# jzhang-dev/FEDRANN

Hardware: AMD Instinct MI355X
Metric: read-pairs/sec (overlap candidates) (higher is better)
Workload: dtype f32 (canonical fp32 results; fp16 MFMA candidate prefilter + exact fp32 re-rank)

## Files before the change

### fedrann_amd/csrc/fedrann_hip.hip

```cpp
#include <hip/hip_runtime.h>
#include <rocprim/device/device_radix_sort.hpp>
#include <rocprim/device/device_scan.hpp>
#include <rocprim/device/device_run_length_encode.hpp>
#include <rocprim/device/device_merge.hpp>
#include <rocprim/device/device_reduce_by_key.hpp>

#include <algorithm>
#include <array>
#include <atomic>
#include <cmath>
#include <condition_variable>
#include <cstdarg>
#include <cstdint>
#include <cstdio>
#include <cstdlib>
#include <cstring>
#include <functional>
#include <limits>
#include <mutex>
#include <new>
#include <string>
#include <thread>
#include <type_traits>
#include <utility>
// ... 392 lines not shown
    auto ask = [&](const auto &call) {
        size_t bytes = 0;
        if (e == hipSuccess) e = call(nullptr, bytes);
        need = std::max(need, bytes);
    };
    (ask(calls), ...);
    if (e != hipSuccess) return fail(FDR_E_HIP, "rocprim temporary storage size query failed: %s", hipGetErrorString(e));
    return tmp.reserve(need);
}
template <class F>
static int rocprim_run(DevArray<char> &tmp, const char *what, const F &call) {
    if (int rc = rocprim_reserve(tmp, call)) return rc;
    size_t bytes = tmp.bytes();
    const hipError_t e = call(tmp.ptr(), bytes);
    if (e != hipSuccess)
        return fail(e == hipErrorOutOfMemory ? FDR_E_NOMEM : FDR_E_HIP, "%s failed: %s", what, hipGetErrorString(e));
    return FDR_OK;
}

struct PinnedBuf {
    void *p = nullptr;
    size_t cap = 0;
    int reserve(size_t bytes) {
        if (bytes <= cap) return FDR_OK;
        if (p) (void)hipHostFree(p);
        p = nullptr;
        cap = 0;
        hipError_t e = hipHostMalloc(&p, bytes ? bytes : 1, hipHostMallocDefault);
        if (e != hipSuccess) {
            p = nullptr;
            return fail(FDR_E_NOMEM, "hipHostMalloc(%zu bytes) failed: %s", bytes, hipGetErrorString(e));
        }
        cap = bytes;
        return FDR_OK;
    }
    PinnedBuf() = default;
    PinnedBuf(const PinnedBuf &) = delete;
    PinnedBuf &operator=(const PinnedBuf &) = delete;
    ~PinnedBuf() {
        if (p) (void)hipHostFree(p);
    }
};

struct KnnCallRecord {
    struct {
        int flagged = 0;
        int launches = 0, queues = 0;
    } pass;
    int unique_targets = 0, unique_queries = 0;
    struct {
        const uint8_t *dev = nullptr;
        int64_t n = 0;
        uint8_t all = FDR_PATH_NONE;
        hipStream_t stream = nullptr;
    } paths;
    fdr_knn_trace trace = {};
    struct {
        int nseg = 0;
        int nt = 0;
        SegBounds segs;
        hipStream_t stream = nullptr;
    } skip;
};

struct KnnArgs {
    const float *Qhat;
    const uint8_t *qzero;
    int64_t nq;
    const float *That;
    const uint8_t *tzero;
    int64_t nt, t_base;
    int d, k;
    int32_t *idx;
    float *dist;
    void *ws;
    size_t ws_bytes;
    hipStream_t st;
};


struct KmerSearchScratch {
    DevArray<unsigned char> seq;
    DevArray<long long> off;
    DevArray<u64> lib_codes;
    DevArray<u64> keys;
    DevArray<unsigned> vals;
    DevArray<u64> bloom;
    DevArray<unsigned long long> counter;
    DevArray<u64> pairs, sorted;
    DevArray<int> flag, scan;
    DevArray<int> indices, rows;
    DevArray<long long> indptr;
    DevArray<char> tmp;
    long long nnz = 0;
    void release() {
        release_all(seq, off, lib_codes, keys, vals, bloom, counter, pairs, sorted, flag, scan, indices, rows, indptr, tmp);
        nnz = 0;
    }
};

struct KmerCountScratch {
    DevArray<unsigned char> seq;
    DevArray<long long> off;
    DevArray<u64> codes;
    DevArray<u64> sorted;
    DevArray<unsigned> run_len;
    DevArray<unsigned> n_runs;
    DevArray<u64> run_counts;
    DevArray<u64> acc_codes[2], acc_counts[2];
    DevArray<u64> merged_codes, merged_counts;
    DevArray<unsigned long long> n_table;
    DevArray<int> keep, keep_scan;
    DevArray<u64> kept_counts;
    DevArray<long long> run_off, samp_pre;
    DevArray<u64> samples, bounds;
    DevArray<long long> slices;
    DevArray<long long> part_off;
    DevArray<char> tmp;
    int k = 0;
    int acc = 0;
    long long na = 0;
    long long n = 0;
    int64_t block_chars = 0;
    int blocks = 0;
    void release() {
        release_all(seq, off, codes, sorted, run_len, n_runs, run_counts, acc_codes[0], acc_codes[1], acc_counts[0],
                    acc_counts[1], merged_codes, merged_counts, n_table, keep, keep_scan, kept_counts, run_off, samp_pre,
                    samples, bounds, slices, part_off, tmp);
        k = acc = 0;
        na = n = 0;
    }
};

struct SparseIndex {
    DevArray<long long> indptr;
    DevArray<int> indices;
    DevArray<float> values;
    DevArray<float> xhat;
    DevArray<int> asize;
    DevArray<float> mass;
    DevArray<unsigned char> zero;
    DevArray<u64> keys, sorted_keys;
    DevArray<unsigned> pos, sorted_pos;
    DevArray<int> efeat;
    DevArray<float> pval;
    DevArray<long long> runptr;
    DevArray<int> runfeat;
    DevArray<int> heavy;
    DevArray<u64> cnt;
    DevArray<char> tmp;
    struct Built {
        bool valid = false;
        int metric = 0;
        long long n = 0, kept = 0, nzero = 0;
        long long n_features = 0;
    } built;
    int *run_flags() const { return reinterpret_cast<int *>(keys.ptr()); }
    int *run_numbers(long long kept) const { return run_flags() + kept; }
    int *posting_rows() const { return reinterpret_cast<int *>(pos.ptr()); }
    static constexpr size_t cnt_words = 8 + FDR_MAX_K;
    int *zidx() const { return reinterpret_cast<int *>(cnt.ptr() + 8); }
    float *zdist() const { return reinterpret_cast<float *>(zidx() + FDR_MAX_K); }
    template <class F>
    auto each(F f) {
        return f(indptr, indices, values, xhat, asize, mass, zero, keys, sorted_keys, pos, sorted_pos, efeat, pval, runptr,
                 runfeat, heavy, cnt, tmp);
    }
    size_t bytes() {
        return each([](auto &...a) { return (a.bytes() + ...); });
    }
    void release() {
        each([](auto &...a) { release_all(a...); });
        built = {};
    }
};

struct SparseQuerySet {
    DevArray<long long> indptr;
    DevArray<int> indices;
    DevArray<float> values;
    DevArray<float> xhat;
    DevArray<int> efeat;
    DevArray<int> asize;
    DevArray<float> mass;
    DevArray<unsigned char> zero;
    DevArray<int> heavy;
    template <class F>
    auto each(F f) {
        return f(indptr, indices, values, xhat, efeat, asize, mass, zero, heavy);
    }
    size_t bytes() {
        return each([](auto &...a) { return (a.bytes() + ...); });
    }
    void release() {
        each([](auto &...a) { release_all(a...); });
    }
};

#define RR_FLAG_MISMATCH 0
#define RR_FLAG_ZLIST 1
#define RR_FLAG_ZEROQ 2
#define RR_FLAG_NZERO 3
#define RR_FLAGS 4
struct RadiusResult {
    DevArray<long long> count, off;
    DevArray<u64> keys, sorted;
    DevArray<int> zlist;
    DevArray<u64> flags;
    long long counted = 0;
    long long held = -1;
    int *idx() const { return reinterpret_cast<int *>(keys.ptr()); }
    float *dist() const { return reinterpret_cast<float *>(idx() + held); }
    void drop() { held = -1; }
    template <class F>
    auto each(F f) { return f(count, off, keys, sorted, zlist, flags); }
    size_t bytes() { return each([](auto &...a) { return (a.bytes() + ...); }); }
    void release() {
        each([](auto &...a) { release_all(a...); });
        counted = 0;
        held = -1;
    }
};

struct SparseRadius {
    RadiusResult rr;
    DevArray<long long> seg_lo, seg_hi;
    DevArray<unsigned char> handed;
    size_t bytes() { return rr.bytes() + seg_lo.bytes() + seg_hi.bytes() + handed.bytes(); }
    void release() {
        rr.release();
        release_all(seg_lo, seg_hi, handed);
    }
};

struct DenseIndex {
    DevArray<float> ehat;
    DevArray<_Float16> half;
    DevArray<unsigned char> zero;
    DevArray<float> qhat;
    DevArray<_Float16> qhalf;
    DevArray<unsigned char> qzero;
    DevArray<float> theta;
    RadiusResult rr;
    DevArray<long long> ind;
    DevArray<int> fill;
    DevArray<char> tmp;
    bool valid = false;
    long long n = 0, nzero = 0;
    int d = 0, dp = 0;
    long long last_candidates = 0, last_hits = 0;
    int last_query_blocks = 0, last_segments = 0;
    template <class F>
    auto each(F f) {
        return f(ehat, half, zero, qhat, qhalf, qzero, theta, ind, fill, tmp);
    }
    size_t bytes() { return rr.bytes() + each([](auto &...a) { return (a.bytes() + ...); }); }
    void release() {
        each([](auto &...a) { release_all(a...); });
        rr.release();
        valid = false;
        n = nzero = 0;
        d = dp = 0;
        last_candidates = last_hits = 0;
        last_query_blocks = last_segments = 0;
    }
};

struct TopkMergeScratch {
    DevArray<int> idx_parts;
    DevArray<float> dist_parts;
    DevArray<int> idx_out;
    DevArray<float> dist_out;
    DevArray<u64> refusal;
    void release() { release_all(idx_parts, dist_parts, idx_out, dist_out, refusal); }
};

struct fdr_ctx {
    int device = 0;
    int num_cus = 256;
    hipStream_t stream = nullptr;
    hipStream_t aux_stream[3] = {nullptr, nullptr, nullptr};
    hipEvent_t aux_ev[4] = {nullptr, nullptr, nullptr, nullptr};
    hipDeviceProp_t prop;
    long long n_features = 0;
    int d = 0;
    long long p_nnz = 0, p_rows = 0;
    DevBuf ftab, crow, ent;
    std::vector<uint32_t> h_bits;
    DevBuf a_indptr, a_indices, E, Ehat, zero, idx, dist, ws;
    DevBuf c_indptr, c_indices;
    PinnedBuf stage_ids, stage_ptr;
    hipEvent_t up_ev[3] = {nullptr, nullptr, nullptr};
    hup::WorkerPool up_pool;
    KmerSearchScratch ks;
    KmerCountScratch kc;
    SparseIndex sp;
    SparseQuerySet spq;
    SparseRadius spr;
    DenseIndex di;
    TopkMergeScratch tm;
    int knn_mode = FDR_MODE_AUTO;
    int dedup_mode = FDR_DEDUP_AUTO;
    int live_mode = FDR_LIVE_AUTO;
    std::vector<unsigned> live_host;
    int skip_mode = FDR_SKIP_AUTO;
    std::vector<int> skip_host;
    int compact_mode = FDR_COMPACT_AUTO;
    KnnCallRecord last;
    struct {
        int what = 0;
        bool cand_valid = false, range_valid = false;
        int64_t nq = 0, n_range = 0;
        int kp = 0, qbits = 0;
        DevBuf cand, rq, rtheta, rcnt, rrows;
        DevBuf lists;
        hipStream_t stream = nullptr;
    } cap;
    struct {
        bool valid = false;
        const float *That = nullptr;
        const uint8_t *tzero = nullptr;
        int64_t nt = 0, nq_max = 0;
        int d = 0, k = 0, nu = 0;
        void *ws = nullptr;
        size_t ws_bytes = 0;
    } cls;
    bool timing = false;
    std::vector<hipEvent_t> ev_pool[FDR_NUM_KERNELS];
    size_t ev_used[FDR_NUM_KERNELS] = {};
};

static void knn_call_begin(fdr_ctx *ctx) {
    ctx->last.trace = fdr_knn_trace{};
    ctx->last.paths = {};
    ctx->last.skip.nseg = 0;
    ctx->cap.cand_valid = ctx->cap.range_valid = false;
    ctx->cap.nq = ctx->cap.n_range = 0;
}

static void knn_call_header(fdr_ctx *ctx, int kind, int dp, int k, int64_t nq, int64_t nt) {
    ctx->last.trace.kind = kind;
    ctx->last.trace.dp = dp;
    ctx->last.trace.k = k;
    ctx->last.trace.queries = nq;
    ctx->last.trace.targets = nt;
}
static void knn_call_whole(fdr_ctx *ctx, uint8_t path, int kind, int dp, int k, int64_t nq, int64_t nt) {
    knn_call_header(ctx, kind, dp, k, nq, nt);
    ctx->last.paths = {nullptr, nq, path, nullptr};
    ctx->last.pass = {};
}

static int timing_begin(fdr_ctx *ctx, int kind, hipStream_t st) {
    if (!ctx->timing) return FDR_OK;
    std::vector<hipEvent_t> &pool = ctx->ev_pool[kind];
    if (ctx->ev_used[kind] + 2 > pool.size()) {
        hipEvent_t a, b;
        HIP_TRY(hipEventCreate(&a));
        HIP_TRY(hipEventCreate(&b));
        pool.push_back(a);
        pool.push_back(b);
    }
    HIP_TRY(hipEventRecord(pool[ctx->ev_used[kind]], st));
    return FDR_OK;
}

static int timing_end(fdr_ctx *ctx, int kind, hipStream_t st) {
    if (!ctx->timing) return FDR_OK;
    HIP_TRY(hipEventRecord(ctx->ev_pool[kind][ctx->ev_used[kind] + 1], st));
    ctx->ev_used[kind] += 2;
    return FDR_OK;
}

static int use_device(fdr_ctx *ctx) {
    if (!ctx) return fail(FDR_E_ARG, "null context");
    HIP_TRY(hipSetDevice(ctx->device));
    return FDR_OK;
}

FDR_EXPORT const char *fdr_last_error(void) { return g_err; }

FDR_EXPORT int fdr_padded_dim(int d) { return padded_dim(d); }

FDR_EXPORT int fdr_create(int device_id, fdr_ctx **out) {
    if (!out) return fail(FDR_E_ARG, "fdr_create: out is null");
    *out = nullptr;
    int n = 0;
    HIP_TRY(hipGetDeviceCount(&n));
    if (n <= 0) return fail(FDR_E_HIP, "no HIP device visible: the MI355X path cannot run");
    if (device_id < 0 || device_id >= n)
        return fail(FDR_E_ARG, "device %d out of range (have %d)", device_id, n);
    fdr_ctx *c = new (std::nothrow) fdr_ctx();
    if (!c) return fail(FDR_E_NOMEM, "out of host memory");
    c->device = device_id;
    hipError_t e = hipSetDevice(device_id);
    if (e == hipSuccess) e = hipGetDeviceProperties(&c->prop, device_id);
    if (e == hipSuccess) e = hipStreamCreateWithFlags(&c->stream, hipStreamNonBlocking);
    if (e != hipSuccess) {
        delete c;
        return fail(FDR_E_HIP, "fdr_create: device %d: %s", device_id, hipGetErrorString(e));
    }
    c->num_cus = c->prop.multiProcessorCount > 0 ? c->prop.multiProcessorCount : 256;
    if (const char *m = getenv("FDR_KNN_MODE")) {
        if (strcmp(m, "exact") == 0) c->knn_mode = FDR_MODE_EXACT;
        else if (strcmp(m, "prefilter") == 0) c->knn_mode = FDR_MODE_PREFILTER;
    }
    *out = c;
    return FDR_OK;
}

FDR_EXPORT int fdr_destroy(fdr_ctx *ctx) {
    if (!ctx) return FDR_OK;
    (void)hipSetDevice(ctx->device);
    (void)hipStreamSynchronize(ctx->stream);
    ctx->up_pool.stop();
    for (hipEvent_t e : ctx->up_ev)
        if (e) (void)hipEventDestroy(e);
    for (int i = 0; i < FDR_NUM_KERNELS; ++i)
        for (hipEvent_t e : ctx->ev_pool[i]) (void)hipEventDestroy(e);
    (void)hipStreamDestroy(ctx->stream);
    for (hipStream_t a : ctx->aux_stream)
        if (a) {
            (void)hipStreamSynchronize(a);
            (void)hipStreamDestroy(a);
        }
    for (hipEvent_t e : ctx->aux_ev)
        if (e) (void)hipEventDestroy(e);
    delete ctx;
    return FDR_OK;
}

FDR_EXPORT int fdr_device_info(fdr_ctx *ctx, char *buf, int buflen) {
    if (!ctx || !buf || buflen <= 0) return fail(FDR_E_ARG, "fdr_device_info: bad argument");
    snprintf(buf, (size_t)buflen, "%s|%s|%d|%zu", ctx->prop.name, ctx->prop.gcnArchName,
             ctx->prop.multiProcessorCount, (size_t)ctx->prop.totalGlobalMem);
    return FDR_OK;
}

FDR_EXPORT int fdr_last_uncertified(fdr_ctx *ctx) { return ctx ? ctx->last.pass.flagged : 0; }

FDR_EXPORT int fdr_last_query_paths(fdr_ctx *ctx, uint8_t *paths, int64_t n_queries) {
    int rc = use_device(ctx);
    if (rc) return rc;
    if (!paths || n_queries <= 0) return fail(FDR_E_ARG, "last_query_paths: bad argument");
    const auto &rec = ctx->last.paths;
    if (rec.n != n_queries)
        return fail(FDR_E_STATE, "last_query_paths: the last k-NN call recorded codes for %lld query rows, not %lld",
                    (long long)rec.n, (long long)n_queries);
    if (!rec.dev) {
        memset(paths, rec.all, (size_t)n_queries);
        return FDR_OK;
    }
    HIP_TRY(hipMemcpyAsync(paths, rec.dev, (size_t)n_queries, hipMemcpyDeviceToHost, rec.stream));
    HIP_TRY(hipStreamSynchronize(rec.stream));
    return FDR_OK;
}

FDR_EXPORT int fdr_last_unique(fdr_ctx *ctx, int *unique_targets, int *unique_queries) {
    if (!ctx || !unique_targets || !unique_queries) return fail(FDR_E_ARG, "bad argument");
    *unique_targets = ctx->last.unique_targets;
    *unique_queries = ctx->last.unique_queries;
    return FDR_OK;
}

FDR_EXPORT int fdr_last_prefilter_launches(fdr_ctx *ctx, int *launches, int *queues) {
    if (!ctx || !launches || !queues) return fail(FDR_E_ARG, "bad argument");
    *launches = ctx->last.pass.launches;
    *queues = ctx->last.pass.queues;
    return FDR_OK;
}

FDR_EXPORT int fdr_last_knn_trace(fdr_ctx *ctx, fdr_knn_trace *out) {
    if (!ctx || !out) return fail(FDR_E_ARG, "bad argument");
    *out = ctx->last.trace;
    return FDR_OK;
}

FDR_EXPORT int fdr_set_knn_capture(fdr_ctx *ctx, int what) {
    if (!ctx || what < 0 || what > (FDR_CAPTURE_CANDIDATES | FDR_CAPTURE_RANGE | FDR_CAPTURE_LIVE_LISTS)) return fail(FDR_E_ARG, "bad capture flags");
    ctx->cap.what = what;
    return FDR_OK;
}

FDR_EXPORT int fdr_last_candidates(fdr_ctx *ctx, uint64_t *keys, int64_t n_queries, int32_t kp, int32_t *qbits_out) {
    int rc = use_device(ctx);
    if (rc) return rc;
    if (!keys || n_queries <= 0 || kp <= 0) return fail(FDR_E_ARG, "last_candidates: bad argument");
    if (!ctx->cap.cand_valid) return fail(FDR_E_STATE, "last_candidates: the last k-NN call captured no candidates");
    if (ctx->cap.nq != n_queries || ctx->cap.kp != kp)
        return fail(FDR_E_STATE, "last_candidates: the last k-NN call captured %lld x %d keys, not %lld x %d",
                    (long long)ctx->cap.nq, ctx->cap.kp, (long long)n_queries, kp);
    HIP_TRY(hipMemcpyAsync(keys, ctx->cap.cand.p, (size_t)n_queries * kp * 8, hipMemcpyDeviceToHost, ctx->cap.stream));
    HIP_TRY(hipStreamSynchronize(ctx->cap.stream));
    if (qbits_out) *qbits_out = ctx->cap.qbits;
    return FDR_OK;
}

FDR_EXPORT int fdr_last_range_sets(fdr_ctx *ctx, int64_t n_range, int32_t *queries, float *theta, int32_t *counts,
                                   int32_t *rows) {
    int rc = use_device(ctx);
    if (rc) return rc;
    if (!queries || !theta || !counts || !rows || n_range <= 0) return fail(FDR_E_ARG, "last_range_sets: bad argument");
    if (!ctx->cap.range_valid) return fail(FDR_E_STATE, "last_range_sets: the last k-NN call captured no range pass");
    if (ctx->cap.n_range != n_range)
        return fail(FDR_E_STATE, "last_range_sets: the last k-NN call captured %lld range queries, not %lld",
                    (long long)ctx->cap.n_range, (long long)n_range);
    const hipStream_t st = ctx->cap.stream;
    HIP_TRY(hipMemcpyAsync(queries, ctx->cap.rq.p, (size_t)n_range * 4, hipMemcpyDeviceToHost, st));
    HIP_TRY(hipMemcpyAsync(theta, ctx->cap.rtheta.p, (size_t)n_range * 4, hipMemcpyDeviceToHost, st));
    HIP_TRY(hipMemcpyAsync(counts, ctx->cap.rcnt.p, (size_t)n_range * 4, hipMemcpyDeviceToHost, st));
    HIP_TRY(hipMemcpyAsync(rows, ctx->cap.rrows.p, (size_t)n_range * RANGE_CAP * 4, hipMemcpyDeviceToHost, st));
    HIP_TRY(hipStreamSynchronize(st));
    for (int64_t i = 0; i < n_range; ++i)
        for (int m = std::max(0, std::min(counts[i], RANGE_CAP)); m < RANGE_CAP; ++m) rows[i * RANGE_CAP + m] = -1;
    return FDR_OK;
}

FDR_EXPORT int fdr_set_knn_mode(fdr_ctx *ctx, int mode) {
    if (!ctx || mode < FDR_MODE_AUTO || mode > FDR_MODE_PREFILTER) return fail(FDR_E_ARG, "bad k-NN mode");
    ctx->knn_mode = mode;
    return FDR_OK;
}

FDR_EXPORT int fdr_set_dedup_mode(fdr_ctx *ctx, int mode) {
    if (!ctx || mode < FDR_DEDUP_AUTO || mode > FDR_DEDUP_FORCE) return fail(FDR_E_ARG, "bad duplicate-row mode");
    ctx->dedup_mode = mode;
    return FDR_OK;
}

FDR_EXPORT int fdr_set_live_chunks(fdr_ctx *ctx, int mode) {
    if (!ctx || mode < FDR_LIVE_AUTO || mode > FDR_LIVE_FORCE) return fail(FDR_E_ARG, "bad live-chunk mode");
    ctx->live_mode = mode;
    return FDR_OK;
}

FDR_EXPORT int fdr_set_live_skip(fdr_ctx *ctx, int mode) {
    if (!ctx || mode < FDR_SKIP_AUTO || mode > FDR_SKIP_OFF) return fail(FDR_E_ARG, "bad stage-skip mode");
    ctx->skip_mode = mode;
    return FDR_OK;
}

FDR_EXPORT int fdr_set_rerank_compact(fdr_ctx *ctx, int mode) {
    if (!ctx || mode < FDR_COMPACT_AUTO || mode > FDR_COMPACT_FORCE) return fail(FDR_E_ARG, "bad compact re-rank mode");
    ctx->compact_mode = mode;
    return FDR_OK;
}

FDR_EXPORT int fdr_last_live_stage_lists(fdr_ctx *ctx, int32_t segment, int32_t *first_row_out, int32_t *nstages_out,
                                         int32_t *lens, uint16_t *lists) {
    int rc = use_device(ctx);
    if (rc) return rc;
    const auto &rec = ctx->last.skip;
    if (rec.nseg <= 0)
        return fail(FDR_E_STATE, "last_live_stage_lists: the last k-NN call captured no live-chunk pass's stage lists");
    if (segment < 0 || segment >= rec.nseg || !nstages_out)
        return fail(FDR_E_ARG, "last_live_stage_lists: bad argument (the pass had %d segments)", rec.nseg);
    const int t_begin = rec.segs.b[segment], t_end = std::min(rec.nt, rec.segs.b[segment + 1]);
    const int nstages = t_end > t_begin ? (t_end - t_begin + 127) >> 7 : 0;
    *nstages_out = nstages;
    if (first_row_out) *first_row_out = t_begin;
    if (lens) memcpy(lens, ctx->skip_host.data() + (size_t)segment * 256, 256 * sizeof(int));
    if (!lists || nstages == 0) return FDR_OK;
    const int stride = live_list_stride(nstages);
    HIP_TRY(hipMemcpy2DAsync(lists, (size_t)nstages * 2, static_cast<const uint16_t *>(ctx->cap.lists.p) + (size_t)live_stage_row(t_begin, segment) * 256,
                             (size_t)stride * 2, (size_t)nstages * 2, 256, hipMemcpyDeviceToHost, rec.stream));
    HIP_TRY(hipStreamSynchronize(rec.stream));
    for (int v = 0; v < 256; ++v)
        for (int i = std::max(0, std::min(ctx->skip_host[(size_t)segment * 256 + v], nstages)); i < nstages; ++i)
            lists[(size_t)v * nstages + i] = 0xffffu;
    return FDR_OK;
}

FDR_EXPORT int fdr_timing(fdr_ctx *ctx, int enable) {
    if (!ctx) return fail(FDR_E_ARG, "null context");
    ctx->timing = enable != 0;
    for (int i = 0; i < FDR_NUM_KERNELS; ++i) ctx->ev_used[i] = 0;
    return FDR_OK;
}

FDR_EXPORT int fdr_timing_read(fdr_ctx *ctx, int which, int *count_out, float *total_ms_out) {
    int rc = use_device(ctx);
    if (rc) return rc;
    if (which < 0 || which >= FDR_NUM_KERNELS || !count_out || !total_ms_out)
        return fail(FDR_E_ARG, "fdr_timing_read: bad argument");
    float total = 0.f;
    const size_t used = ctx->ev_used[which];
    for (size_t i = 0; i + 1 < used; i += 2) {
        float ms = 0.f;
        HIP_TRY(hipEventSynchronize(ctx->ev_pool[which][i + 1]));
        HIP_TRY(hipEventElapsedTime(&ms, ctx->ev_pool[which][i], ctx->ev_pool[which][i + 1]));
        total += ms;
    }
    *count_out = (int)(used / 2);
    *total_ms_out = total;
    ctx->ev_used[which] = 0;
    return FDR_OK;
}

FDR_EXPORT int fdr_projection_load(fdr_ctx *ctx, int64_t n_features, int32_t d,
                                   const int64_t *p_indptr, const int32_t *p_cols,
                                   const float *p_vals) {
    int rc = use_device(ctx);
    if (rc) return rc;
    ProjectionTables T;
    if ((rc = build_projection_tables(n_features, d, p_indptr, p_cols, p_vals, T))) return rc;
    const std::vector<PU2> &ftab = T.ftab, &ent = T.ent;
    const std::vector<PU4> &crow = T.rowinfo;
    const int64_t nnz = p_indptr[n_features];
    const unsigned rows = T.rows;
    static_assert(sizeof(PU2) == sizeof(uint2) && sizeof(PU4) == sizeof(uint4), "table records = the kernel's uint2 / uint4");
    if ((rc = ctx->ftab.reserve(ftab.size() * sizeof(uint2)))) return rc;
    if ((rc = ctx->crow.reserve(crow.size() * sizeof(uint4)))) return rc;
    if ((rc = ctx->ent.reserve(ent.size() * sizeof(uint2)))) return rc;
    HIP_TRY(hipMemcpyAsync(ctx->ftab.p, ftab.data(), ftab.size() * sizeof(uint2), hipMemcpyHostToDevice, ctx->stream));
    HIP_TRY(hipMemcpyAsync(ctx->crow.p, crow.data(), crow.size() * sizeof(uint4), hipMemcpyHostToDevice, ctx->stream));
    HIP_TRY(hipMemcpyAsync(ctx->ent.p, ent.data(), ent.size() * sizeof(uint2), hipMemcpyHostToDevice, ctx->stream));
    HIP_TRY(hipStreamSynchronize(ctx->stream));
    ctx->n_features = n_features;
    ctx->d = d;
    ctx->p_nnz = nnz;
    ctx->p_rows = rows;
    ctx->h_bits.resize(ftab.size());
    for (size_t w = 0; w < ftab.size(); ++w) ctx->h_bits[w] = ftab[w].x;
    return FDR_OK;
}

FDR_EXPORT int fdr_csr_compact(fdr_ctx *ctx, int64_t n_rows, const int64_t *a_indptr, const int32_t *a_indices,
                               int64_t *out_indptr, int32_t *out_indices, int64_t out_capacity, int32_t n_threads) {
    if (!ctx) return fail(FDR_E_ARG, "null context");
    if (ctx->n_features <= 0) return fail(FDR_E_STATE, "csr_compact: no projection loaded");
    return csrc::compact(ctx->h_bits, ctx->n_features, n_rows, a_indptr, a_indices, out_indptr, out_indices,
                         out_capacity, n_threads);
}

FDR_EXPORT int fdr_host_register(fdr_ctx *ctx, void *ptr, size_t bytes) {
    int rc = use_device(ctx);
    if (rc) return rc;
    if (!ptr || bytes == 0) return fail(FDR_E_ARG, "host_register: empty buffer");
    HIP_TRY(hipHostRegister(ptr, bytes, hipHostRegisterDefault));
    return FDR_OK;
}

FDR_EXPORT int fdr_host_unregister(fdr_ctx *ctx, void *ptr) {
    int rc = use_device(ctx);
    if (rc) return rc;
    if (!ptr) return fail(FDR_E_ARG, "host_unregister: null pointer");
    HIP_TRY(hipHostUnregister(ptr));
    return FDR_OK;
}

static int launch_embed(fdr_ctx *ctx, int64_t n_rows, const int64_t *d_indptr,
                        const int32_t *d_indices, float *d_E, hipStream_t st) {
    if (ctx->n_features <= 0) return fail(FDR_E_STATE, "embed: no projection loaded");
    if (n_rows < 0) return fail(FDR_E_ARG, "embed: n_rows < 0");
    if (n_rows == 0) return FDR_OK;
    const int dp = fdr_padded_dim(ctx->d);
    const long long blocks_needed = (n_rows + 7) / 8;
    const int grid = (int)std::min<long long>(blocks_needed, (long long)ctx->num_cus * 8 * 4);
    int trc = timing_begin(ctx, FDR_KERNEL_EMBED, st);
    if (trc) return trc;
#define FDR_LAUNCH_EMBED(DP_)                                                                   \
    hipLaunchKernelGGL(FDR_EMBED_KERNEL<DP_>, dim3(grid), dim3(256), 0, st, (long long)n_rows,  \
                       (const long long *)d_indptr, d_indices, ctx->n_features,                 \
                       (const uint2 *)ctx->ftab.p, (const uint4 *)ctx->crow.p,                  \
                       (const uint2 *)ctx->ent.p, ctx->d, d_E)
#define FDR_EMBED_KERNEL embed_csr_kernel
    if (dp == 128)
        FDR_LAUNCH_EMBED(128);
    else if (dp == 256)
        FDR_LAUNCH_EMBED(256);
    else if (dp == 512)
        FDR_LAUNCH_EMBED(512);
#undef FDR_EMBED_KERNEL
#define FDR_EMBED_KERNEL embed_csr_wide_kernel
    else if (dp == 1024)
        FDR_LAUNCH_EMBED(1024);
    else
        FDR_LAUNCH_EMBED(2048);
#undef FDR_EMBED_KERNEL
#undef FDR_LAUNCH_EMBED
    HIP_TRY(hipGetLastError());
    return timing_end(ctx, FDR_KERNEL_EMBED, st);
}

static int launch_normalize(fdr_ctx *ctx, const float *d_E, int64_t n_rows, int d, float *d_Ehat,
                            uint8_t *d_zero, hipStream_t st) {
    const int dp = fdr_padded_dim(d);
    if (dp < 0) return fail(FDR_E_ARG, "normalize: dimension %d unsupported (1..%d)", d, FDR_MAX_DIM);
    if (n_rows < 0) return fail(FDR_E_ARG, "normalize: n_rows < 0");
    if (n_rows == 0) return FDR_OK;
    const int rb = dp == 128 ? 64 : dp == 256 ? 32 : dp == 512 ? 16 : dp == 1024 ? 8 : 4;
    const long long grid = (n_rows + rb - 1) / rb;
    if (grid > 0x7fffffffll) return fail(FDR_E_ARG, "normalize: too many rows");
    int trc = timing_begin(ctx, FDR_KERNEL_NORMALIZE, st);
    if (trc) return trc;
    const bool vec = d % 4 == 0 && (reinterpret_cast<uintptr_t>(d_E) & 15) == 0 && (reinterpret_cast<uintptr_t>(d_Ehat) & 15) == 0;
#define FDR_LAUNCH_NORM(DP_, RB_)                                                                                  \
    do {                                                                                                            \
        if (vec)                                                                                                    \
            hipLaunchKernelGGL((normalize_rows_kernel<DP_, RB_, true>), dim3((unsigned)grid), dim3(256), 0, st, d_E, \
                               (long long)n_rows, d, d_Ehat, d_zero);                                              \
        else                                                                                                        \
            hipLaunchKernelGGL((normalize_rows_kernel<DP_, RB_, false>), dim3((unsigned)grid), dim3(256), 0, st,    \
                               d_E, (long long)n_rows, d, d_Ehat, d_zero);                                         \
    } while (0)
    if (dp == 128) FDR_LAUNCH_NORM(128, 64);
    else if (dp == 256) FDR_LAUNCH_NORM(256, 32);
    else if (dp == 512) FDR_LAUNCH_NORM(512, 16);
    else if (dp == 1024) FDR_LAUNCH_NORM(1024, 8);
    else FDR_LAUNCH_NORM(2048, 4);
#undef FDR_LAUNCH_NORM
    HIP_TRY(hipGetLastError());
    return timing_end(ctx, FDR_KERNEL_NORMALIZE, st);
}

static size_t order_sort_tmp_bytes(size_t rows) {
    size_t t = 0;
    (void)rocprim::radix_sort_pairs(nullptr, t, (u64 *)nullptr, (u64 *)nullptr, (int *)nullptr, (int *)nullptr, rows, 0, 40,
                                    (hipStream_t) nullptr);
    return t;
}
static size_t class_tables_tmp_bytes(size_t rows) {
    size_t t_sort = 0, t_scan = 0;
    (void)rocprim::radix_sort_pairs(nullptr, t_sort, (u64 *)nullptr, (u64 *)nullptr, (int *)nullptr, (int *)nullptr, rows, 0,
                                    64, (hipStream_t) nullptr);
    (void)rocprim::inclusive_scan(nullptr, t_scan, (int *)nullptr, (int *)nullptr, rows, rocprim::plus<int>(),
                                  (hipStream_t) nullptr);
    return std::max(t_sort, t_scan);
}
static WsEnv ws_env(const fdr_ctx *ctx) {
    return {ctx->num_cus, ctx->knn_mode, ctx->dedup_mode, order_sort_tmp_bytes, class_tables_tmp_bytes, ctx->live_mode,
            ctx->compact_mode};
}

FDR_EXPORT size_t fdr_knn_workspace_bytes(fdr_ctx *ctx, int64_t nq, int64_t nt, int32_t d,
                                          int32_t k) {
    if (!ctx || nq <= 0 || nt <= 0 || k <= 0 || k > FDR_MAX_K || fdr_padded_dim(d) < 0) return 0;
    return knn_workspace_bytes(ws_env(ctx), nq, nt, d, k);
}

#ifndef FDR_SHAPE_MASK
#define FDR_SHAPE_MASK (~0ull)
#endif
#ifndef FDR_LH_MASK
#define FDR_LH_MASK 48
#endif
typedef void (*TileKernel)(const float *, const unsigned char *, int, const float *, const unsigned *, int, int, SegBounds,
                           int, int, u64 *, unsigned *, int, int, int FDR_DBG_PARAM);
typedef void (*PassKernel)(const _Float16 *, int, const _Float16 *, int, int, SegBounds, int, int, u64 *, unsigned *, int,
                           int, int, OrderArgs FDR_DBG_PARAM);
typedef void (*RangeKernel)(const _Float16 *, const float *, int, const _Float16 *, int, int, SegBounds, RangeOut);
static_assert(kShapes[FDR_R128].tps == RANGE_STAGES && kShapes[FDR_R256].tps == RANGE_STAGES &&
              kShapes[FDR_R512].tps == RANGE_STAGES, "the range kernel's ring");

template <int S>
static constexpr bool shape_compiled() {
    constexpr KnnShape e = kShapes[S];
#ifdef FDR_DEV
    constexpr bool built = true;
#else
    constexpr bool built = e.release;
#endif
    constexpr bool pass = e.family == FDR_FAM_PREFILTER || e.family == FDR_FAM_PINGPONG;
    return built && (!pass || (((unsigned long long)(FDR_SHAPE_MASK) >> S) & 1));
}
template <int S>
static constexpr TileKernel tile_kernel() {
    constexpr KnnShape e = kShapes[S];
    if constexpr (e.family == FDR_FAM_TILE && shape_compiled<S>()) return knn_tile_kernel<e.dp, e.nq, e.nw, e.wps>;
    else if constexpr (e.family == FDR_FAM_TILE_SPLIT && shape_compiled<S>()) return knn_tile_split_kernel<e.dp>;
    else return nullptr;
}
template <int S, int LH>
static constexpr PassKernel pass_kernel() {
    constexpr KnnShape e = kShapes[S];
    if constexpr (!shape_compiled<S>() || !(e.lists & LH & FDR_LH_MASK)) return nullptr;
    else if constexpr (e.family == FDR_FAM_PREFILTER)
        return knn_prefilter_kernel<e.dp, e.nq, e.nw, e.wps, e.units(), LH, e.paired && LH == 16>;
    else if constexpr (e.family == FDR_FAM_PINGPONG) return knn_prefilter_pp_kernel<e.dp, e.units(), LH>;
    else return nullptr;
}
template <int S>
static constexpr RangeKernel range_kernel() {
    constexpr KnnShape e = kShapes[S];
    if constexpr (!shape_compiled<S>()) return nullptr;
    else if constexpr (e.family == FDR_FAM_RANGE) return knn_range_kernel<e.dp, e.nw, e.dp == 128 ? e.wps : 2>;
    else if constexpr (e.family == FDR_FAM_RANGE_PP) return knn_range_pp_kernel<e.dp, e.units()>;
    else return nullptr;
}
template <size_t... S>
struct KnnKernelTable {
    static constexpr TileKernel tile[] = {tile_kernel<S>()...};
    static constexpr PassKernel pass[][2] = {{pass_kernel<S, 16>(), pass_kernel<S, 32>()}...};
    static constexpr RangeKernel range[] = {range_kernel<S>()...};
};
template <size_t... S>
static KnnKernelTable<S...> knn_kernel_table(std::index_sequence<S...>);
typedef decltype(knn_kernel_table(std::make_index_sequence<FDR_NUM_SHAPES>())) KnnKernels;

static int no_kernel(int shape) {
    return fail(FDR_E_STATE, "this development build was compiled without the kernel shape this call needs (kShapes[%d])",
                shape);
}

#include "knn_debug.inc"

struct Rounds { int launches = 0, queues = 0; };
template <class Launch>
static int launch_rounds(fdr_ctx *ctx, const KnnPlan &p, const std::vector<long long> &items, int max_queues, int kind,
                         bool span_each, hipStream_t st, Rounds &r, Launch launch) {
    const int dealt = p.cohort > 0 ? std::max(1, std::min(p.queues, max_queues)) : 1;
    const std::vector<RoundLaunch> sched = round_schedule(items, p.cohort > 0 ? p.cohort : 0, dealt);
    const int nqueues = sched.size() > 1 ? dealt : 1;
    hipStream_t qs[4] = {st, st, st, st};
    if (nqueues > 1) {
        if (!ctx->aux_ev[0]) {
            for (hipStream_t &a : ctx->aux_stream) HIP_TRY(hipStreamCreateWithFlags(&a, hipStreamNonBlocking));
            for (hipEvent_t &e : ctx->aux_ev) HIP_TRY(hipEventCreateWithFlags(&e, hipEventDisableTiming));
        }
        for (int q = 1; q < nqueues; ++q) qs[q] = ctx->aux_stream[q - 1];
    }
    const bool one_span = nqueues > 1 || !span_each;
    int trc;
    if (one_span && (trc = timing_begin(ctx, kind, st))) return trc;
    if (nqueues > 1) {
        HIP_TRY(hipEventRecord(ctx->aux_ev[0], st));
        for (int q = 1; q < nqueues; ++q) HIP_TRY(hipStreamWaitEvent(qs[q], ctx->aux_ev[0], 0));
    }
    for (const RoundLaunch &l : sched) {
        const hipStream_t ls = qs[l.queue];
        if (!one_span && (trc = timing_begin(ctx, kind, ls))) return trc;
        launch(ls, (unsigned)l.grid, l.base, l.group);
        if (!one_span && (trc = timing_end(ctx, kind, ls))) return trc;
    }
    HIP_TRY(hipGetLastError());
    r.launches = (int)sched.size();
    r.queues = nqueues;
    for (int q = 1; q < nqueues; ++q) {
        HIP_TRY(hipEventRecord(ctx->aux_ev[q], qs[q]));
        HIP_TRY(hipStreamWaitEvent(st, ctx->aux_ev[q], 0));
    }
    return one_span ? timing_end(ctx, kind, st) : FDR_OK;
}

static int check_knn_args(fdr_ctx *, const KnnArgs &a) {
    const int dp = fdr_padded_dim(a.d);
    if (dp < 0) return fail(FDR_E_ARG, "knn: dimension %d unsupported (1..%d)", a.d, FDR_MAX_DIM);
    if (a.k < 1 || a.k > FDR_MAX_K) return fail(FDR_E_ARG, "knn: k=%d, d=%d outside the MFMA kernels' shapes", a.k, a.d);
    if (a.nq < 0 || a.nt < a.k) return fail(FDR_E_ARG, "knn: need n_targets (%lld) >= k (%d)", (long long)a.nt, a.k);
    if (a.nt + a.t_base > 0x7fffffffll || a.nq > 0x7fffffffll) return fail(FDR_E_ARG, "knn: row numbers exceed int32");
    if (a.nq == 0) return FDR_OK;
    const bool need_ws = knn_route(dp, a.k, a.nt) != FDR_ROUTE_GENERIC;
    if (!a.Qhat || !a.qzero || !a.That || !a.tzero || !a.idx || !a.dist || (need_ws && !a.ws))
        return fail(FDR_E_ARG, "knn: null device pointer");
    return FDR_OK;
}
static_assert(FDR_MAX_K == FDR_EXACT_MAX_K, "every k the generic kernel takes, the exact MFMA pass takes from 8192 targets");

static int launch_knn_exact(fdr_ctx *ctx, const KnnArgs &a) {
    if (a.nq == 0) return FDR_OK;
    const hipStream_t st = a.st;
    const int k = a.k;
    const KnnPlan p = knn_plan(ctx->num_cus, a.nq, a.nt, a.d, k);
    if (a.ws_bytes < p.total_bytes) return fail(FDR_E_ARG, "knn: workspace %zu < required %zu bytes", a.ws_bytes, p.total_bytes);
    const TileKernel kern = KnnKernels::tile[p.shape];
    if (!kern) return no_kernel(p.shape);
    const PlanRegions R = plan_regions(a.ws, p);
    hipLaunchKernelGGL(pack_zero_bits_kernel, dim3((unsigned)((a.nt + 255) / 256)), dim3(256), 0, st,
                       a.tzero, (int)a.nt, R.bits, R.shared, p.nq_pad);
    HIP_TRY(hipGetLastError());
    const KnnShape &sh = kShapes[p.shape];
    const size_t lds = knn_lds_bytes(sh, k);
    if (lds > 160 * 1024) return fail(FDR_E_ARG, "knn: k=%d, d=%d needs %zu B of LDS (> 160 KiB)", k, a.d, lds);
    ctx->last.trace.exact_calls++;
    ctx->last.trace.exact_queries += (int32_t)a.nq;
    ctx->last.trace.exact_waves = sh.nw;
    ctx->last.trace.exact_qsets = sh.nq;
    ctx->last.trace.exact_segments = p.nseg;
    [[maybe_unused]] const int dbg = dev_knobs().debug;
    const int qcap = knn_qcap(sh, k);
    HIP_TRY(hipFuncSetAttribute(reinterpret_cast<const void *>(kern), hipFuncAttributeMaxDynamicSharedMemorySize, (int)lds));
    Rounds r;
    int trc = launch_rounds(ctx, p, {(long long)p.nqb * p.nseg}, 2, FDR_KERNEL_KNN_TILE, false, st, r,
                            [&](hipStream_t s, unsigned grid, int base, int) {
        hipLaunchKernelGGL(kern, dim3(grid), dim3(64 * sh.nw), lds, s, a.Qhat, a.qzero, (int)a.nq, a.That, R.bits, (int)a.nt,
                           (int)a.t_base, p.segs, k, p.nq_pad, R.partial, R.shared, qcap, base, p.nqb FDR_DBG_ARG(dbg));
    });
    if (trc) return trc;
    if ((trc = dump_debug_counters(st, "tile", p, "update calls, rounds, flushes, flush iterations, rescans, -"))) return trc;
    if ((trc = timing_begin(ctx, FDR_KERNEL_KNN_MERGE, st))) return trc;
    hipLaunchKernelGGL(k <= FDR_FAST_MAX_K ? knn_merge_kernel : knn_merge_wide_kernel, dim3((unsigned)((a.nq + 3) / 4)),
                       dim3(256), 0, st, (const u64 *)R.partial, p.nseg, (int)a.nq, p.nq_pad, k, a.idx, a.dist);
    HIP_TRY(hipGetLastError());
    return timing_end(ctx, FDR_KERNEL_KNN_MERGE, st);
}

struct PrefilterCounts { int exact, zero, range; };
struct PrefilterCall {
    fdr_ctx *ctx;
    KnnArgs a;
    bool self;
    int dp;
    PrefilterWs L;
    int shape;
    KnnPlan p;
    PassKernel kern;
    PlanRegions R;
    int ib;
    const _Float16 *p1_q, *p1_t;
    OrderArgs ord;
    const KnnShape &sh() const { return kShapes[shape]; }
    size_t lds() const { return knn_lds_bytes(sh(), L.kp); }
    _Float16 *hq() const { return self ? L.ht : L.hq; }
    int setup(), pass_dense(Rounds &r), pass_live(Rounds &r);
    int certify(PrefilterCounts &n), range(PrefilterCounts &n), exact_rest(const PrefilterCounts &n);
};

int PrefilterCall::setup() {
    const hipStream_t st = a.st;
    const int64_t nq = a.nq, nt = a.nt;
    int trc = timing_begin(ctx, FDR_KERNEL_KNN_RERANK, st);
    if (trc) return trc;
    HIP_TRY(hipMemsetAsync(L.counter, 0, 64, st));
    if (L.rc) {
        hipLaunchKernelGGL(to_half_compact_kernel, dim3((unsigned)((nt * (dp / 8) + 255) / 256)), dim3(256), 0, st, a.That,
                           (long long)nt * (dp / 8), L.ht, L.rc, L.counter + 8);
    } else
        hipLaunchKernelGGL(to_half_kernel, dim3((unsigned)((nt * (dp / 8) + 255) / 256)), dim3(256), 0, st, a.That,
                           (long long)nt * (dp / 8), L.ht);
    if (!self)
        hipLaunchKernelGGL(to_half_kernel, dim3((unsigned)((nq * (dp / 8) + 255) / 256)), dim3(256), 0, st, a.Qhat,
                           (long long)nq * (dp / 8), L.hq);
    hipLaunchKernelGGL(pack_zero_bits_kernel, dim3((unsigned)((nt + 255) / 256)), dim3(256), 0, st,
                       a.tzero, (int)nt, R.bits, R.shared, p.nq_pad);
    HIP_TRY(hipGetLastError());
    ord = {nullptr, nullptr};
    p1_q = hq();
    p1_t = L.ht;
    if (L.ordered) {
        _Float16 *const ho_t = L.ho_t, *const ho_q = self ? L.ho_t : L.ho_q;
        auto order = [&](const float *X, int64_t n, int *perm, _Float16 *out) -> int {
            hipLaunchKernelGGL(row_chunk_keys_kernel, dim3((unsigned)(((size_t)n * 16 + 255) / 256)), dim3(256), 0, st, X,
                               (int)n, dp, L.okeys, L.ovals);
            size_t tb = L.otmp_bytes;
            HIP_TRY(rocprim::radix_sort_pairs(L.otmp, tb, L.okeys, L.okeys_s, L.ovals, perm, (size_t)n, 0, 40, st));
            const long long groups = (long long)n * (dp / 8);
            hipLaunchKernelGGL(to_half_ordered_kernel, dim3((unsigned)((groups + 255) / 256)), dim3(256), 0, st, X,
                               (const int *)perm, groups, dp / 8, out);
            HIP_TRY(hipGetLastError());
            return FDR_OK;
        };
        int orc;
        if ((orc = order(a.That, nt, L.perm_t, ho_t))) return orc;
        if (L.live) {
            int max_stages = 1;
            for (int i = 0; i < p.nseg; ++i)
                max_stages = std::max(max_stages, (std::min<int>((int)nt, p.segs.b[i + 1]) - p.segs.b[i] + 127) >> 7);
            hipLaunchKernelGGL(live_stage_masks_kernel, dim3((unsigned)max_stages, (unsigned)p.nseg), dim3(64), 0, st,
                               (const u64 *)L.okeys_s, (int)nt, p.segs, L.live_smask);
            const int all = !(FDR_SKIP_AUTO_ON && ctx->skip_mode == FDR_SKIP_AUTO);
            hipLaunchKernelGGL(live_stage_lists_kernel, dim3(256, (unsigned)p.nseg), dim3(64), 0, st,
                               (const uint8_t *)L.live_smask, (int)nt, p.segs, all, L.live_lists, L.live_lens);
            HIP_TRY(hipGetLastError());
            ctx->last.trace.skip_live = !all;
        }
        if (!self && (orc = order(a.Qhat, nq, L.perm_q, ho_q))) return orc;
        ord.perm_t = L.perm_t;
        p1_t = ho_t;
        ord.perm_q = self ? L.perm_t : L.perm_q;
        p1_q = ho_q;
        if (L.live) {
            const long long bgroups = (long long)((nt + 31) / 32 + 4) * 32 * 16;
            hipLaunchKernelGGL(to_half_blocked_kernel, dim3((unsigned)((bgroups + 255) / 256)), dim3(256), 0, st, a.That,
                               (const int *)L.perm_t, (int)nt, bgroups, L.hb_t);
            hipLaunchKernelGGL(live_block_masks_kernel, dim3((unsigned)((nq + 255) / 256)), dim3(64), 0, st,
                               (const u64 *)L.okeys_s, (int)nq, L.live_masks);
            HIP_TRY(hipGetLastError());
        }
    }
    int max_seg = 1;
    for (int i = 0; i < p.nseg; ++i) max_seg = std::max(max_seg, p.segs.b[i + 1] - p.segs.b[i]);
    ib = prefilter_index_bits(max_seg);
    if (ib > FDR_PREFILTER_MAX_IB) return fail(FDR_E_ARG, "knn prefilter: segment of %d rows", max_seg);
    if ((trc = timing_end(ctx, FDR_KERNEL_KNN_RERANK, st))) return trc;
    if (lds() > 32768)
        HIP_TRY(hipFuncSetAttribute(reinterpret_cast<const void *>(kern), hipFuncAttributeMaxDynamicSharedMemorySize, (int)lds()));
    return FDR_OK;
}

int PrefilterCall::pass_dense(Rounds &r) {
    return launch_rounds(ctx, p, {(long long)p.nqb * p.nseg}, 4, FDR_KERNEL_KNN_PREFILTER, true, a.st, r,
                         [&](hipStream_t s, unsigned grid, int base, int) {
        hipLaunchKernelGGL(kern, dim3(grid), dim3(64 * sh().nw), lds(), s, p1_q, (int)a.nq, p1_t, (int)a.nt, (int)a.t_base,
                           p.segs, L.kp, p.nq_pad, R.partial, R.shared, ib, base, p.nqb, ord FDR_DBG_ARG(dev_knobs().debug));
    });
}

int PrefilterCall::pass_live(Rounds &r) {
    const hipStream_t st = a.st;
    const int nqb = p.nqb, kp = L.kp;
    fdr_knn_trace &tr = ctx->last.trace;
    std::vector<unsigned> &masks = ctx->live_host;
    masks.resize((size_t)nqb);
    HIP_TRY(hipMemcpyAsync(masks.data(), L.live_masks, (size_t)nqb * 4, hipMemcpyDeviceToHost, st));
    std::vector<int> &lens = ctx->skip_host;
    lens.resize((size_t)p.nseg * 256);
    HIP_TRY(hipMemcpyAsync(lens.data(), L.live_lens, (size_t)p.nseg * 256 * 4, hipMemcpyDeviceToHost, st));
    HIP_TRY(hipStreamSynchronize(st));
    if (ctx->cap.what & FDR_CAPTURE_LIVE_LISTS) {
        const size_t bytes = live_stage_rows(a.nt) * 256 * sizeof(uint16_t);
        int crc = ctx->cap.lists.reserve(bytes);
        if (crc) return crc;
        HIP_TRY(hipMemcpyAsync(ctx->cap.lists.p, L.live_lists, bytes, hipMemcpyDeviceToDevice, st));
        ctx->last.skip.nseg = p.nseg;
        ctx->last.skip.nt = (int)a.nt;
        ctx->last.skip.segs = p.segs;
        ctx->last.skip.stream = st;
    }
    const LivePlan lp = live_plan(masks.data(), nqb, p.nseg, ctx->live_mode == FDR_LIVE_FORCE ? 0 : p.cohort);
    HIP_TRY(hipMemcpyAsync(L.live_ids, lp.ids.data(), (size_t)nqb * 4, hipMemcpyHostToDevice, st));
    HIP_TRY(hipMemcpyAsync(L.live_order, lp.order.data(), (size_t)nqb * 4, hipMemcpyHostToDevice, st));
    HIP_TRY(hipStreamSynchronize(st));
    tr.pass_live = 1;
    int dense_nq = 0;
    std::vector<long long> items;
    for (const LiveGroup &g : lp.groups) {
        items.push_back((long long)g.count * p.nseg);
        if (g.nl != FDR_LIVE_DENSE) {
            tr.pass_live_items[g.nl - FDR_LIVE_MIN_NL] = g.count * p.nseg;
            for (int sg = 0; sg < p.nseg; ++sg) {
                const int len = std::min<int>((int)a.nt, p.segs.b[sg + 1]) - p.segs.b[sg];
                const int64_t nst = len > 0 ? (len + 127) >> 7 : 0;
                int64_t walked = 0;
                for (int i = 0; i < g.count; ++i)
                    walked += std::min<int64_t>(nst, lens[(size_t)sg * 256 + (masks[(size_t)lp.order[(size_t)(g.first + i)]] & 0xffu)]);
                tr.skip_stages_walked += walked;
                tr.skip_stages_skipped += nst * g.count - walked;
            }
            continue;
        }
        tr.pass_live_dense_items = g.count * p.nseg;
        const int last = lp.order[(size_t)(g.first + g.count - 1)];
        dense_nq = (g.count - 1) * 256 + (int)std::min<int64_t>(256, a.nq - (int64_t)last * 256);
        hipLaunchKernelGGL(live_gather_dense_kernel, dim3((unsigned)g.count), dim3(256), 0, st, p1_q, ord.perm_q,
                           (const unsigned *)R.shared, (int)a.nq, (const int *)(L.live_order + g.first), L.live_hq,
                           L.live_perm, L.live_tau);
    }
    for (int nl = FDR_LIVE_MIN_NL; nl <= FDR_LIVE_MAX_NL; ++nl)
        if (live_lds_bytes(nl) > 32768)
            HIP_TRY(hipFuncSetAttribute(reinterpret_cast<const void *>(kLiveKernels[nl - FDR_LIVE_MIN_NL]),
                                        hipFuncAttributeMaxDynamicSharedMemorySize, (int)live_lds_bytes(nl)));
    return launch_rounds(ctx, p, items, 4, FDR_KERNEL_KNN_PREFILTER, false, st, r,
                         [&](hipStream_t s, unsigned grid, int base, int group) {
        const LiveGroup &g = lp.groups[(size_t)group];
        if (g.nl == FDR_LIVE_DENSE)
            hipLaunchKernelGGL(kern, dim3(grid), dim3(64 * sh().nw), lds(), s, (const _Float16 *)L.live_hq, dense_nq, p1_t,
                               (int)a.nt, (int)a.t_base, p.segs, kp, p.nq_pad, R.partial, L.live_tau, ib, base, g.count,
                               OrderArgs{ord.perm_t, (const int *)L.live_perm} FDR_DBG_ARG(dev_knobs().debug));
        else
            hipLaunchKernelGGL(kLiveKernels[g.nl - FDR_LIVE_MIN_NL], dim3(grid), dim3(512), live_lds_bytes(g.nl), s,
                               p1_q, (int)a.nq, (const _Float16 *)L.hb_t, (int)a.nt, (int)a.t_base, p.segs, kp, p.nq_pad,
                               R.partial, R.shared, ib, base, g.count, (const int *)(L.live_order + g.first),
                               (const unsigned *)L.live_ids, ord, (const unsigned *)L.live_masks,
                               reinterpret_cast<const unsigned *>(L.live_lists), (const int *)L.live_lens);
    });
}

int PrefilterCall::certify(PrefilterCounts &n) {
    const hipStream_t st = a.st;
    const int kp = L.kp, k = a.k;
    const int64_t nq = a.nq;
    int trc;
    if ((trc = timing_begin(ctx, FDR_KERNEL_KNN_RERANK, st))) return trc;
    const int64_t mq = p.nseg * kp <= 64 ? 4 * MERGE_QPW : 4;
    hipLaunchKernelGGL(knn_merge_keys_kernel, dim3((unsigned)((nq + mq - 1) / mq)), dim3(256), 0, st,
                       (const u64 *)R.partial, p.nseg, (int)nq, p.nq_pad, kp, L.cand);
    HIP_TRY(hipGetLastError());
    if (ctx->cap.what & FDR_CAPTURE_CANDIDATES) {
        if ((trc = ctx->cap.cand.reserve((size_t)nq * kp * 8))) return trc;
        HIP_TRY(hipMemcpyAsync(ctx->cap.cand.p, L.cand, (size_t)nq * kp * 8, hipMemcpyDeviceToDevice, st));
        ctx->cap.nq = nq;
        ctx->cap.kp = kp;
        ctx->cap.qbits = std::min(20, 32 - ib);
        ctx->cap.stream = st;
        ctx->cap.cand_valid = true;
    }
    const float margin = 2.0f * prefilter_eps(ib) + 4.0e-7f;
    const auto rerank = L.rc ? knn_rerank_kernel<RERANK_ROWS_COMPACT> : knn_rerank_kernel<RERANK_ROWS_DENSE>;
    const int rerank_lds = L.rc ? RERANK_LDS_BYTES(RERANK_ROWS_COMPACT) : RERANK_LDS_BYTES(RERANK_ROWS_DENSE);
    const int long_limit = ctx->compact_mode == FDR_COMPACT_FORCE ? 0x7fffffff : (int)(a.nt / RC_LONG_SHARE);
    HIP_TRY(hipFuncSetAttribute(reinterpret_cast<const void *>(rerank), hipFuncAttributeMaxDynamicSharedMemorySize, rerank_lds));
    hipLaunchKernelGGL(rerank, dim3((unsigned)((nq + 3) / 4)), dim3(256), rerank_lds, st,
                       (const u64 *)L.cand, kp, k, a.Qhat, a.qzero, a.That, (int)nq, dp, (int)a.t_base, margin,
                       a.idx, a.dist, L.counter, L.flagged, L.rlist, L.theta, L.path, (const unsigned char *)L.rc, long_limit);
    hipLaunchKernelGGL(zero_answer_kernel, dim3(1), dim3(1024), 0, st, (const unsigned *)R.bits, (int)a.nt,
                       (int)a.t_base, k, L.zidx, L.zdist);
    hipLaunchKernelGGL(scatter_zero_answer_kernel, dim3((unsigned)(((int64_t)nq * k + 255) / 256)),
                       dim3(256), 0, st, (const int *)L.zidx, (const float *)L.zdist,
                       (const int *)L.flagged, (int)nq, (const int *)L.counter, k, a.idx, a.dist);
    HIP_TRY(hipGetLastError());
    if ((trc = timing_end(ctx, FDR_KERNEL_KNN_RERANK, st))) return trc;
    int counts[9] = {};
    HIP_TRY(hipMemcpyAsync(counts, L.counter, sizeof counts, hipMemcpyDeviceToHost, st));
    HIP_TRY(hipStreamSynchronize(st));
    n = {counts[0], counts[1], counts[2]};
    ctx->last.trace.rerank_compact = L.rc && counts[8] <= long_limit;
    ctx->last.trace.rerank_compact_entries = L.rc ? RC_ENTRIES : 0;
    ctx->last.trace.rerank_compact_long = counts[8];
    ctx->last.pass.flagged = n.exact + n.range;
    ctx->last.trace.uncertified = n.exact;
    ctx->last.trace.zero_queries = n.zero;
    ctx->last.trace.range_queries = n.range;
    return FDR_OK;
}

int PrefilterCall::range(PrefilterCounts &n) {
    const hipStream_t st = a.st;
    const int rcount = n.range;
    fdr_knn_trace &tr = ctx->last.trace;
    int trc;
    if ((trc = timing_begin(ctx, FDR_KERNEL_KNN_RERANK, st))) return trc;
    const bool rcap = ctx->cap.what & FDR_CAPTURE_RANGE;
    if (rcap) {
        if ((trc = ctx->cap.rq.reserve((size_t)rcount * 4)) || (trc = ctx->cap.rtheta.reserve((size_t)rcount * 4)) ||
            (trc = ctx->cap.rcnt.reserve((size_t)rcount * 4)) || (trc = ctx->cap.rrows.reserve((size_t)rcount * RANGE_CAP * 4)))
            return trc;
        ctx->cap.stream = st;
    }
    for (int first = 0; first < rcount; first += L.rchunk) {
        const int cq = std::min(L.rchunk, rcount - first);
        hipLaunchKernelGGL(gather_half_queries_kernel, dim3((unsigned)cq), dim3(256), 0, st, (const _Float16 *)hq(),
                           (const float *)L.theta, (const int *)L.rlist, first, cq, dp, L.hqc, L.thetac, L.cnt);
        HIP_TRY(hipGetLastError());
        const int rs = range_shape(dp, cq, rcount);
        const KnnShape &rsh = kShapes[rs];
        const RangeKernel rk = KnnKernels::range[rs];
        if (!rk) return no_kernel(rs);
        const KnnPlan rp = knn_plan(ctx->num_cus, cq, a.nt, a.d, 1, rs);
        const size_t rlds = knn_lds_bytes(rsh, 1) + (size_t)RANGE_LANE_BUF * 64 * rsh.nw * 4;
        if (rsh.family == FDR_FAM_RANGE_PP)
            HIP_TRY(hipFuncSetAttribute(reinterpret_cast<const void *>(rk), hipFuncAttributeMaxDynamicSharedMemorySize, (int)rlds));
        hipLaunchKernelGGL(rk, dim3((unsigned)rp.nqb, (unsigned)rp.nseg), dim3(64 * rsh.nw), rlds, st, (const _Float16 *)L.hqc,
                           (const float *)L.thetac, cq, (const _Float16 *)L.ht, (int)a.nt, (int)a.t_base, rp.segs, RangeOut{L.cnt, L.rcand});
        HIP_TRY(hipGetLastError());
        tr.range_chunks++;
        tr.range_pp_chunks += rsh.family == FDR_FAM_RANGE_PP;
        tr.range_w8_chunks += rs == FDR_R128_W8;
        if (rcap) {
            auto keep = [&](const DevBuf &to, const void *from, size_t row_bytes) {
                return hipMemcpyAsync(static_cast<char *>(to.p) + first * row_bytes, from, cq * row_bytes, hipMemcpyDeviceToDevice, st);
            };
            HIP_TRY(keep(ctx->cap.rq, L.rlist + first, 4));
            HIP_TRY(keep(ctx->cap.rtheta, L.thetac, 4));
            HIP_TRY(keep(ctx->cap.rcnt, L.cnt, 4));
            HIP_TRY(keep(ctx->cap.rrows, L.rcand, (size_t)RANGE_CAP * 4));
        }
        hipLaunchKernelGGL(knn_rerank_long_kernel, dim3((unsigned)((cq + 3) / 4)), dim3(256), 0, st,
                           (const int *)(L.rlist + first), cq, (const int *)L.cnt, (const int *)L.rcand, a.k,
                           a.Qhat, a.That, dp, (int)a.t_base, a.idx, a.dist, L.counter, L.flagged, L.path);
        HIP_TRY(hipGetLastError());
    }
    if (rcap) {
        ctx->cap.n_range = rcount;
        ctx->cap.range_valid = true;
    }
    if ((trc = timing_end(ctx, FDR_KERNEL_KNN_RERANK, st))) return trc;
    int count = 0;
    HIP_TRY(hipMemcpyAsync(&count, L.counter, 4, hipMemcpyDeviceToHost, st));
    HIP_TRY(hipStreamSynchronize(st));
    tr.range_overflow = count - n.exact;
    n.exact = count;
    return FDR_OK;
}

int PrefilterCall::exact_rest(const PrefilterCounts &n) {
    const hipStream_t st = a.st;
    KnnArgs e = a;
    e.ws_bytes = L.knn_bytes;
    if ((int64_t)n.exact * 2 > a.nq - n.zero) {
        ctx->last.trace.exact_fallback = FDR_FALLBACK_WHOLE;
        ctx->last.paths = {nullptr, a.nq, FDR_PATH_EXACT, nullptr};
        return launch_knn_exact(ctx, e);
    }
    ctx->last.trace.exact_fallback = FDR_FALLBACK_CHUNKED;
    e.Qhat = L.qc;
    e.qzero = L.qzc;
    e.idx = L.idxc;
    e.dist = L.distc;
    for (int first = 0; first < n.exact; first += L.chunk) {
        const int cq = std::min(L.chunk, n.exact - first);
        hipLaunchKernelGGL(gather_queries_kernel, dim3((unsigned)cq), dim3(256), 0, st, a.Qhat, a.qzero,
                           (const int *)L.flagged, first, cq, dp, L.qc, L.qzc);
        HIP_TRY(hipGetLastError());
        e.nq = cq;
        int rc = launch_knn_exact(ctx, e);
        if (rc) return rc;
        hipLaunchKernelGGL(scatter_results_kernel, dim3((unsigned)(((int64_t)cq * a.k + 255) / 256)), dim3(256), 0, st,
                           (const int *)L.idxc, (const float *)L.distc, (const int *)L.flagged, first, cq, a.k, a.idx, a.dist);
        HIP_TRY(hipGetLastError());
    }
    return FDR_OK;
}

static int launch_knn_prefilter(fdr_ctx *ctx, const KnnArgs &a) {
    PrefilterCall c = {ctx, a};
    c.self = a.Qhat == a.That && a.qzero == a.tzero && a.nq == a.nt;
    c.dp = fdr_padded_dim(a.d);
    c.L = prefilter_ws(ws_env(ctx), a.ws, a.nq, a.nt, a.d, a.k);
    if (a.ws_bytes < c.L.total) return fail(FDR_E_ARG, "knn: workspace %zu < required %zu bytes", a.ws_bytes, c.L.total);
    const int kp = c.L.kp;
    knn_call_header(ctx, FDR_TRACE_PREFILTER, c.dp, a.k, a.nq, a.nt);
    ctx->last.paths = {c.L.path, a.nq, FDR_PATH_NONE, a.st};

    c.shape = prefilter_shape_live(ctx->live_mode, c.dp, kp, a.nq, ctx->num_cus, a.nt);
    c.p = knn_plan(ctx->num_cus, a.nq, a.nt, a.d, kp, c.shape);
    fdr_knn_trace &tr = ctx->last.trace;
    tr.kp = kp;
    tr.pass_waves = c.sh().nw;
    tr.pass_wps = c.sh().wps;
    tr.pass_units = c.sh().tps;
    tr.pass_list_keys = kp <= 32 ? 16 : 32;
    tr.pass_pingpong = c.sh().family == FDR_FAM_PINGPONG;
    tr.pass_segments = c.p.nseg;
    c.kern = KnnKernels::pass[c.shape][kp > 32];
    if (!c.kern) return no_kernel(c.shape);
    c.R = plan_regions(c.L.knn, c.p);
    int rc;
    if ((rc = c.setup())) return rc;
    Rounds r;
    rc = c.L.live ? c.pass_live(r) : c.pass_dense(r);
    ctx->last.pass.launches = r.launches;
    ctx->last.pass.queues = r.queues;
    tr.pass_launches = r.launches;
    tr.pass_queues = r.queues;
    if (rc) return rc;
#ifdef FDR_STAMPS
    if ((rc = dump_stamps(a.st, c.sh().nw))) return rc;
#endif
    if ((rc = dump_debug_counters(a.st, "prefilter", c.p, "wave-tiles, cold, groups, rounds, second rounds, candidates"))) return rc;
    PrefilterCounts n;
    if ((rc = c.certify(n))) return rc;
    if (n.range > 0 && (rc = c.range(n))) return rc;
    if (n.exact <= 0) return FDR_OK;
    return c.exact_rest(n);
}

static int launch_knn_mode(fdr_ctx *ctx, const KnnArgs &a) {
    const int dp = fdr_padded_dim(a.d);
    if (knn_route(dp, a.k, a.nt) == FDR_ROUTE_FAST && a.nq > 0 && knn_prefilter_wanted(ctx->knn_mode, a.nt, a.k)) {
        const int rc = launch_knn_prefilter(ctx, a);
        if (rc) ctx->cap.cand_valid = ctx->cap.range_valid = false;
        return rc;
    }
    knn_call_whole(ctx, FDR_PATH_EXACT, FDR_TRACE_EXACT, dp, a.k, a.nq, a.nt);
    return launch_knn_exact(ctx, a);
}

static int queue_class_tables(const DedupWs &W, const float *d_That, int n, int dp, hipStream_t st) {
    const unsigned g1 = (unsigned)((n + 255) / 256);
    size_t tb = W.tmp_bytes;
    HIP_TRY(rocprim::radix_sort_pairs(W.tmp, tb, W.hash, W.hash_s, W.idx, W.idx_s, (size_t)n, 0, 64, st));
    hipLaunchKernelGGL(mark_class_starts_kernel, dim3(g1), dim3(256), 0, st, d_That, n, dp, (const u64 *)W.hash_s,
                       (const int *)W.idx_s, W.flag);
    tb = W.tmp_bytes;
    HIP_TRY(rocprim::inclusive_scan(W.tmp, tb, W.flag, W.cid, (size_t)n, rocprim::plus<int>(), st));
    hipLaunchKernelGGL(class_tables_kernel, dim3(g1), dim3(256), 0, st, n, (const int *)W.flag, (const int *)W.cid,
                       (const int *)W.idx_s, W.cls, W.cstart, W.isrep);
    tb = W.tmp_bytes;
    HIP_TRY(rocprim::inclusive_scan(W.tmp, tb, W.isrep, W.upos, (size_t)n, rocprim::plus<int>(), st));
    hipLaunchKernelGGL(unique_tables_kernel, dim3(g1), dim3(256), 0, st, n, (const int *)W.isrep, (const int *)W.upos,
                       (const int *)W.cls, (const int *)W.cstart, W.uofc, W.cofu, W.rep_m);
    HIP_TRY(hipGetLastError());
    return FDR_OK;
}

static int launch_expand(const DedupWs &W, int64_t q0, int64_t nq, int k, int64_t t_base, const int *uqpos,
                         const int32_t *idx_u, const float *dist_u, int64_t u_stride, int32_t *d_idx, float *d_dist,
                         const uint8_t *upath, uint8_t path_all, uint8_t *rowpath, hipStream_t st) {
    const int xw = (size_t)4 * k * k * 8 <= 32768 ? 4 : (size_t)2 * k * k * 8 <= 32768 ? 2 : 1;
    const int xq = xw * (64 / k) * EXPAND_UNROLL;
    hipLaunchKernelGGL(expand_classes_kernel, dim3((unsigned)((nq + xq - 1) / xq)), dim3(64 * xw), (size_t)xw * k * k * 8,
                       st, (int)q0, (int)nq, k, 64 / k, (int)t_base, (const int *)W.cls, (const int *)W.uofc, uqpos,
                       (const int *)idx_u, dist_u, (const int *)W.idx_s, (const int4 *)W.rep_m, d_idx, d_dist,
                       (int)u_stride, upath, path_all, rowpath);
    HIP_TRY(hipGetLastError());
    return FDR_OK;
}

static int launch_knn(fdr_ctx *ctx, const KnnArgs &a) {
    int rc = check_knn_args(ctx, a);
    if (rc) return rc;
    const float *const d_Qhat = a.Qhat, *const d_That = a.That;
    const int64_t nq = a.nq, nt = a.nt;
    const int d = a.d, k = a.k;
    const hipStream_t st = a.st;
    const int dp = fdr_padded_dim(d);
    const int route = knn_route(dp, k, nt);
    if (route == FDR_ROUTE_GENERIC) {
        if (nq == 0) return FDR_OK;
        ctx->last.unique_targets = (int)nt;
        ctx->last.unique_queries = (int)nq;
        knn_call_whole(ctx, FDR_PATH_GENERIC, FDR_TRACE_GENERIC, dp, k, nq, nt);
        ctx->last.trace.generic = 1;
        int trc = timing_begin(ctx, FDR_KERNEL_KNN_TILE, st);
        if (trc) return trc;
        hipLaunchKernelGGL(knn_generic_kernel, dim3((unsigned)((nq + GEN_QPB - 1) / GEN_QPB)), dim3(256),
                           (size_t)GEN_QPB * dp * 4, st, d_Qhat, a.qzero, (int)nq, d_That, a.tzero, (int)nt, (int)a.t_base, dp, k,
                           a.idx, a.dist);
        HIP_TRY(hipGetLastError());
        return timing_end(ctx, FDR_KERNEL_KNN_TILE, st);
    }
    auto plain = [&](size_t bytes) {
        ctx->last.unique_targets = (int)nt;
        ctx->last.unique_queries = (int)nq;
        KnnArgs b = a;
        b.ws_bytes = bytes;
        return launch_knn_mode(ctx, b);
    };
    const bool q_in_t = nq > 0 && d_Qhat >= d_That && d_Qhat + (size_t)nq * dp <= d_That + (size_t)nt * dp &&
                        ((d_Qhat - d_That) % dp) == 0;
    if (!(route == FDR_ROUTE_FAST && q_in_t && knn_dedup_wanted(ctx->dedup_mode, nq, nt))) return plain(a.ws_bytes);
    const WsEnv env = ws_env(ctx);
    const DedupWs W = dedup_ws(env, a.ws, nq, nt, d, k);
    if (a.ws_bytes < W.total) return fail(FDR_E_ARG, "knn: workspace %zu < required %zu bytes", a.ws_bytes, W.total);
    const int n = (int)nt;
    const int q0 = (int)((d_Qhat - d_That) / dp);
    const unsigned g16 = (unsigned)(((size_t)n * 16 + 255) / 256), g1 = (unsigned)((n + 255) / 256);

    int trc = timing_begin(ctx, FDR_KERNEL_KNN_DEDUP, st);
    if (trc) return trc;
    hipLaunchKernelGGL(hash_rows_kernel, dim3(g16), dim3(256), 0, st, d_That, n, dp, W.hash, W.idx);
    HIP_TRY(hipGetLastError());
    if (ctx->dedup_mode != FDR_DEDUP_FORCE && W.probe_slots) {
        HIP_TRY(hipMemsetAsync(W.probe_table, 0, (size_t)W.probe_slots * 8 + 4, st));
        hipLaunchKernelGGL(dedup_probe_kernel, dim3(g1), dim3(256), 0, st, (const u64 *)W.hash, n, W.probe_table,
                           W.probe_slots - 1, W.probe_count);
        HIP_TRY(hipGetLastError());
        int dups = 0;
        HIP_TRY(hipMemcpyAsync(&dups, W.probe_count, 4, hipMemcpyDeviceToHost, st));
        HIP_TRY(hipStreamSynchronize(st));
        if ((double)dups < 0.05 * (double)n) {
            if ((trc = timing_end(ctx, FDR_KERNEL_KNN_DEDUP, st))) return trc;
            return plain(W.inner_bytes);
        }
    }
    if ((rc = queue_class_tables(W, d_That, n, dp, st))) return rc;
    HIP_TRY(hipMemsetAsync(W.uqflag, 0, (size_t)n * 4, st));
    hipLaunchKernelGGL(mark_query_classes_kernel, dim3((unsigned)((nq + 255) / 256)), dim3(256), 0, st, q0,
                       (int)nq, (const int *)W.cls, (const int *)W.uofc, W.uqflag);
    size_t tb = W.tmp_bytes;
    HIP_TRY(rocprim::inclusive_scan(W.tmp, tb, W.uqflag, W.uqpos, (size_t)n, rocprim::plus<int>(), st));
    HIP_TRY(hipGetLastError());
    int nu = 0, nuq = 0;
    HIP_TRY(hipMemcpyAsync(&nu, W.cid + (n - 1), 4, hipMemcpyDeviceToHost, st));
    HIP_TRY(hipMemcpyAsync(&nuq, W.uqpos + (n - 1), 4, hipMemcpyDeviceToHost, st));
    HIP_TRY(hipStreamSynchronize(st));
    if (!dedup_worth(nu, nuq, nt, nq, k, ctx->dedup_mode) || knn_mode_workspace_bytes(env, nuq, nu, d, k) > W.inner_bytes) {
        if ((trc = timing_end(ctx, FDR_KERNEL_KNN_DEDUP, st))) return trc;
        return plain(W.inner_bytes);
    }
    ctx->last.unique_targets = nu;
    ctx->last.unique_queries = nuq;
    hipLaunchKernelGGL(gather_unique_rows_kernel, dim3(g16), dim3(256), 0, st, d_That, a.tzero, n, dp,
                       (const int *)W.isrep, (const int *)W.upos, W.U, W.uzero);
    if (nuq != nu)
        hipLaunchKernelGGL(gather_unique_queries_kernel, dim3((unsigned)(((size_t)nu * 16 + 255) / 256)), dim3(256),
                           0, st, (const float *)W.U, (const unsigned char *)W.uzero, nu, dp, (const int *)W.uqflag,
                           (const int *)W.uqpos, W.Uq, W.uqz);
    HIP_TRY(hipGetLastError());
    if ((trc = timing_end(ctx, FDR_KERNEL_KNN_DEDUP, st))) return trc;
    const bool all_q = nuq == nu;
    KnnArgs u = a;
    u.Qhat = all_q ? W.U : W.Uq;
    u.qzero = all_q ? W.uzero : W.uqz;
    u.nq = nuq;
    u.That = W.U;
    u.tzero = W.uzero;
    u.nt = nu;
    u.t_base = 0;
    u.idx = W.idx_u;
    u.dist = W.dist_u;
    u.ws_bytes = W.inner_bytes;
    if ((rc = launch_knn_mode(ctx, u))) return rc;
    if ((trc = timing_begin(ctx, FDR_KERNEL_KNN_DEDUP, st))) return trc;
    const auto &inner = ctx->last.paths;
    if ((rc = launch_expand(W, q0, nq, k, a.t_base, W.uqpos, W.idx_u, W.dist_u, k, a.idx, a.dist,
                            inner.n == nuq ? inner.dev : nullptr, inner.all, W.rowpath, st)))
        return rc;
    ctx->last.paths = {W.rowpath, nq, FDR_PATH_NONE, st};
    return timing_end(ctx, FDR_KERNEL_KNN_DEDUP, st);
}

FDR_EXPORT int fdr_knn_classes_dev(fdr_ctx *ctx, const float *d_That, const uint8_t *d_tzero, int64_t nt, int32_t d,
                                   int32_t k, int64_t nq_max, void *d_ws, size_t ws_bytes, void *stream,
                                   int32_t *n_unique_out) {
    int rc = use_device(ctx);
    if (rc) return rc;
    knn_call_begin(ctx);
    hipStream_t st = (hipStream_t)stream;
    ctx->cls.valid = false;
    if (!n_unique_out) return fail(FDR_E_ARG, "knn_classes: n_unique_out is null");
    *n_unique_out = 0;
    const int dp = fdr_padded_dim(d);
    if (dp < 0 || k < 1 || k > FDR_MAX_K || nt < k || nq_max <= 0 || nq_max > nt || !d_That || !d_tzero || !d_ws ||
        nt > 0x7fffffffll)
        return fail(FDR_E_ARG, "knn_classes: bad argument");
    if (knn_route(dp, k, nt) != FDR_ROUTE_FAST) return FDR_OK;
    if (!knn_dedup_wanted(ctx->dedup_mode, nq_max, nt)) return FDR_OK;
    const DedupWs W = dedup_ws(ws_env(ctx), d_ws, nq_max, nt, d, k);
    if (ws_bytes < W.total) return fail(FDR_E_ARG, "knn_classes: workspace %zu < required %zu bytes", ws_bytes, W.total);
    const int n = (int)nt;
    const unsigned g16 = (unsigned)(((size_t)n * 16 + 255) / 256);
    int trc = timing_begin(ctx, FDR_KERNEL_KNN_DEDUP, st);
    if (trc) return trc;
    hipLaunchKernelGGL(hash_rows_kernel, dim3(g16), dim3(256), 0, st, d_That, n, dp, W.hash, W.idx);
    HIP_TRY(hipGetLastError());
    if ((rc = queue_class_tables(W, d_That, n, dp, st))) return rc;
    int nu = 0;
    HIP_TRY(hipMemcpyAsync(&nu, W.cid + (n - 1), 4, hipMemcpyDeviceToHost, st));
    HIP_TRY(hipStreamSynchronize(st));
    if (!dedup_worth(nu, nu, nt, nt, k, ctx->dedup_mode)) return timing_end(ctx, FDR_KERNEL_KNN_DEDUP, st);
    hipLaunchKernelGGL(gather_unique_rows_kernel, dim3(g16), dim3(256), 0, st, d_That, d_tzero, n, dp,
                       (const int *)W.isrep, (const int *)W.upos, W.U, W.uzero);
    HIP_TRY(hipGetLastError());
    if ((trc = timing_end(ctx, FDR_KERNEL_KNN_DEDUP, st))) return trc;
    ctx->cls.valid = true;
    ctx->cls.That = d_That;
    ctx->cls.tzero = d_tzero;
    ctx->cls.nt = nt;
    ctx->cls.nq_max = nq_max;
    ctx->cls.d = d;
    ctx->cls.k = k;
    ctx->cls.nu = nu;
    ctx->cls.ws = d_ws;
    ctx->cls.ws_bytes = ws_bytes;
    ctx->last.unique_targets = nu;
    *n_unique_out = nu;
    return FDR_OK;
}

static DedupWs classes_ws(const fdr_ctx *ctx) {
    return dedup_ws(ws_env(ctx), ctx->cls.ws, ctx->cls.nq_max, ctx->cls.nt, ctx->cls.d, ctx->cls.k);
}

FDR_EXPORT int fdr_knn_unique_dev(fdr_ctx *ctx, int64_t u_lo, int64_t u_hi, int32_t *d_idx_u, float *d_dist_u,
                                  void *stream) {
    int rc = use_device(ctx);
    if (rc) return rc;
    knn_call_begin(ctx);
    if (!ctx->cls.valid) return fail(FDR_E_STATE, "knn_unique: no classes (call fdr_knn_classes_dev first)");
    if (u_lo < 0 || u_hi < u_lo || u_hi > ctx->cls.nu || u_hi - u_lo > ctx->cls.nq_max)
        return fail(FDR_E_ARG, "knn_unique: bad range [%lld, %lld) of %d unique rows (at most %lld per call)",
                    (long long)u_lo, (long long)u_hi, ctx->cls.nu, (long long)ctx->cls.nq_max);
    if (u_hi == u_lo) return FDR_OK;
    if (!d_idx_u || !d_dist_u) return fail(FDR_E_ARG, "knn_unique: null output");
    const int dp = fdr_padded_dim(ctx->cls.d);
    const DedupWs W = classes_ws(ctx);
    ctx->last.unique_queries = (int)(u_hi - u_lo);
    rc = launch_knn_mode(ctx, KnnArgs{W.U + (size_t)u_lo * dp, W.uzero + u_lo, u_hi - u_lo, W.U, W.uzero, ctx->cls.nu, 0,
                                      ctx->cls.d, ctx->cls.k, d_idx_u, d_dist_u, ctx->cls.ws, W.inner_bytes,
                                      (hipStream_t)stream});
    ctx->last.paths = {};
    return rc;
}

FDR_EXPORT int fdr_knn_expand_dev(fdr_ctx *ctx, int64_t q0, int64_t nq, int64_t t_base, const int32_t *d_idx_u_all,
                                  const float *d_dist_u_all, int64_t u_row_stride, int32_t *d_idx, float *d_dist,
                                  void *stream) {
    int rc = use_device(ctx);
    if (rc) return rc;
    knn_call_begin(ctx);
    if (!ctx->cls.valid) return fail(FDR_E_STATE, "knn_expand: no classes (call fdr_knn_classes_dev first)");
    if (q0 < 0 || nq < 0 || q0 + nq > ctx->cls.nt) return fail(FDR_E_ARG, "knn_expand: bad row range");
    if (nq == 0) return FDR_OK;
    if (!d_idx_u_all || !d_dist_u_all || !d_idx || !d_dist) return fail(FDR_E_ARG, "knn_expand: null pointer");
    hipStream_t st = (hipStream_t)stream;
    const int k = ctx->cls.k;
    if (u_row_stride == 0) u_row_stride = k;
    if (u_row_stride < k || u_row_stride > 0x7fffffffll) return fail(FDR_E_ARG, "knn_expand: bad row stride");
    int trc = timing_begin(ctx, FDR_KERNEL_KNN_DEDUP, st);
    if (trc) return trc;
    if ((rc = launch_expand(classes_ws(ctx), q0, nq, k, t_base, nullptr, d_idx_u_all, d_dist_u_all, u_row_stride, d_idx,
                            d_dist, nullptr, 0, nullptr, st)))
        return rc;
    return timing_end(ctx, FDR_KERNEL_KNN_DEDUP, st);
}

FDR_EXPORT int fdr_embed_dev(fdr_ctx *ctx, int64_t n_rows, const int64_t *d_indptr,
                             const int32_t *d_indices, float *d_E, void *stream) {
    int rc = use_device(ctx);
    if (rc) return rc;
    if (n_rows > 0 && (!d_indptr || !d_E)) return fail(FDR_E_ARG, "embed: null device pointer");
    return launch_embed(ctx, n_rows, d_indptr, d_indices, d_E, (hipStream_t)stream);
}

FDR_EXPORT int fdr_normalize_dev(fdr_ctx *ctx, const float *d_E, int64_t n_rows, int32_t d,
                                 float *d_Ehat, uint8_t *d_zero, void *stream) {
    int rc = use_device(ctx);
    if (rc) return rc;
    if (n_rows > 0 && (!d_E || !d_Ehat || !d_zero)) return fail(FDR_E_ARG, "normalize: null device pointer");
    return launch_normalize(ctx, d_E, n_rows, d, d_Ehat, d_zero, (hipStream_t)stream);
}

FDR_EXPORT int fdr_knn_dev(fdr_ctx *ctx, const float *d_Qhat, const uint8_t *d_qzero, int64_t nq,
                           const float *d_That, const uint8_t *d_tzero, int64_t nt, int64_t t_base,
                           int32_t d, int32_t k, int32_t *d_idx, float *d_dist, void *d_workspace,
                           size_t workspace_bytes, void *stream) {
    int rc = use_device(ctx);
    if (rc) return rc;
    knn_call_begin(ctx);
    if (d_workspace == ctx->cls.ws) ctx->cls.valid = false;
    return launch_knn(ctx, KnnArgs{d_Qhat, d_qzero, nq, d_That, d_tzero, nt, t_base, d, k, d_idx, d_dist, d_workspace,
                                   workspace_bytes, (hipStream_t)stream});
}

static int check_csr(int64_t n_rows, const int64_t *a_indptr, const int32_t *a_indices) {
    if (n_rows < 0 || !a_indptr) return fail(FDR_E_ARG, "embed: bad CSR (n_rows=%lld)", (long long)n_rows);
    if (a_indptr[0] != 0 || a_indptr[n_rows] < 0) return fail(FDR_E_ARG, "embed: bad indptr");
    if (a_indptr[n_rows] > 0 && !a_indices) return fail(FDR_E_ARG, "embed: indices is null");
    return FDR_OK;
}

static int upload_csr(fdr_ctx *ctx, int64_t n_rows, const int64_t *a_indptr,
                      const int32_t *a_indices) {
    int rc;
    const int64_t nnz = a_indptr[n_rows];
    if ((rc = ctx->a_indptr.reserve((size_t)(n_rows + 1) * 8))) return rc;
    if ((rc = ctx->a_indices.reserve((size_t)std::max<int64_t>(nnz, 1) * 4))) return rc;
    HIP_TRY(hipMemcpyAsync(ctx->a_indptr.p, a_indptr, (size_t)(n_rows + 1) * 8, hipMemcpyHostToDevice, ctx->stream));
    if (nnz > 0)
        HIP_TRY(hipMemcpyAsync(ctx->a_indices.p, a_indices, (size_t)nnz * 4, hipMemcpyHostToDevice, ctx->stream));
    return FDR_OK;
}

struct UploadLink {
    fdr_ctx *ctx;
    int64_t n_rows;
    const int64_t *a_indptr;
    const int32_t *a_indices;
    float *d_E;
    int64_t stage_cap;
    int send_raw(int64_t r0, int64_t r1, int slot) {
        hipStream_t st = ctx->stream;
        const int64_t o = a_indptr[r0], len = a_indptr[r1] - o;
        if (len > 0)
            HIP_TRY(hipMemcpyAsync((int32_t *)ctx->a_indices.p + o, a_indices + o, (size_t)len * 4, hipMemcpyHostToDevice, st));
        int erc = launch_embed(ctx, r1 - r0, (const int64_t *)ctx->a_indptr.p + r0, (const int32_t *)ctx->a_indices.p,
                               d_E + (size_t)r0 * ctx->d, st);
        if (erc) return erc;
        if (slot >= 0) HIP_TRY(hipEventRecord(ctx->up_ev[slot], st));
        return FDR_OK;
    }
    int wait_slot(int slot) {
        HIP_TRY(hipEventSynchronize(ctx->up_ev[slot]));
        return FDR_OK;
    }
    int send_staged(int64_t rb, int64_t used) {
        hipStream_t st = ctx->stream;
        const int32_t *stage_ids = (const int32_t *)ctx->stage_ids.p;
        const int64_t *stage_ptr = (const int64_t *)ctx->stage_ptr.p;
        if (used > 0)
            HIP_TRY(hipMemcpyAsync((int32_t *)ctx->c_indices.p + (stage_cap - used), stage_ids + (stage_cap - used),
                                   (size_t)used * 4, hipMemcpyHostToDevice, st));
        HIP_TRY(hipMemcpyAsync((int64_t *)ctx->c_indptr.p + rb, stage_ptr + rb, (size_t)(n_rows - rb + 1) * 8,
                               hipMemcpyHostToDevice, st));
        HIP_TRY(hipEventRecord(ctx->up_ev[2], st));
        return launch_embed(ctx, n_rows - rb, (const int64_t *)ctx->c_indptr.p + rb, (const int32_t *)ctx->c_indices.p,
                            d_E + (size_t)rb * ctx->d, st);
    }
};

static int upload_embed_pipelined(fdr_ctx *ctx, int64_t n_rows, const int64_t *a_indptr, const int32_t *a_indices,
                                  float *d_E) {
    int rc;
    const int64_t nnz = a_indptr[n_rows];
    const hup::Tuning tune;
    if (nnz < tune.min_ids || ctx->h_bits.empty()) {
        if ((rc = upload_csr(ctx, n_rows, a_indptr, a_indices))) return rc;
        return launch_embed(ctx, n_rows, (const int64_t *)ctx->a_indptr.p, (const int32_t *)ctx->a_indices.p, d_E, ctx->stream);
    }
    for (hipEvent_t &e : ctx->up_ev)
        if (!e) HIP_TRY(hipEventCreateWithFlags(&e, hipEventDisableTiming));
    HIP_TRY(hipEventSynchronize(ctx->up_ev[2]));
    const int64_t stage_cap = hup::Tuning::stage_cap(nnz);
    if ((rc = ctx->a_indptr.reserve((size_t)(n_rows + 1) * 8))) return rc;
    if ((rc = ctx->a_indices.reserve((size_t)nnz * 4))) return rc;
    if ((rc = ctx->c_indptr.reserve((size_t)(n_rows + 1) * 8))) return rc;
    if ((rc = ctx->c_indices.reserve((size_t)stage_cap * 4))) return rc;
    if ((rc = ctx->stage_ids.reserve((size_t)stage_cap * 4))) return rc;
    if ((rc = ctx->stage_ptr.reserve((size_t)(n_rows + 1) * 8))) return rc;
    HIP_TRY(hipMemcpyAsync(ctx->a_indptr.p, a_indptr, (size_t)(n_rows + 1) * 8, hipMemcpyHostToDevice, ctx->stream));
    UploadLink link{ctx, n_rows, a_indptr, a_indices, d_E, stage_cap};
    return hup::upload(tune, n_rows, a_indptr, a_indices, ctx->h_bits.data(), (uint64_t)ctx->n_features,
                       (int32_t *)ctx->stage_ids.p, (int64_t *)ctx->stage_ptr.p, stage_cap, ctx->up_pool,
                       hup::Tuning::helpers(host_cpu_budget()), link)
        .rc;
}

FDR_EXPORT int fdr_embed(fdr_ctx *ctx, int64_t n_rows, const int64_t *a_indptr,
                         const int32_t *a_indices, float *E_out) {
    int rc = use_device(ctx);
    if (rc) return rc;
    if ((rc = check_csr(n_rows, a_indptr, a_indices))) return rc;
    if (ctx->n_features <= 0) return fail(FDR_E_STATE, "embed: no projection loaded");
    if (n_rows == 0) return FDR_OK;
    if (!E_out) return fail(FDR_E_ARG, "embed: E_out is null");
    const size_t ebytes = (size_t)n_rows * ctx->d * 4;
    if ((rc = ctx->E.reserve(ebytes))) return rc;
    if ((rc = upload_embed_pipelined(ctx, n_rows, a_indptr, a_indices, (float *)ctx->E.p))) return rc;
    HIP_TRY(hipMemcpyAsync(E_out, ctx->E.p, ebytes, hipMemcpyDeviceToHost, ctx->stream));
    HIP_TRY(hipStreamSynchronize(ctx->stream));
    return FDR_OK;
}

static int knn_from_device_E(fdr_ctx *ctx, const float *d_E, int64_t n, int d, int k,
                             int32_t *idx_out, float *dist_out) {
    int rc;
    const int dp = fdr_padded_dim(d);
    if (dp < 0) return fail(FDR_E_ARG, "knn: dimension %d unsupported (1..%d)", d, FDR_MAX_DIM);
    if (k < 1 || k > FDR_MAX_K) return fail(FDR_E_ARG, "knn: k=%d unsupported (1..%d)", k, FDR_MAX_K);
    if (n < k) return fail(FDR_E_ARG, "knn: need n (%lld) >= k (%d)", (long long)n, k);
    if (!idx_out || !dist_out) return fail(FDR_E_ARG, "knn: null output pointer");
    if ((rc = ctx->Ehat.reserve((size_t)n * dp * 4))) return rc;
    if ((rc = ctx->zero.reserve((size_t)n))) return rc;
    if ((rc = ctx->idx.reserve((size_t)n * k * 4))) return rc;
    if ((rc = ctx->dist.reserve((size_t)n * k * 4))) return rc;
    const size_t wsb = fdr_knn_workspace_bytes(ctx, n, n, d, k);
    if ((rc = ctx->ws.reserve(wsb))) return rc;
    if ((rc = launch_normalize(ctx, d_E, n, d, (float *)ctx->Ehat.p, (uint8_t *)ctx->zero.p, ctx->stream)))
        return rc;
    const float *const Ehat = (const float *)ctx->Ehat.p;
    const uint8_t *const zero = (const uint8_t *)ctx->zero.p;
    const KnnArgs a = {Ehat, zero, n, Ehat, zero, n, 0, d, k, (int32_t *)ctx->idx.p, (float *)ctx->dist.p, ctx->ws.p, wsb, ctx->stream};
    if ((rc = launch_knn(ctx, a))) return rc;
    HIP_TRY(hipMemcpyAsync(idx_out, ctx->idx.p, (size_t)n * k * 4, hipMemcpyDeviceToHost, ctx->stream));
    HIP_TRY(hipMemcpyAsync(dist_out, ctx->dist.p, (size_t)n * k * 4, hipMemcpyDeviceToHost, ctx->stream));
    HIP_TRY(hipStreamSynchronize(ctx->stream));
    return FDR_OK;
}

FDR_EXPORT int fdr_knn(fdr_ctx *ctx, const float *E, int64_t n, int32_t d, int32_t k,
                       int32_t *idx_out, float *dist_out) {
    int rc = use_device(ctx);
    if (rc) return rc;
    knn_call_begin(ctx);
    if (!E || n <= 0) return fail(FDR_E_ARG, "knn: empty input");
    if (fdr_padded_dim(d) < 0) return fail(FDR_E_ARG, "knn: dimension %d unsupported (1..%d)", d, FDR_MAX_DIM);
    if ((rc = ctx->E.reserve((size_t)n * d * 4))) return rc;
    HIP_TRY(hipMemcpyAsync(ctx->E.p, E, (size_t)n * d * 4, hipMemcpyHostToDevice, ctx->stream));
    return knn_from_device_E(ctx, (const float *)ctx->E.p, n, d, k, idx_out, dist_out);
}

FDR_EXPORT int fdr_embed_knn(fdr_ctx *ctx, int64_t n_rows, const int64_t *a_indptr,
                             const int32_t *a_indices, int32_t k, int32_t *idx_out, float *dist_out,
                             float *E_out) {
    int rc = use_device(ctx);
    if (rc) return rc;
    knn_call_begin(ctx);
    if ((rc = check_csr(n_rows, a_indptr, a_indices))) return rc;
    if (ctx->n_features <= 0) return fail(FDR_E_STATE, "embed: no projection loaded");
    if (n_rows <= 0) return fail(FDR_E_ARG, "embed_knn: empty input");
    const size_t ebytes = (size_t)n_rows * ctx->d * 4;
    if ((rc = ctx->E.reserve(ebytes))) return rc;
    if ((rc = upload_embed_pipelined(ctx, n_rows, a_indptr, a_indices, (float *)ctx->E.p))) return rc;
    if (E_out) HIP_TRY(hipMemcpyAsync(E_out, ctx->E.p, ebytes, hipMemcpyDeviceToHost, ctx->stream));
    return knn_from_device_E(ctx, (const float *)ctx->E.p, n_rows, ctx->d, k, idx_out, dist_out);
}

#include "knn_sparse.inc"
#include "knn_radius_common.inc"
#include "knn_sparse_radius.inc"
#include "knn_dense_radius.inc"
#include "topk_merge.inc"
#include "kmer_search.inc"
#include "kmer_output_loader.inc"
#include "reads_parser.inc"
#include "overlaps_writer.inc"
```

### fedrann_amd/csrc/knn_order.inc

```

__global__ __launch_bounds__(256) void row_chunk_keys_kernel(const float *__restrict__ X, int n, int DP,
                                                             u64 *__restrict__ keys, int *__restrict__ vals) {
    const int t = blockIdx.x * 256 + threadIdx.x;
    const int row = t >> 4, sub = t & 15;
    unsigned m = 0;
    if (row < n) {
        const int per = DP / 16;
        const uint4 *p = reinterpret_cast<const uint4 *>(X + (size_t)row * DP + (size_t)sub * per);
        for (int i = 0; i < per / 4; ++i) {
            const uint4 v = p[i];
            const bool nz = ((v.x | v.y | v.z | v.w) & 0x7fffffffu) != 0u;
            if (nz) m |= 1u << ((sub * per + 4 * i) >> 4);
        }
    }
#pragma unroll
    for (int off = 8; off >= 1; off >>= 1) m |= __shfl_xor(m, off);
    if (row < n && sub == 0) {
        keys[row] = ((u64)__popc(m) << 32) | m;
        vals[row] = row;
    }
}

__global__ __launch_bounds__(256) void to_half_ordered_kernel(const float *__restrict__ Ehat,
                                                              const int *__restrict__ perm, long long n_groups,
                                                              int gpr, _Float16 *__restrict__ out) {
    const long long t = (long long)blockIdx.x * 256 + threadIdx.x;
    if (t >= n_groups) return;
    const long long i = t / gpr;
    const int g = (int)(t - i * gpr);
    const f32x4 *src = reinterpret_cast<const f32x4 *>(Ehat) + ((size_t)perm[i] * gpr + g) * 2;
    const f32x4 e = src[0], o = src[1];
    f16x8 h;
    h[0] = (_Float16)e.x; h[1] = (_Float16)o.x; h[2] = (_Float16)e.y; h[3] = (_Float16)o.y;
    h[4] = (_Float16)e.z; h[5] = (_Float16)o.z; h[6] = (_Float16)e.w; h[7] = (_Float16)o.w;
    reinterpret_cast<f16x8 *>(out)[t] = h;
}
```

### fedrann_amd/csrc/knn_prefilter.inc

```
typedef _Float16 f16x8 __attribute__((ext_vector_type(8)));

__device__ __forceinline__ void to_half_group(const float *__restrict__ Ehat, long long t, _Float16 *__restrict__ out,
                                              float (&v)[8]) {
    const f32x4 *src = reinterpret_cast<const f32x4 *>(Ehat) + t * 2;
    const f32x4 e = src[0], o = src[1];
    v[0] = e.x; v[1] = o.x; v[2] = e.y; v[3] = o.y; v[4] = e.z; v[5] = o.z; v[6] = e.w; v[7] = o.w;
    f16x8 h;
#pragma unroll
    for (int i = 0; i < 8; ++i) h[i] = (_Float16)v[i];
    reinterpret_cast<f16x8 *>(out)[t] = h;
}
__global__ __launch_bounds__(256) void to_half_kernel(const float *__restrict__ Ehat, long long n_groups,
                                                      _Float16 *__restrict__ out) {
    const long long t = (long long)blockIdx.x * 256 + threadIdx.x;
    if (t >= n_groups) return;
    float v[8];
    to_half_group(Ehat, t, out, v);
}

__global__ __launch_bounds__(256) void to_half_compact_kernel(const float *__restrict__ Ehat, long long n_groups,
                                                              _Float16 *__restrict__ out, unsigned char *__restrict__ rc,
                                                              int *__restrict__ n_long) {
    __shared__ int wg_long;
    if (threadIdx.x == 0) wg_long = 0;
    __syncthreads();
    const long long t = (long long)blockIdx.x * 256 + threadIdx.x;
    const bool live = t < n_groups;
    float v[8] = {0.f, 0.f, 0.f, 0.f, 0.f, 0.f, 0.f, 0.f};
    if (live) to_half_group(Ehat, t, out, v);
    const int g = (int)(t & 15);
    unsigned nzm = 0;
#pragma unroll
    for (int i = 0; i < 8; ++i) nzm |= (unsigned)((__float_as_uint(v[i]) & 0x7fffffffu) != 0u) << i;
    const int mine = __popc(nzm);
    int incl = mine;
#pragma unroll
    for (int off = 1; off < 16; off <<= 1) {
        const int below = __shfl_up(incl, off, 16);
        if (g >= off) incl += below;
    }
    const int total = __shfl(incl, 15, 16);
    if (live) {
        unsigned char *rec = rc + (size_t)(t >> 4) * RC_BYTES;
        if (g == 0) rec[0] = (unsigned char)total;
        if (total <= RC_ENTRIES) {
            int e = incl - mine;
#pragma unroll
            for (int i = 0; i < 8; ++i) {
                if ((nzm >> i) & 1u) {
                    unsigned char *hf = rec + 64 * (e / RC_HALF_ENTRIES);
                    const int s = e % RC_HALF_ENTRIES;
                    hf[1 + s] = (unsigned char)(8 * g + (i & 1) * 4 + (i >> 1));
                    reinterpret_cast<float *>(hf + 16)[s] = v[i];
                    ++e;
                }
            }
        }
    }
    const u64 lm = __ballot(live && g == 0 && total > RC_ENTRIES);
    if ((threadIdx.x & 63) == 0 && lm) atomicAdd(&wg_long, __popcll(lm));
    __syncthreads();
    if (threadIdx.x == 0 && wg_long) atomicAdd(n_long, wg_long);
}

template <int OFF>
__device__ __forceinline__ void lds_read128(f16x8 &dst, unsigned addr, std::integral_constant<int, OFF>) {
    static_assert(OFF >= 0 && OFF < 65536, "ds_read offset is 16 bits");
    asm volatile("ds_read_b128 %0, %1 offset:%2" : "=v"(dst) : "v"(addr), "n"(OFF));
}

template <int N>
__device__ __forceinline__ void wait_lgkmcnt(f16x8 &frag) {
    static_assert(N >= 0 && N <= 6, "count out of range");
    if constexpr (N == 0) asm volatile("s_waitcnt lgkmcnt(0)" : "+v"(frag));
    else if constexpr (N == 1) asm volatile("s_waitcnt lgkmcnt(1)" : "+v"(frag));
    else if constexpr (N == 2) asm volatile("s_waitcnt lgkmcnt(2)" : "+v"(frag));
    else if constexpr (N == 3) asm volatile("s_waitcnt lgkmcnt(3)" : "+v"(frag));
    else if constexpr (N == 4) asm volatile("s_waitcnt lgkmcnt(4)" : "+v"(frag));
    else if constexpr (N == 5) asm volatile("s_waitcnt lgkmcnt(5)" : "+v"(frag));
    else asm volatile("s_waitcnt lgkmcnt(6)" : "+v"(frag));
}

template <int... S, class F>
__device__ __forceinline__ void static_for(std::integer_sequence<int, S...>, F &&f) {
    (f(std::integral_constant<int, S>{}), ...);
}

template <int N>
__device__ __forceinline__ void wait_vmcnt() {
    static_assert(N >= 0 && N <= 16, "count out of range");
    if constexpr (N == 0) asm volatile("s_waitcnt vmcnt(0)" ::: "memory");
    else if constexpr (N == 1) asm volatile("s_waitcnt vmcnt(1)" ::: "memory");
    else if constexpr (N == 2) asm volatile("s_waitcnt vmcnt(2)" ::: "memory");
    else if constexpr (N == 3) asm volatile("s_waitcnt vmcnt(3)" ::: "memory");
    else if constexpr (N == 4) asm volatile("s_waitcnt vmcnt(4)" ::: "memory");
    else if constexpr (N == 6) asm volatile("s_waitcnt vmcnt(6)" ::: "memory");
    else if constexpr (N == 8) asm volatile("s_waitcnt vmcnt(8)" ::: "memory");
    else if constexpr (N == 12) asm volatile("s_waitcnt vmcnt(12)" ::: "memory");
    else if constexpr (N == 16) asm volatile("s_waitcnt vmcnt(16)" ::: "memory");
    else static_assert(N == 0, "add the literal form for this count");
}

#define PK_EMPTY 0xffffffffu
#ifdef FDR_STAMPS
__device__ unsigned long long g_stamps[16][8];
#define STAMP(v) const unsigned v = (unsigned)__builtin_readcyclecounter()
#define STAMP_ADD(ph, a, b) do { if (stamp_on) stamp_acc[ph] += (b) - (a); } while (0)
#else
#define STAMP(v) do { } while (0)
#define STAMP_ADD(ph, a, b) do { } while (0)
#endif
constexpr int FDR_SHARE_EVERY = 63;


__device__ __forceinline__ void fragment_addresses(unsigned (&fa)[8], const unsigned char *ring_base, int j, int h) {
    const unsigned ring = (unsigned)(size_t)(__attribute__((address_space(3))) const unsigned char *)ring_base;
#pragma unroll
    for (int s8 = 0; s8 < 8; ++s8) {
        fa[s8] = ring + (unsigned)(j * 256 + (((2 * s8 + h) ^ (j & 15)) * 16));
        asm volatile("" : "+v"(fa[s8]));
    }
}

__device__ __forceinline__ unsigned partner32(unsigned x, int h) {
    const auto r = __builtin_amdgcn_permlane32_swap(x, x, false, false);
    return h ? r[0] : r[1];
}

template <int LH>
struct RegList {
    unsigned v[LH];
    unsigned pmax;
};

template <int LH>
__device__ __forceinline__ unsigned reglist_round(RegList<LH> &L, unsigned cand, int h) {
    const unsigned c = min(cand, partner32(cand, h));
    const unsigned mymax = L.v[LH - 1];
    const bool hold = mymax > L.pmax || (mymax == L.pmax && h == 0);
    const unsigned ce = (hold && c < mymax) ? c : PK_EMPTY;
#pragma unroll
    for (int e = LH - 1; e >= 1; --e) L.v[e] = max(min(L.v[e - 1], ce), min(max(L.v[e - 1], ce), L.v[e]));
    L.v[0] = min(L.v[0], ce);
    L.pmax = partner32(L.v[LH - 1], h);
    return c;
}

struct OrderArgs {
    const int *perm_t;
    const int *perm_q;
};

template <int DP, int NQ, int NW, int WPS, int U, int LH, bool PAIRED = false>
__global__ __launch_bounds__(64 * NW, WPS) void knn_prefilter_kernel(
    const _Float16 *__restrict__ Qh, int nq, const _Float16 *__restrict__ Th, int nt, int t_base,
    SegBounds segs, int K, int nq_pad, u64 *__restrict__ partial, unsigned *__restrict__ tau_shared,
    int ib, int item_base, int nqb, OrderArgs ord FDR_DBG_PARAM) {
#ifndef FDR_DEV
    constexpr int dbg = 0;
#endif
    extern __shared__ __attribute__((aligned(16))) unsigned char smem[];
    constexpr int QW = 32 * NQ * NW;
    constexpr int NCH = DP / 128;
    const int item = item_base + (int)blockIdx.x;
    const int seg = item / nqb, qb = item - seg * nqb;
    constexpr int UNIT_BYTES = 32 * 256;
    constexpr int STAGE_BYTES = U * UNIT_BYTES;
    constexpr int ROW_BYTES = DP * 2;
    static_assert(NCH % U == 0 || U % NCH == 0, "a stage holds whole tiles or a tile spans whole stages");
    static_assert(NCH <= 2 * U, "a tile spans at most two stages (the loop is unrolled by stage parity)");

    const int tid = threadIdx.x;
    const int lane = tid & 63;
    const int wave = __builtin_amdgcn_readfirstlane(tid >> 6);
    const int j = lane & 31, h = lane >> 5;
    const int ql0 = wave * 32 * NQ + j;
    const int qg0 = qb * QW + ql0;

    f16x8 b[NQ][NCH * 8];
#pragma unroll
    for (int n = 0; n < NQ; ++n) {
        const int qg = qg0 + 32 * n;
        const f16x8 *qp = reinterpret_cast<const f16x8 *>(Qh + (size_t)(qg < nq ? qg : nq - 1) * DP);
#pragma unroll
        for (int i = 0; i < NCH * 8; ++i) b[n][i] = qp[2 * i + h];
    }
    const int qbits = min(20, 32 - ib);
    const unsigned QM1 = (1u << qbits) - 2u;
    const float qscale = (float)QM1, qinv = 1.0f / qscale;
    const int nlive = (K - h + 1) >> 1, dead = LH - nlive;
    RegList<LH> L[NQ];
    unsigned flim[NQ];
    int cthr[NQ];
#pragma unroll
    for (int n = 0; n < NQ; ++n) {
#pragma unroll
        for (int e = 0; e < LH; ++e) L[n].v[e] = e < dead ? 0u : PK_EMPTY;
        L[n].pmax = PK_EMPTY;
    }
    auto share = [&](RegList<LH> &Ln, unsigned &fl, int n) {
        unsigned *slot = tau_shared + qg0 + 32 * n;
        const unsigned tk = max(Ln.v[LH - 1], Ln.pmax);
        const unsigned mine = tk == PK_EMPTY ? 0x7F800000u : (tk >> ib);
        unsigned seen = mine;
        if (h == 0) {
            const unsigned old = mine <= QM1
                                     ? __hip_atomic_fetch_min(slot, mine, __ATOMIC_RELAXED, __HIP_MEMORY_SCOPE_AGENT)
                                     : __hip_atomic_load(slot, __ATOMIC_RELAXED, __HIP_MEMORY_SCOPE_AGENT);
            seen = min(old, mine);
        }
        const unsigned ps = partner32(seen, h);
        fl = min(h ? ps : seen, QM1 + 1);
    };
    auto rethreshold = [&](const RegList<LH> &Ln, unsigned fl) -> int {
        const unsigned tk = max(Ln.v[LH - 1], Ln.pmax);
        const unsigned oq = tk >> ib;
        const unsigned lim = tk == PK_EMPTY ? fl : min(oq - 1u, fl);
        int th = lim >= QM1 ? (int)0x80000000u : __float_as_int(((float)(QM1 - lim) - 0.75f) * qinv) + 1;
        if (tk != PK_EMPTY && oq == 0u) th = 0x7fffffff;
        return th;
    };
#pragma unroll
    for (int n = 0; n < NQ; ++n) {
        share(L[n], flim[n], n);
        cthr[n] = rethreshold(L[n], flim[n]);
        if (dbg & 16) cthr[n] = 0x7fffffff;
    }

    const int t_begin = segs.b[seg];
    const int t_end = min(nt, segs.b[seg + 1]);
    const int ntiles = (t_end - t_begin + 31) >> 5;
    const int nunits = ntiles * NCH;
    const int nstages = (nunits + U - 1) / U;

    constexpr int PPW = 8 * U / NW;
    static_assert((8 * U) % NW == 0, "unsupported wave count");
    const char *seg_base = reinterpret_cast<const char *>(Th + (size_t)t_begin * DP);
    const unsigned last_row_off = (unsigned)(t_end - 1 - t_begin) * ROW_BYTES;
    constexpr bool ONEPAIR = NW == 8 && NCH <= U;
    constexpr int NOFF = ONEPAIR ? 1 : PPW;
    unsigned soff[NOFF];
    unsigned scol[NOFF];
#pragma unroll
    for (int u = 0; u < NOFF; ++u) {
        const int piece = wave + NW * u;
        const int row = 4 * (piece & 7) + (lane >> 4), pslot = lane & 15;
        scol[u] = (unsigned)((pslot ^ (row & 15)) * 16 + ((piece >> 3) % NCH) * 256);
        soff[u] = (unsigned)(32 * ((piece >> 3) / NCH) + row) * ROW_BYTES;
    }
    auto issue_stage = [&](auto par_c) {
        constexpr int par = decltype(par_c)::value;
        unsigned char *dst = smem + par * STAGE_BYTES;
        if constexpr (ONEPAIR) {
            static_for(std::make_integer_sequence<int, PPW>{}, [&](auto u_c) {
                constexpr int u = decltype(u_c)::value;
                constexpr unsigned row_c = (unsigned)(32 * (u / NCH)) * ROW_BYTES, col_c = (unsigned)((u % NCH) * 256);
                unsigned vrow = soff[0];
                asm volatile("" : "+v"(vrow));
                const unsigned off = min(vrow + row_c, last_row_off) + scol[0] + col_c;
                __builtin_amdgcn_global_load_lds((const __attribute__((address_space(1))) void *)(seg_base + off),
                                                 (__attribute__((address_space(3))) void *)(dst + (wave + NW * u) * 1024),
                                                 16, 0, 0);
            });
            soff[0] += (unsigned)(32 * (U / NCH)) * ROW_BYTES;
        } else {
#pragma unroll
            for (int u = 0; u < PPW; ++u) {
                const int piece = wave + NW * u;
                const unsigned off = min(soff[u], last_row_off) + scol[u] + (NCH > U ? par * U * 256 : 0);
                __builtin_amdgcn_global_load_lds((const __attribute__((address_space(1))) void *)(seg_base + off),
                                                 (__attribute__((address_space(3))) void *)(dst + piece * 1024),
                                                 16, 0, 0);
                if constexpr (NCH <= U) soff[u] += (unsigned)(32 * (U / NCH)) * ROW_BYTES;
                else if constexpr (par == 1) soff[u] += (unsigned)32 * ROW_BYTES;
            }
        }
    };
    if (nstages > 0) issue_stage(std::integral_constant<int, 0>{});
    __syncthreads();

    unsigned q0[NQ], q1[NQ];
#pragma unroll
    for (int n = 0; n < NQ; ++n) q0[n] = q1[n] = PK_EMPTY;
    auto flush = [&](RegList<LH> &Ln, unsigned &a0, unsigned &a1) {
        const bool dbgc = (dbg & 2) != 0;
        while (__any(a0 != PK_EMPTY)) {
            DBG_COUNT(4);
            const unsigned took = reglist_round<LH>(Ln, a0, h);
            if (a0 == took) {
                a0 = a1;
                a1 = PK_EMPTY;
            }
        }
    };
    auto offer = [&](const f32x16 &a, const int (&g)[4], RegList<LH> &Ln, unsigned &a0, unsigned &a1,
                     const unsigned fl, const int th, int lrow, int nvalid) {
        const bool dbgc = (dbg & 2) != 0;
        DBG_COUNT(1);
#pragma unroll
        for (int q4 = 0; q4 < 4; ++q4) {
            if (!__any(g[q4] >= th)) continue;
            DBG_COUNT(2);
#pragma unroll
            for (int r = 4 * q4; r < 4 * q4 + 4; ++r) {
                const int roff = (r & 3) + 8 * (r >> 2);
                const bool pass = __float_as_int(a[r]) >= th && roff + 4 * h < nvalid;
                if (!__any(pass)) continue;
                unsigned cand = PK_EMPTY;
                if (pass) {
                    const float sc = fminf(fmaxf(a[r], 0.0f), 1.0f);
                    const unsigned qd = QM1 - (unsigned)__builtin_rintf(sc * qscale);
                    if (qd <= fl) cand = (qd << ib) | (unsigned)(lrow + roff);
                }
                DBG_COUNT(3);
                if (__any(cand != PK_EMPTY && a1 != PK_EMPTY)) flush(Ln, a0, a1);
                a1 = (a0 != PK_EMPTY && a1 == PK_EMPTY) ? cand : a1;
                a0 = a0 == PK_EMPTY ? cand : a0;
            }
        }
    };
    typedef const f16x8 __attribute__((address_space(3))) lds_f16x8;
    unsigned fa[8];
    fragment_addresses(fa, smem, j, h);

    f32x16 acc[NQ];
#pragma unroll
    for (int n = 0; n < NQ; ++n)
#pragma unroll
        for (int r = 0; r < 16; ++r) acc[n][r] = 0.f;

    auto score = [&](const f32x16 &av, int n, int t) __attribute__((always_inline)) {
        int g[4];
#pragma unroll
        for (int q4 = 0; q4 < 4; ++q4)
            g[q4] = max(max(max(__float_as_int(av[4 * q4]), __float_as_int(av[4 * q4 + 1])),
                            __float_as_int(av[4 * q4 + 2])),
                        __float_as_int(av[4 * q4 + 3]));
        const int mx = max(max(max(g[0], g[1]), g[2]), g[3]);
        const bool dbgc = (dbg & 2) != 0;
        DBG_COUNT(0);
        if (dbg & 1) {
            if (mx == 0x7fffffff) cthr[n] = mx;
        } else if (__any(mx >= cthr[n])) {
            int lrow = t * 32 + 4 * h;
            int nvalid = t_end - (t_begin + t * 32);
            asm volatile("" : "+v"(lrow), "+s"(nvalid));
            offer(av, g, L[n], q0[n], q1[n], flim[n], cthr[n], lrow, nvalid);
            cthr[n] = rethreshold(L[n], flim[n]);
        }
    };
    constexpr bool PAIR = PAIRED && NCH == 1 && (U == 2 || U == 4) && NQ == 1;
    constexpr int NP = U / 2;
    constexpr bool STAGGER = PAIR && NW == 8;
    const bool late = STAGGER && wave >= NW / 2;
    f32x16 accB;
#pragma unroll
    for (int r = 0; r < 16; ++r) accB[r] = 0.f;
#ifdef FDR_STAMPS
    unsigned stamp_acc[6] = {0, 0, 0, 0, 0, 0};
    const bool stamp_on = blockIdx.x == 0;
#endif
    auto stage_body = [&](auto par_c, int it) {
        constexpr int par = decltype(par_c)::value;
        STAMP(ts0);
        if (it + 1 < nstages) issue_stage(std::integral_constant<int, par ^ 1>{});
        STAMP(ts1);
        STAMP_ADD(0, ts0, ts1);
        if constexpr (PAIR) {
            auto mfma_pair = [&](auto p_c) __attribute__((always_inline)) {
                constexpr int OFF0 = par * STAGE_BYTES + 2 * decltype(p_c)::value * UNIT_BYTES, OFF1 = OFF0 + UNIT_BYTES;
                f16x8 fa0[2], fa1[2];
                lds_read128(fa0[0], fa[0], std::integral_constant<int, OFF0>{});
                lds_read128(fa1[0], fa[0], std::integral_constant<int, OFF1>{});
#pragma unroll
                for (int s8 = 0; s8 < 8; ++s8) {
                    if (s8 < 7) {
                        lds_read128(fa0[(s8 + 1) & 1], fa[s8 + 1], std::integral_constant<int, OFF0>{});
                        lds_read128(fa1[(s8 + 1) & 1], fa[s8 + 1], std::integral_constant<int, OFF1>{});
                        asm volatile("s_waitcnt lgkmcnt(2)" : "+v"(fa0[s8 & 1]), "+v"(fa1[s8 & 1]));
                    } else {
                        asm volatile("s_waitcnt lgkmcnt(0)" : "+v"(fa0[s8 & 1]), "+v"(fa1[s8 & 1]));
                    }
                    __builtin_amdgcn_sched_barrier(0);
                    acc[0] = __builtin_amdgcn_mfma_f32_32x32x16_f16(fa0[s8 & 1], b[0][s8], s8 == 0 ? f32x16{} : acc[0], 0, 0, 0);
                    accB = __builtin_amdgcn_mfma_f32_32x32x16_f16(fa1[s8 & 1], b[0][s8], s8 == 0 ? f32x16{} : accB, 0, 0, 0);
                    __builtin_amdgcn_sched_barrier(0);
                }
            };
            auto score_pair = [&](const int ts) __attribute__((always_inline)) {
                score(acc[0], 0, ts);
                if (ts + 1 < nunits) score(accB, 0, ts + 1);
            };
            if constexpr (STAGGER) {
                if (late && it > 0 && U * it - 2 < nunits) score_pair(U * it - 2);
                if (it < nstages) {
                    static_for(std::make_integer_sequence<int, NP>{}, [&](auto p_c) {
                        constexpr int p = decltype(p_c)::value;
                        const int tp = U * it + 2 * p;
                        if (tp < nunits) {
                            mfma_pair(p_c);
                            if (!late || p < NP - 1) score_pair(tp);
                        }
                    });
                }
            } else {
                static_for(std::make_integer_sequence<int, NP>{}, [&](auto p_c) {
                    const int tp = U * it + 2 * decltype(p_c)::value;
                    if (tp < nunits) {
                        mfma_pair(p_c);
                        score_pair(tp);
                    }
                });
            }
        } else {
        constexpr bool DEEP = WPS <= 2 || (WPS == 3 && DP == 256 && LH == 16);
        if (DEEP && U * (it + 1) <= nunits) {
            if constexpr (DEEP) {
                constexpr int KS = 8 * U, D = WPS <= 2 ? 4 : 2, R = D + 1;
                f16x8 fr[R];
                constexpr bool FAR = STAGE_BYTES * 2 > 65536;
                unsigned fb[8];
#pragma unroll
                for (int i = 0; i < 8; ++i) fb[i] = FAR ? fa[i] + (unsigned)(par * STAGE_BYTES) : fa[i];
                auto rd = [&](auto s_c) __attribute__((always_inline)) {
                    constexpr int s = decltype(s_c)::value;
                    lds_read128(fr[s % R], fb[s % 8],
                                std::integral_constant<int, (FAR ? 0 : par * STAGE_BYTES) + (s / 8) * UNIT_BYTES>{});
                };
                static_for(std::make_integer_sequence<int, D>{}, rd);
                auto kstep = [&](auto s_c) __attribute__((always_inline)) {
                    constexpr int s = decltype(s_c)::value;
                    constexpr int uu = s / 8, s8 = s % 8;
                    constexpr int c = NCH <= U ? uu % NCH : (U * par + uu) % NCH;
                    if constexpr (s + D < KS) rd(std::integral_constant<int, s + D>{});
                    wait_lgkmcnt<(KS - 1 - s < D ? KS - 1 - s : D)>(fr[s % R]);
                    __builtin_amdgcn_sched_barrier(0);
#pragma unroll
                    for (int n = 0; n < NQ; ++n)
                        acc[n] = __builtin_amdgcn_mfma_f32_32x32x16_f16(fr[s % R], b[n][c * 8 + s8],
                                                                        (c == 0 && s8 == 0) ? f32x16{} : acc[n], 0, 0, 0);
                    __builtin_amdgcn_sched_barrier(0);
                    if constexpr (s8 == 7 && c == NCH - 1) {
                        const int t = (U * it + uu) / NCH;
#pragma unroll
                        for (int n = 0; n < NQ; ++n) score(acc[n], n, t);
                    }
                };
                static_for(std::make_integer_sequence<int, KS>{}, kstep);
            }
        } else {
#pragma unroll
        for (int uu = 0; uu < U; ++uu) {
            const int c = NCH <= U ? uu % NCH : (U * par + uu) % NCH;
            const int unit = U * it + uu;
            if (unit < nunits) {
                const int t = unit / NCH;
                if (c == 0) {
#pragma unroll
                    for (int n = 0; n < NQ; ++n)
#pragma unroll
                        for (int r = 0; r < 16; ++r) acc[n][r] = 0.f;
                }
                if constexpr (WPS <= 2) {
                    f16x8 a[8];
#pragma unroll
                    for (int s8 = 0; s8 < 8; ++s8)
                        a[s8] = *(lds_f16x8 *)(size_t)(fa[s8] + (unsigned)(par * STAGE_BYTES + uu * UNIT_BYTES));
                    __builtin_amdgcn_sched_barrier(0);
#pragma unroll
                    for (int s8 = 0; s8 < 8; ++s8)
#pragma unroll
                        for (int n = 0; n < NQ; ++n)
                            acc[n] = __builtin_amdgcn_mfma_f32_32x32x16_f16(a[s8], b[n][c * 8 + s8], acc[n], 0, 0, 0);
                } else {
#pragma unroll
                    for (int s8 = 0; s8 < 8; ++s8) {
                        const f16x8 a = *(lds_f16x8 *)(size_t)(fa[s8] + (unsigned)(par * STAGE_BYTES + uu * UNIT_BYTES));
#pragma unroll
                        for (int n = 0; n < NQ; ++n)
                            acc[n] = __builtin_amdgcn_mfma_f32_32x32x16_f16(a, b[n][c * 8 + s8], acc[n], 0, 0, 0);
                    }
                }
                if (c == NCH - 1) {
#pragma unroll
                    for (int n = 0; n < NQ; ++n) score(acc[n], n, t);
                }
            }
        }
        }
        }
        STAMP(ts2);
        STAMP_ADD(1, ts1, ts2);
        if ((it & FDR_SHARE_EVERY) == FDR_SHARE_EVERY) {
#pragma unroll
            for (int n = 0; n < NQ; ++n) {
                flush(L[n], q0[n], q1[n]);
                share(L[n], flim[n], n);
                cthr[n] = rethreshold(L[n], flim[n]);
                if (dbg & 16) cthr[n] = 0x7fffffff;
            }
        }
        STAMP(ts3);
        STAMP_ADD(2, ts2, ts3);
#ifdef FDR_STAMPS
        asm volatile("s_waitcnt vmcnt(0)" ::: "memory");
        STAMP(ts3b);
        STAMP_ADD(3, ts3, ts3b);
        __syncthreads();
        STAMP(ts4);
        STAMP_ADD(4, ts3b, ts4);
        if (stamp_on) stamp_acc[5] += 1;
#else
        __syncthreads();
#endif
    };
    const int niter = nstages + (STAGGER ? 1 : 0);
    for (int it0 = 0; it0 < niter; it0 += 2) {
        stage_body(std::integral_constant<int, 0>{}, it0);
        if (it0 + 1 < niter) stage_body(std::integral_constant<int, 1>{}, it0 + 1);
    }
#ifdef FDR_STAMPS
    if (stamp_on && lane == 0)
        for (int ph = 0; ph < 6; ++ph) atomicAdd(&g_stamps[wave][ph], (unsigned long long)stamp_acc[ph]);
#endif
    const unsigned imask = (1u << ib) - 1u;
#pragma unroll
    for (int n = 0; n < NQ; ++n) {
        flush(L[n], q0[n], q1[n]);
        size_t qrow = (size_t)qb * QW + ql0 + 32 * n;
        if (ord.perm_q) {
            if (qrow >= (size_t)nq) continue;
            qrow = (size_t)ord.perm_q[qrow];
        }
        u64 *out = partial + ((size_t)seg * nq_pad + qrow) * K + (h ? (K + 1) >> 1 : 0);
#pragma unroll
        for (int e = 0; e < LH; ++e) {
            if (e >= dead) {
                const unsigned kv = L[n].v[e];
                u64 o = KEY_INF;
                if (kv != PK_EMPTY) {
                    int trow = t_begin + (int)(kv & imask);
                    if (ord.perm_t) trow = ord.perm_t[trow];
                    o = ((u64)__float_as_uint((float)(kv >> ib) / qscale) << 32) | (unsigned)(t_base + trow);
                }
                out[e - dead] = o;
            }
        }
    }
}

template <int J>
__device__ __forceinline__ unsigned lane_xor(unsigned v, const int lane) {
    static_assert(J == 1 || J == 2 || J == 4 || J == 8 || J == 16 || J == 32, "a power of two below 64");
    if constexpr (J == 1) {
        return (unsigned)__builtin_amdgcn_update_dpp(0, (int)v, 0xB1, 0xF, 0xF, true);
    } else if constexpr (J == 2) {
        return (unsigned)__builtin_amdgcn_update_dpp(0, (int)v, 0x4E, 0xF, 0xF, true);
    } else if constexpr (J == 4) {
        const int up = __builtin_amdgcn_update_dpp(0, (int)v, 0x104, 0xF, 0xF, true);
        const int dn = __builtin_amdgcn_update_dpp(0, (int)v, 0x114, 0xF, 0xF, true);
        return (unsigned)((lane & 4) ? dn : up);
    } else if constexpr (J == 8) {
        return (unsigned)__builtin_amdgcn_update_dpp(0, (int)v, 0x128, 0xF, 0xF, true);
    } else if constexpr (J == 16) {
        const auto r = __builtin_amdgcn_permlane16_swap(v, v, false, false);
        return (lane & 16) ? r[0] : r[1];
    } else {
        const auto r = __builtin_amdgcn_permlane32_swap(v, v, false, false);
        return (lane & 32) ? r[0] : r[1];
    }
}
template <int J>
__device__ __forceinline__ u64 lane_xor64(u64 v, const int lane) {
    return ((u64)lane_xor<J>((unsigned)(v >> 32), lane) << 32) | lane_xor<J>((unsigned)v, lane);
}

template <int KMIN, int KMAX>
__device__ __forceinline__ u64 wave_bitonic(u64 key, const int lane) {
    static_for(std::integer_sequence<int, 2, 4, 8, 16, 32, 64>{}, [&](auto kc) {
        constexpr int k = decltype(kc)::value;
        if constexpr (k >= KMIN && k <= KMAX) {
            static_for(std::make_integer_sequence<int, 6>{}, [&](auto sc) {
                constexpr int j = (k >> 1) >> decltype(sc)::value;
                if constexpr (j > 0) {
                    const u64 other = lane_xor64<j>(key, lane);
                    const bool up = k == KMAX || (lane & k) == 0;
                    const bool take_min = ((lane & j) == 0) == up;
                    key = (take_min == (other < key)) ? other : key;
                }
            });
        }
    });
    return key;
}
__device__ __forceinline__ u64 wave_sort64(u64 key, const int lane) { return wave_bitonic<2, 64>(key, lane); }
__device__ __forceinline__ u64 wave_sort32(u64 key, const int lane) { return wave_bitonic<2, 32>(key, lane); }

__device__ __forceinline__ void wave_sort128(u64 &a, u64 &b, const int lane) {
    static_for(std::integer_sequence<int, 2, 4, 8, 16, 32, 64, 128>{}, [&](auto kc) {
        constexpr int k = decltype(kc)::value;
        static_for(std::make_integer_sequence<int, 7>{}, [&](auto sc) {
            constexpr int j = (k >> 1) >> decltype(sc)::value;
            if constexpr (j == 64) {
                const u64 lo = a < b ? a : b, hi = a < b ? b : a;
                a = lo;
                b = hi;
            } else if constexpr (j > 0) {
                const u64 oa = lane_xor64<j>(a, lane), ob = lane_xor64<j>(b, lane);
                const bool up_a = k >= 64 || (lane & k) == 0;
                const bool up_b = k == 128 || (k < 64 && (lane & k) == 0);
                const bool lower = (lane & j) == 0;
                a = ((lower == up_a) == (oa < a)) ? oa : a;
                b = ((lower == up_b) == (ob < b)) ? ob : b;
            }
        });
    });
}

#define MERGE_QPW 4
#define MERGE_ADAPTIVE_FROM 8
__device__ __forceinline__ u64 lane_reverse64(u64 v, const int lane) {
    u64 r = v;
    r = lane_xor64<1>(r, lane);
    r = lane_xor64<2>(r, lane);
    r = lane_xor64<4>(r, lane);
    r = lane_xor64<8>(r, lane);
    r = lane_xor64<16>(r, lane);
    r = lane_xor64<32>(r, lane);
    return r;
}
__global__ __launch_bounds__(256) void knn_merge_keys_kernel(const u64 *__restrict__ partial, int nseg,
                                                             int nq, int nq_pad, int KP,
                                                             u64 *__restrict__ cand) {
    __shared__ u64 stage[4][MERGE_CAP];
    static_assert(MERGE_CAP >= 256, "a wave's stage row doubles as its survivor buffer (256 keys)");
    const int lane = threadIdx.x & 63, wave = threadIdx.x >> 6;
    const int M = nseg * KP;
    if (M <= 64) {
        const int q0 = (blockIdx.x * 4 + wave) * MERGE_QPW;
        const bool runs16 = KP == 32;
        const int sg = lane / KP;
        const int e = runs16 && (lane & 16) ? (lane & 16) + 15 - (lane & 15) : lane - sg * KP;
        u64 kv[MERGE_QPW];
#pragma unroll
        for (int t = 0; t < MERGE_QPW; ++t)
            kv[t] = (lane < M && q0 + t < nq) ? partial[((size_t)sg * nq_pad + q0 + t) * KP + e] : KEY_INF;
        if (runs16) {
#pragma unroll
            for (int t = 0; t < MERGE_QPW; ++t) kv[t] = wave_bitonic<32, 64>(kv[t], lane);
        } else {
#pragma unroll
            for (int t = 0; t < MERGE_QPW; ++t) kv[t] = wave_sort64(kv[t], lane);
        }
#pragma unroll
        for (int t = 0; t < MERGE_QPW; ++t)
            if (lane < KP && q0 + t < nq) cand[(size_t)(q0 + t) * KP + lane] = kv[t];
        return;
    }
    u64 *sv = stage[wave];
    const int q = blockIdx.x * 4 + wave;
    if (q >= nq) return;
    if (nseg > MERGE_ADAPTIVE_FROM) {
        u64 best = KEY_INF, bound = KEY_INF;
        int pc = 0;
        auto merge64 = [&]() {
            const u64 srt = wave_sort64(sv[lane], lane);
            const u64 rev = lane_reverse64(srt, lane);
            best = wave_bitonic<64, 64>(rev < best ? rev : best, lane);
            bound = __shfl(best, KP - 1);
            const u64 tail = sv[64 + lane];
            __builtin_amdgcn_fence(__ATOMIC_RELEASE, "wavefront");
            __builtin_amdgcn_wave_barrier();
            sv[lane] = tail;
            __builtin_amdgcn_fence(__ATOMIC_RELEASE, "wavefront");
            __builtin_amdgcn_wave_barrier();
            __builtin_amdgcn_fence(__ATOMIC_ACQUIRE, "wavefront");
        };
        u64 kvs[8];
        for (int sg0 = 0; sg0 < nseg; sg0 += 8) {
#pragma unroll
            for (int i = 0; i < 8; ++i)
                kvs[i] = (lane < KP && sg0 + i < nseg) ? partial[((size_t)(sg0 + i) * nq_pad + q) * KP + lane] : KEY_INF;
#pragma unroll
            for (int i = 0; i < 8; ++i) {
                const u64 kv = kvs[i];
                const bool keep = kv < KEY_INF && kv <= bound;
                const u64 mask = __ballot(keep);
                if (mask == 0ull) continue;
                if (keep) sv[pc + __popcll(mask & ((1ull << lane) - 1ull))] = kv;
                pc += __popcll(mask);
                __builtin_amdgcn_fence(__ATOMIC_RELEASE, "wavefront");
                __builtin_amdgcn_wave_barrier();
                __builtin_amdgcn_fence(__ATOMIC_ACQUIRE, "wavefront");
                if (pc >= 64) {
                    if (pc < 128 && lane >= pc - 64) sv[64 + lane] = KEY_INF;
                    __builtin_amdgcn_fence(__ATOMIC_RELEASE, "wavefront");
                    __builtin_amdgcn_wave_barrier();
                    __builtin_amdgcn_fence(__ATOMIC_ACQUIRE, "wavefront");
                    merge64();
                    pc -= 64;
                }
            }
        }
        if (pc > 0) {
            if (lane >= pc) sv[lane] = KEY_INF;
            sv[64 + lane] = KEY_INF;
            __builtin_amdgcn_fence(__ATOMIC_RELEASE, "wavefront");
            __builtin_amdgcn_wave_barrier();
            __builtin_amdgcn_fence(__ATOMIC_ACQUIRE, "wavefront");
            merge64();
        }
        if (lane < KP) cand[(size_t)q * KP + lane] = best;
        return;
    }
    {
        u64 kvs[8];
        auto load_batch = [&](int sg0) {
#pragma unroll
            for (int i = 0; i < 8; ++i)
                kvs[i] = (lane < KP && sg0 + i < nseg) ? partial[((size_t)(sg0 + i) * nq_pad + q) * KP + lane]
                                                       : KEY_INF;
        };
        load_batch(0);
        u64 bound = KEY_INF;
        for (int sg = lane; sg < nseg; sg += 64) {
            const u64 *l = partial + ((size_t)sg * nq_pad + q) * KP;
            const u64 a = l[((KP + 1) >> 1) - 1], b2 = l[KP - 1];
            if (a != KEY_INF && b2 != KEY_INF) {
                const u64 m = (a > b2 ? a : b2) | 0xffffffffull;
                bound = m < bound ? m : bound;
            }
        }
#pragma unroll
        for (int off = 32; off >= 1; off >>= 1) {
            const u64 o = __shfl_xor(bound, off);
            bound = o < bound ? o : bound;
        }
        int total = 0;
        if (bound != KEY_INF) {
            for (int sg0 = 0;;) {
#pragma unroll
                for (int i = 0; i < 8; ++i) {
                    const u64 kv = kvs[i];
                    const bool keep = kv <= bound;
                    const u64 mask = __ballot(keep);
                    const int pos = total + __popcll(mask & ((1ull << lane) - 1ull));
                    if (keep && pos < 256) sv[pos] = kv;
                    total += __popcll(mask);
                }
                sg0 += 8;
                if (sg0 >= nseg) break;
                load_batch(sg0);
            }
        }
        if (bound != KEY_INF && total <= 256) {
            if (total <= 64) {
                const u64 kv = wave_sort64(lane < total ? sv[lane] : KEY_INF, lane);
                if (lane < KP) cand[(size_t)q * KP + lane] = kv;
                return;
            }
            u64 ka = sv[lane];
            u64 kb = 64 + lane < total ? sv[64 + lane] : KEY_INF;
            wave_sort128(ka, kb, lane);
            bool done = total <= 128;
            if (!done) {
                const u64 b2 = __shfl(ka, KP - 1);
                const u64 e0 = 128 + lane < total ? sv[128 + lane] : KEY_INF;
                const u64 e1 = 192 + lane < total ? sv[192 + lane] : KEY_INF;
                const bool k0 = e0 <= b2, k1 = e1 <= b2;
                const u64 m0 = __ballot(k0), m1 = __ballot(k1);
                const int n0 = __popcll(m0), nx = n0 + __popcll(m1);
                if (KP + nx <= 128) {
                    const u64 below = (1ull << lane) - 1ull;
                    if (lane < KP) sv[lane] = ka;
                    if (k0) sv[KP + __popcll(m0 & below)] = e0;
                    if (k1) sv[KP + n0 + __popcll(m1 & below)] = e1;
                    ka = lane < KP + nx ? sv[lane] : KEY_INF;
                    kb = 64 + lane < KP + nx ? sv[64 + lane] : KEY_INF;
                    wave_sort128(ka, kb, lane);
                    done = true;
                }
            }
            if (done) {
                if (lane < KP) cand[(size_t)q * KP + lane] = ka;
                return;
            }
        }
    }
    const bool staged = M <= MERGE_CAP;
    u64 *mine_lds = stage[wave];
    auto key_at = [&](int m) -> u64 {
        const int seg = m / KP, e = m - seg * KP;
        return partial[((size_t)seg * nq_pad + q) * KP + e];
    };
    if (staged)
        for (int m = lane; m < M; m += 64) mine_lds[m] = key_at(m);
    u64 prev1 = 0, mine = KEY_INF;
    for (int r = 0; r < KP; ++r) {
        u64 best = ~0ull;
        for (int m = lane; m < M; m += 64) {
            u64 kv;
            kv = staged ? mine_lds[m] : key_at(m);
            if (kv + 1 > prev1 && kv < best) best = kv;
        }
#pragma unroll
        for (int off = 32; off >= 1; off >>= 1) {
            const u64 o = __shfl_xor(best, off);
            best = o < best ? o : best;
        }
        if (best >= KEY_INF) best = KEY_INF; else prev1 = best + 1;
        if (lane == r) mine = best;
    }
    if (lane < KP) cand[(size_t)q * KP + lane] = mine;
}

#define RERANK_ROWS_DENSE 32
#define RERANK_ROWS_COMPACT 16
#define RERANK_STRIDE 132
#define RERANK_WAVE_FLOATS(ROWS) ((ROWS) * RERANK_STRIDE + ((ROWS) == RERANK_ROWS_COMPACT ? RC_DP : 0))
#define RERANK_LDS_BYTES(ROWS) (4 * RERANK_WAVE_FLOATS(ROWS) * 4)
template <int ROWS>
__global__ __launch_bounds__(256) void knn_rerank_kernel(
    const u64 *__restrict__ cand, int KP, int K, const float *__restrict__ Qhat,
    const unsigned char *__restrict__ qzero, const float *__restrict__ That, int nq, int DP, int t_base,
    float margin, int *__restrict__ idx_out, float *__restrict__ dist_out, int *__restrict__ counter,
    int *__restrict__ flagged, int *__restrict__ range_list, float *__restrict__ theta,
    unsigned char *__restrict__ path,
    const unsigned char *__restrict__ rc,
    int long_limit) {
    extern __shared__ float rerank_rows[];
    const int lane = threadIdx.x & 63;
    const int wave = __builtin_amdgcn_readfirstlane((int)(threadIdx.x >> 6));
    float *rows = rerank_rows + wave * RERANK_WAVE_FLOATS(ROWS);
    const int q = blockIdx.x * 4 + wave;
    if (q >= nq) return;
    if (qzero[q]) {
        if (lane == 0) {
            flagged[nq - 1 - atomicAdd(counter + 1, 1)] = q;
            path[q] = FDR_PATH_ZERO;
        }
        return;
    }
    u64 key = KEY_INF;
    if (lane < KP) key = cand[(size_t)q * KP + lane];
    const float dt = __uint_as_float((unsigned)(key >> 32));
    const float dK = __shfl(dt, K - 1), dKP = __shfl(dt, KP - 1);
    const bool valid = (dK + margin < 1.0f) && (dK + margin < dKP);
    if (!valid) {
        if (lane == 0) {
            if (range_list && dK + margin < 1.0f) {
                range_list[atomicAdd(counter + 2, 1)] = q;
                theta[q] = dK + margin;
                path[q] = FDR_PATH_RANGE;
            } else {
                flagged[atomicAdd(counter, 1)] = q;
                path[q] = FDR_PATH_EXACT;
            }
        }
        return;
    }
    if (lane == 0) path[q] = FDR_PATH_CERTIFIED;
    const bool need = lane < KP && key < KEY_INF && dt <= dK + margin;
    const int tidx = (int)(unsigned)(key & 0xffffffffull);
    u64 densemask = __ballot(need);
    const int half = lane >> 5, l5 = lane & 31;
    float c = 0.0f;
    if (ROWS == RERANK_ROWS_COMPACT && rc && counter[8] <= long_limit) {
        float *qs = rows + ROWS * RERANK_STRIDE;
        reinterpret_cast<float2 *>(qs)[lane] = reinterpret_cast<const float2 *>(Qhat + (size_t)q * RC_DP)[lane];
        __builtin_amdgcn_fence(__ATOMIC_RELEASE, "wavefront");
        __builtin_amdgcn_wave_barrier();
        __builtin_amdgcn_fence(__ATOMIC_ACQUIRE, "wavefront");
        const uint4 *rec = reinterpret_cast<const uint4 *>(rc + (size_t)(need ? tidx - t_base : 0) * RC_BYTES);
        int mine = 0;
        int most = 0;
#pragma unroll
        for (int h = 0; h < RC_HALVES; ++h) {
            if (h > 0 && most <= RC_HALF_ENTRIES * h) continue;
            const bool live = h == 0 ? need : mine > RC_HALF_ENTRIES * h;
            unsigned w[16] = {};
            if (live) {
#pragma unroll
                for (int i = 0; i < 4; ++i) {
                    const uint4 x = rec[4 * h + i];
                    w[4 * i] = x.x; w[4 * i + 1] = x.y; w[4 * i + 2] = x.z; w[4 * i + 3] = x.w;
                }
            }
            if (h == 0) {
                const int cnt = (int)(w[0] & 0xffu);
                mine = cnt <= RC_ENTRIES ? cnt : 0;
                densemask = __ballot(need && cnt > RC_ENTRIES);
                static_assert(RC_ENTRIES < 32, "the largest count is found over five bits");
#pragma unroll
                for (int bit = 4; bit >= 0; --bit)
                    if (__ballot((mine >> bit) == ((most >> bit) | 1))) most |= 1 << bit;
            }
#pragma unroll
            for (int e = 0; e < RC_HALF_ENTRIES; ++e) {
                if (RC_HALF_ENTRIES * h + e < most) {
                    const int pos = (int)((w[(1 + e) >> 2] >> (8 * ((1 + e) & 3))) & (RC_DP - 1));
                    if (RC_HALF_ENTRIES * h + e < mine) c = __builtin_fmaf(qs[pos], __uint_as_float(w[4 + e]), c);
                }
            }
        }
    }
    for (int b = 0; b * ROWS < KP; ++b) {
        const unsigned bm = (unsigned)(densemask >> (ROWS * b)) & (unsigned)((1ull << ROWS) - 1ull);
        if (!bm) continue;
        int trow[ROWS / 2];
#pragma unroll
        for (int it = 0; it < ROWS / 2; ++it) trow[it] = __shfl(tidx, ROWS * b + 2 * it + half) - t_base;
        for (int ch = 0; ch < DP / 128; ++ch) {
            f32x4 v[ROWS / 2];
#pragma unroll
            for (int it = 0; it < ROWS / 2; ++it) {
                v[it] = f32x4{0.0f, 0.0f, 0.0f, 0.0f};
                if ((bm >> (2 * it + half)) & 1u)
                    v[it] = *reinterpret_cast<const f32x4 *>(That + (size_t)trow[it] * DP + ch * 128 + l5 * 4);
            }
#pragma unroll
            for (int it = 0; it < ROWS / 2; ++it)
                *reinterpret_cast<f32x4 *>(rows + (2 * it + half) * RERANK_STRIDE + l5 * 4) = v[it];
            __builtin_amdgcn_fence(__ATOMIC_RELEASE, "wavefront");
            __builtin_amdgcn_wave_barrier();
            __builtin_amdgcn_fence(__ATOMIC_ACQUIRE, "wavefront");
            if (lane / ROWS == b && ((densemask >> lane) & 1ull)) {
                const f32x4 *tp = reinterpret_cast<const f32x4 *>(rows + (lane % ROWS) * RERANK_STRIDE);
                const f32x4 *qp = reinterpret_cast<const f32x4 *>(Qhat + (size_t)q * DP + ch * 128);
#pragma unroll
                for (int g = 0; g < 16; ++g) {
                    const f32x4 te = tp[2 * g], to = tp[2 * g + 1];
                    const f32x4 qe = qp[2 * g], qo = qp[2 * g + 1];
                    c = __builtin_fmaf(qe.x, te.x, c);
                    c = __builtin_fmaf(qo.x, to.x, c);
                    c = __builtin_fmaf(qe.y, te.y, c);
                    c = __builtin_fmaf(qo.y, to.y, c);
                    c = __builtin_fmaf(qe.z, te.z, c);
                    c = __builtin_fmaf(qo.z, to.z, c);
                    c = __builtin_fmaf(qe.w, te.w, c);
                    c = __builtin_fmaf(qo.w, to.w, c);
                }
            }
            __builtin_amdgcn_fence(__ATOMIC_RELEASE, "wavefront");
            __builtin_amdgcn_wave_barrier();
        }
    }
    u64 exact = ~0ull;
    if (need) exact = ((u64)__float_as_uint(dist_from_sim(c)) << 32) | (unsigned)tidx;
    const u64 mine = KP <= 32 ? wave_sort32(exact, lane) : wave_sort64(exact, lane);
    if (lane < K) {
        idx_out[(size_t)q * K + lane] = (int)(unsigned)(mine & 0xffffffffull);
        dist_out[(size_t)q * K + lane] = __uint_as_float((unsigned)(mine >> 32));
    }
}

#define RANGE_STAGES 4
#define RANGE_LANE_BUF 8

struct RangeOut {
// ... 313 lines not shown
```

### fedrann_amd/csrc/knn_prefilter_live.inc

```

__global__ __launch_bounds__(64) void live_block_masks_kernel(const u64 *__restrict__ keys_s, int nq,
                                                              unsigned *__restrict__ masks) {
    const int b = blockIdx.x, lane = threadIdx.x;
    unsigned m = 0;
#pragma unroll
    for (int i = 0; i < 4; ++i) {
        const int r = b * 256 + i * 64 + lane;
        if (r < nq) m |= (unsigned)keys_s[r] & 0xffu;
    }
#pragma unroll
    for (int off = 32; off >= 1; off >>= 1) m |= __shfl_xor(m, off);
    if (lane == 0) masks[b] = m;
}

__global__ __launch_bounds__(64) void live_stage_masks_kernel(const u64 *__restrict__ keys_s, int nt, SegBounds segs,
                                                              uint8_t *__restrict__ smask) {
    const int seg = blockIdx.y, stage = blockIdx.x, lane = threadIdx.x;
    const int t_begin = segs.b[seg], t_end = min(nt, segs.b[seg + 1]);
    const int r0 = t_begin + stage * 128;
    if (r0 >= t_end) return;
    unsigned m = 0;
#pragma unroll
    for (int i = 0; i < 2; ++i) {
        const int r = r0 + i * 64 + lane;
        if (r < t_end) m |= (unsigned)keys_s[r] & 0xffu;
    }
#pragma unroll
    for (int off = 32; off >= 1; off >>= 1) m |= __shfl_xor(m, off);
    if (lane == 0) smask[live_stage_row(t_begin, seg) + stage] = (uint8_t)m;
}

__global__ __launch_bounds__(64) void live_stage_lists_kernel(const uint8_t *__restrict__ smask, int nt, SegBounds segs,
                                                              int all, uint16_t *__restrict__ lists,
                                                              int *__restrict__ lens) {
    const int seg = blockIdx.y, lane = threadIdx.x;
    const unsigned v = blockIdx.x;
    const int t_begin = segs.b[seg], t_end = min(nt, segs.b[seg + 1]);
    const int nstages = t_end > t_begin ? (t_end - t_begin + 127) >> 7 : 0;
    const size_t row = (size_t)live_stage_row(t_begin, seg);
    const uint8_t *sm = smask + row;
    uint16_t *out = lists + row * 256 + (size_t)v * live_list_stride(nstages);
    int count = 0;
    for (int s0 = 0; s0 < nstages; s0 += 64) {
        const int s = s0 + lane;
        const bool keep = s < nstages && (s == 0 || all != 0 || (sm[s] & v) != 0u);
        const unsigned long long kept = __ballot(keep);
        if (keep) out[count + __popcll(kept & ((1ull << lane) - 1ull))] = (uint16_t)s;
        count += __popcll(kept);
    }
    if (lane == 0) lens[seg * 256 + (int)v] = count;
}

__global__ __launch_bounds__(256) void to_half_blocked_kernel(const float *__restrict__ Ehat,
                                                              const int *__restrict__ perm, int n, long long n_groups,
                                                              _Float16 *__restrict__ out) {
    const long long t = (long long)blockIdx.x * 256 + threadIdx.x;
    if (t >= n_groups) return;
    const long long i = t >> 4;
    const int g = (int)(t & 15);
    f16x8 h;
#pragma unroll
    for (int e = 0; e < 8; ++e) h[e] = (_Float16)0.0f;
    if (i < n) {
        const f32x4 *src = reinterpret_cast<const f32x4 *>(Ehat) + ((size_t)perm[i] * 16 + g) * 2;
        const f32x4 e = src[0], o = src[1];
        h[0] = (_Float16)e.x; h[1] = (_Float16)o.x; h[2] = (_Float16)e.y; h[3] = (_Float16)o.y;
        h[4] = (_Float16)e.z; h[5] = (_Float16)o.z; h[6] = (_Float16)e.w; h[7] = (_Float16)o.w;
    }
    const size_t slot = ((((size_t)(i >> 5) * 8 + (size_t)(g >> 1)) * 32 + (size_t)(i & 31)) << 1) + (size_t)(g & 1);
    reinterpret_cast<f16x8 *>(out)[slot] = h;
}

__global__ __launch_bounds__(256) void live_gather_dense_kernel(const _Float16 *__restrict__ hq, const int *__restrict__ perm_q,
                                                                const unsigned *__restrict__ tau, int nq,
                                                                const int *__restrict__ blocks, _Float16 *__restrict__ out_q,
                                                                int *__restrict__ out_perm, unsigned *__restrict__ out_tau) {
    const int b = blocks[blockIdx.x];
    const int sub = threadIdx.x & 15;
    for (int r = threadIdx.x >> 4; r < 256; r += 16) {
        const int src = b * 256 + r, dst = blockIdx.x * 256 + r;
        if (src >= nq) {
            if (sub == 0) out_tau[dst] = 0x7F800000u;
            continue;
        }
        reinterpret_cast<f16x8 *>(out_q)[(size_t)dst * 16 + sub] = reinterpret_cast<const f16x8 *>(hq)[(size_t)src * 16 + sub];
        if (sub == 0) {
            out_perm[dst] = perm_q[src];
            out_tau[dst] = tau[src];
        }
    }
}

template <int NL>
__global__ __launch_bounds__(512, 4) void knn_prefilter_live_kernel(
    const _Float16 *__restrict__ Qh, int nq, const _Float16 *__restrict__ Tb, int nt, int t_base, SegBounds segs, int K,
    int nq_pad, u64 *__restrict__ partial, unsigned *__restrict__ tau_shared, int ib, int item_base, int nb,
    const int *__restrict__ blocks, const unsigned *__restrict__ live_ids, OrderArgs ord,
    const unsigned *__restrict__ masks, const unsigned *__restrict__ lists, const int *__restrict__ lens) {
    static_assert(NL >= FDR_LIVE_MIN_NL && NL <= FDR_LIVE_MAX_NL, "instances NL = 2 .. 6");
    extern __shared__ __attribute__((aligned(16))) unsigned char smem[];
    constexpr int DP = 128, NW = 8, U = 4, LH = 16, QW = 32 * NW;
    constexpr int TILE_BYTES = 8 * 1024;
    constexpr int UNIT_BYTES = NL * 1024;
    constexpr int STAGE_BYTES = U * UNIT_BYTES;
    constexpr int NPIECE = U * NL;
    constexpr int PPW = (NPIECE + NW - 1) / NW;
    const int item = item_base + (int)blockIdx.x;
    const int seg = item / nb;
    const int qb = __builtin_amdgcn_readfirstlane(blocks[item - seg * nb]);
    const unsigned ids = __builtin_amdgcn_readfirstlane(live_ids[qb]);
    const unsigned bmask = __builtin_amdgcn_readfirstlane(masks[qb]) & 0xffu;

    const int tid = threadIdx.x;
    const int lane = tid & 63;
    const int wave = __builtin_amdgcn_readfirstlane(tid >> 6);
    const int j = lane & 31, h = lane >> 5;
    const int ql0 = wave * 32 + j;
    const int qg0 = qb * QW + ql0;

    f16x8 b[NL];
    {
        const f16x8 *qp = reinterpret_cast<const f16x8 *>(Qh + (size_t)(qg0 < nq ? qg0 : nq - 1) * DP);
#pragma unroll
        for (int s = 0; s < NL; ++s) b[s] = qp[2 * (int)((ids >> (4 * s)) & 7u) + h];
    }
    const int qbits = min(20, 32 - ib);
    const unsigned QM1 = (1u << qbits) - 2u;
    const float qscale = (float)QM1, qinv = 1.0f / qscale;
    const int nlive = (K - h + 1) >> 1, dead = LH - nlive;
    RegList<LH> L;
    unsigned flim;
    int cthr;
#pragma unroll
    for (int e = 0; e < LH; ++e) L.v[e] = e < dead ? 0u : PK_EMPTY;
    L.pmax = PK_EMPTY;
    auto share = [&](RegList<LH> &Ln, unsigned &fl) {
        unsigned *slot = tau_shared + qg0;
        const unsigned tk = max(Ln.v[LH - 1], Ln.pmax);
        const unsigned mine = tk == PK_EMPTY ? 0x7F800000u : (tk >> ib);
        unsigned seen = mine;
        if (h == 0) {
            const unsigned old = mine <= QM1
                                     ? __hip_atomic_fetch_min(slot, mine, __ATOMIC_RELAXED, __HIP_MEMORY_SCOPE_AGENT)
                                     : __hip_atomic_load(slot, __ATOMIC_RELAXED, __HIP_MEMORY_SCOPE_AGENT);
            seen = min(old, mine);
        }
        const unsigned ps = partner32(seen, h);
        fl = min(h ? ps : seen, QM1 + 1);
    };
    auto rethreshold = [&](const RegList<LH> &Ln, unsigned fl) -> int {
        const unsigned tk = max(Ln.v[LH - 1], Ln.pmax);
        const unsigned oq = tk >> ib;
        const unsigned lim = tk == PK_EMPTY ? fl : min(oq - 1u, fl);
        int th = lim >= QM1 ? (int)0x80000000u : __float_as_int(((float)(QM1 - lim) - 0.75f) * qinv) + 1;
        if (tk != PK_EMPTY && oq == 0u) th = 0x7fffffff;
        return th;
    };
    share(L, flim);
    cthr = rethreshold(L, flim);

    const int t_begin = segs.b[seg];
    const int t_end = min(nt, segs.b[seg + 1]);
    const int nunits = (t_end - t_begin + 31) >> 5;
    const int nstages = (nunits + U - 1) / U;
    const int nlist = nstages > 0 ? min(lens[seg * 256 + (int)bmask], nstages) : 0;
    const unsigned *list = lists + (((size_t)live_stage_row(t_begin, seg) * 256 + (size_t)bmask * live_list_stride(nstages)) >> 1);
    auto entry = [&](int i) -> int {
        const int e = max(min(i, nlist - 1), 0);
        const unsigned w = __builtin_amdgcn_readfirstlane(list[e >> 1]);
        return min((int)((w >> (16 * (e & 1))) & 0xffffu), max(nstages - 1, 0));
    };

    const char *seg_base = reinterpret_cast<const char *>(Tb) + (size_t)(t_begin >> 5) * TILE_BYTES;
    unsigned poff[PPW];
#pragma unroll
    for (int u = 0; u < PPW; ++u) {
        const int p = min(wave + NW * u, NPIECE - 1);
        const int tl = p / NL, s = p - tl * NL;
        poff[u] = (unsigned)(tl * TILE_BYTES) + ((ids >> (4 * s)) & 7u) * 1024u;
    }
    const unsigned soff = (unsigned)((lane & 31) * 32 + (lane >> 5) * 16);
    auto issue_stage = [&](auto par_c, int sn) {
        const unsigned stoff = (unsigned)sn * (unsigned)(U * TILE_BYTES);
        constexpr int par = decltype(par_c)::value;
        unsigned char *dst = smem + par * STAGE_BYTES;
        static_for(std::make_integer_sequence<int, PPW>{}, [&](auto u_c) {
            constexpr int u = decltype(u_c)::value;
            if (NW * (u + 1) <= NPIECE || wave < NPIECE - NW * u)
                __builtin_amdgcn_global_load_lds((const __attribute__((address_space(1))) void *)(seg_base + (soff + (poff[u] + stoff))),
                                                 (__attribute__((address_space(3))) void *)(dst + (wave + NW * u) * 1024),
                                                 16, 0, 0);
        });
    };
    int sprev = 0, scur = entry(0), snext = entry(1);
    if (nlist > 0) issue_stage(std::integral_constant<int, 0>{}, scur);
    __syncthreads();

    unsigned q0 = PK_EMPTY, q1 = PK_EMPTY;
    auto flush = [&](RegList<LH> &Ln, unsigned &a0, unsigned &a1) {
        while (__any(a0 != PK_EMPTY)) {
            const unsigned took = reglist_round<LH>(Ln, a0, h);
            if (a0 == took) {
                a0 = a1;
                a1 = PK_EMPTY;
            }
        }
    };
    auto offer = [&](const f32x16 &a, const int (&g)[4], RegList<LH> &Ln, unsigned &a0, unsigned &a1,
                     const unsigned fl, const int th, int lrow, int nvalid) {
#pragma unroll
        for (int q4 = 0; q4 < 4; ++q4) {
            if (!__any(g[q4] >= th)) continue;
#pragma unroll
            for (int r = 4 * q4; r < 4 * q4 + 4; ++r) {
                const int roff = (r & 3) + 8 * (r >> 2);
                const bool pass = __float_as_int(a[r]) >= th && roff + 4 * h < nvalid;
                if (!__any(pass)) continue;
                unsigned cand = PK_EMPTY;
                if (pass) {
                    const float sc = fminf(fmaxf(a[r], 0.0f), 1.0f);
                    const unsigned qd = QM1 - (unsigned)__builtin_rintf(sc * qscale);
                    if (qd <= fl) cand = (qd << ib) | (unsigned)(lrow + roff);
                }
                if (__any(cand != PK_EMPTY && a1 != PK_EMPTY)) flush(Ln, a0, a1);
                a1 = (a0 != PK_EMPTY && a1 == PK_EMPTY) ? cand : a1;
                a0 = a0 == PK_EMPTY ? cand : a0;
            }
        }
    };
    unsigned fa = (unsigned)(size_t)(__attribute__((address_space(3))) const unsigned char *)smem + (unsigned)lane * 16u;
    asm volatile("" : "+v"(fa));

    f32x16 acc, accB;
#pragma unroll
    for (int r = 0; r < 16; ++r) acc[r] = accB[r] = 0.f;

    auto score = [&](const f32x16 &av, int t) __attribute__((always_inline)) {
        int g[4];
#pragma unroll
        for (int q4 = 0; q4 < 4; ++q4)
            g[q4] = max(max(max(__float_as_int(av[4 * q4]), __float_as_int(av[4 * q4 + 1])),
                            __float_as_int(av[4 * q4 + 2])),
                        __float_as_int(av[4 * q4 + 3]));
        const int mx = max(max(max(g[0], g[1]), g[2]), g[3]);
        if (__any(mx >= cthr)) {
            int lrow = t * 32 + 4 * h;
            int nvalid = t_end - (t_begin + t * 32);
            asm volatile("" : "+v"(lrow), "+s"(nvalid));
            offer(av, g, L, q0, q1, flim, cthr, lrow, nvalid);
            cthr = rethreshold(L, flim);
        }
    };
    constexpr int NP = U / 2;
    const bool late = wave >= NW / 2;
#ifdef FDR_STAMPS
    unsigned stamp_acc[6] = {0, 0, 0, 0, 0, 0};
    const bool stamp_on = blockIdx.x == 0;
#endif
    auto stage_body = [&](auto par_c, int it) {
        constexpr int par = decltype(par_c)::value;
        STAMP(ts0);
        const int safter = entry(it + 2);
        if (it + 1 < nlist) issue_stage(std::integral_constant<int, par ^ 1>{}, snext);
        STAMP(ts1);
        STAMP_ADD(0, ts0, ts1);
        auto mfma_pair = [&](auto p_c) __attribute__((always_inline)) {
            constexpr int OFF0 = par * STAGE_BYTES + 2 * decltype(p_c)::value * UNIT_BYTES, OFF1 = OFF0 + UNIT_BYTES;
            f16x8 fa0[2], fa1[2];
            lds_read128(fa0[0], fa, std::integral_constant<int, OFF0>{});
            lds_read128(fa1[0], fa, std::integral_constant<int, OFF1>{});
            static_for(std::make_integer_sequence<int, NL>{}, [&](auto s_c) {
                constexpr int s = decltype(s_c)::value;
                if constexpr (s < NL - 1) {
                    lds_read128(fa0[(s + 1) & 1], fa, std::integral_constant<int, OFF0 + (s + 1) * 1024>{});
                    lds_read128(fa1[(s + 1) & 1], fa, std::integral_constant<int, OFF1 + (s + 1) * 1024>{});
                    asm volatile("s_waitcnt lgkmcnt(2)" : "+v"(fa0[s & 1]), "+v"(fa1[s & 1]));
                } else {
                    asm volatile("s_waitcnt lgkmcnt(0)" : "+v"(fa0[s & 1]), "+v"(fa1[s & 1]));
                }
                __builtin_amdgcn_sched_barrier(0);
                acc = __builtin_amdgcn_mfma_f32_32x32x16_f16(fa0[s & 1], b[s], s == 0 ? f32x16{} : acc, 0, 0, 0);
                accB = __builtin_amdgcn_mfma_f32_32x32x16_f16(fa1[s & 1], b[s], s == 0 ? f32x16{} : accB, 0, 0, 0);
                __builtin_amdgcn_sched_barrier(0);
            });
        };
        auto score_pair = [&](const int ts) __attribute__((always_inline)) {
            score(acc, ts);
            if (ts + 1 < nunits) score(accB, ts + 1);
        };
        if (late && it > 0 && U * sprev + U - 2 < nunits) score_pair(U * sprev + U - 2);
        if (it < nlist) {
            static_for(std::make_integer_sequence<int, NP>{}, [&](auto p_c) {
                constexpr int p = decltype(p_c)::value;
                const int tp = U * scur + 2 * p;
                if (tp < nunits) {
                    mfma_pair(p_c);
                    if (!late || p < NP - 1) score_pair(tp);
                }
            });
        }
        STAMP(ts2);
        STAMP_ADD(1, ts1, ts2);
        if ((it & FDR_SHARE_EVERY) == FDR_SHARE_EVERY) {
            flush(L, q0, q1);
            share(L, flim);
            cthr = rethreshold(L, flim);
        }
        STAMP(ts3);
        STAMP_ADD(2, ts2, ts3);
#ifdef FDR_STAMPS
        asm volatile("s_waitcnt vmcnt(0)" ::: "memory");
        STAMP(ts3b);
        STAMP_ADD(3, ts3, ts3b);
        __syncthreads();
        STAMP(ts4);
        STAMP_ADD(4, ts3b, ts4);
        if (stamp_on) stamp_acc[5] += 1;
#else
        __syncthreads();
#endif
        sprev = scur;
        scur = snext;
        snext = safter;
    };
    const int niter = nlist + 1;
    for (int it0 = 0; it0 < niter; it0 += 2) {
        stage_body(std::integral_constant<int, 0>{}, it0);
        if (it0 + 1 < niter) stage_body(std::integral_constant<int, 1>{}, it0 + 1);
    }
#ifdef FDR_STAMPS
    if (stamp_on && lane == 0)
        for (int ph = 0; ph < 6; ++ph) atomicAdd(&g_stamps[wave][ph], (unsigned long long)stamp_acc[ph]);
#endif
    const unsigned imask = (1u << ib) - 1u;
    flush(L, q0, q1);
    size_t qrow = (size_t)qb * QW + ql0;
    if (qrow >= (size_t)nq) return;
    qrow = (size_t)ord.perm_q[qrow];
    u64 *out = partial + ((size_t)seg * nq_pad + qrow) * K + (h ? (K + 1) >> 1 : 0);
#pragma unroll
    for (int e = 0; e < LH; ++e) {
        if (e >= dead) {
            const unsigned kv = L.v[e];
            u64 o = KEY_INF;
            if (kv != PK_EMPTY) {
                const int trow = ord.perm_t[t_begin + (int)(kv & imask)];
                o = ((u64)__float_as_uint((float)(kv >> ib) / qscale) << 32) | (unsigned)(t_base + trow);
            }
            out[e - dead] = o;
        }
    }
}

typedef void (*LiveKernel)(const _Float16 *, int, const _Float16 *, int, int, SegBounds, int, int, u64 *, unsigned *, int,
                           int, int, const int *, const unsigned *, OrderArgs, const unsigned *, const unsigned *,
                           const int *);
static constexpr LiveKernel kLiveKernels[FDR_LIVE_MAX_NL - FDR_LIVE_MIN_NL + 1] = {
    knn_prefilter_live_kernel<2>, knn_prefilter_live_kernel<3>, knn_prefilter_live_kernel<4>,
    knn_prefilter_live_kernel<5>, knn_prefilter_live_kernel<6>};
static size_t live_lds_bytes(int nl) { return (size_t)2 * 4 * nl * 1024; }
```

Baseline: 285.5 million.

## Cut host syncs and redundant conversions in the KNN prefilter setup

Several unrelated changes land together. Device-to-host scalar and mask reads now go into a reusable pinned buffer with event-based waits, replacing pageable copies and stream syncs, and the host-to-device uploads of the live plan no longer block. The ordered and blocked fp16 layouts are gathered from the already-converted half table instead of reconverting from fp32, and the two live-path copies are fused into one kernel. The compact conversion kernel also emits the sort keys directly, hipFuncSetAttribute calls are cached per kernel, and a new merge path handles KP=32 with few segments. This adds pinned-memory lifetime and ordering risks, since the pinned buffer is reused across async copies.

```diff
diff --git a/devtools/trace_gaps.py b/devtools/trace_gaps.py
--- /dev/null
+++ b/devtools/trace_gaps.py
@@ -0,0 +1,121 @@
+#!/usr/bin/env python
+import argparse
+import collections
+import csv
+import json
+import re
+
+
+def short(name):
+    name = re.sub(r"\s*\[clone .*$", "", name)
+    m = re.match(r"_Z(\d+)", name)
+    if m:
+        end = m.end() + int(m.group(1))
+        ints = re.match(r"I((?:Li\d+E)+)E", name[end:])
+        args = re.findall(r"Li(\d+)E", ints.group(1)) if ints else []
+        return name[m.end():end] + ("<%s>" % ",".join(args) if 0 < len(args) <= 3 else "<..>" if name[end:end + 1] == "I" else "")
+    out, args, depth = [], [], 0
+    for ch in name:
+        if ch == "<":
+            depth += 1
+            if depth == 1:
+                args = []
+                continue
+        elif ch == ">" and depth > 0:
+            depth -= 1
+            if depth == 0:
+                a = "".join(args).replace(" ", "")
+                out.append("<%s>" % (a if len(a) <= 10 else ".."))
+                continue
+        elif ch == "(" and depth == 0:
+            break
+        (args if depth else out).append(ch)
+    words = "".join(out).split()
+    return words[-1] if words else name
+
+
+def load(path):
+    rows = []
+    for r in csv.DictReader(open(path)):
+        rows.append((int(r["Start_Timestamp"]), int(r["End_Timestamp"]), short(r["Kernel_Name"])))
+    rows.sort()
+    return rows
+
+
+def steps_of(rows, step_kernel, skip):
+    cuts = [i for i, r in enumerate(rows) if step_kernel in r[2]]
+    if len(cuts) < skip + 2:
+        raise SystemExit("only %d dispatches of %r: cannot cut %d warm-up steps and a timed one" % (len(cuts), step_kernel, skip))
+    return [rows[a:b] for a, b in zip(cuts[skip:], cuts[skip + 1:] + [len(rows)])]
+
+
+def analyse(step, min_us):
+    busy = 0
+    idle = collections.Counter()
+    count = collections.Counter()
+    small = 0
+    end = step[0][0]
+    for s, e, name in step:
+        if s > end:
+            gap = s - end
+            if gap < min_us * 1000:
+                small += gap
+            else:
+                idle[name] += gap
+                count[name] += 1
+            busy += e - s
+        else:
+            busy += max(0, e - max(s, end))
+        end = max(end, e)
+    return {"span": end - step[0][0], "busy": busy, "idle": idle, "count": count, "small": small}
+
+
+def main():
+    ap = argparse.ArgumentParser()
+    ap.add_argument("trace")
+    ap.add_argument("--skip", type=int, default=3)
+    ap.add_argument("--step-kernel", default="embed_csr")
+    ap.add_argument("--min-us", type=float, default=2.0)
+    ap.add_argument("--json", action="store_true")
+    a = ap.parse_args()
+    rows = load(a.trace)
+    steps = steps_of(rows, a.step_kernel, a.skip)
+    res = [analyse(s, a.min_us) for s in steps]
+    n = len(res)
+    us = lambda ns: ns / 1000.0 / n
+    idle = collections.Counter()
+    count = collections.Counter()
+    for r in res:
+        idle.update(r["idle"])
+        count.update(r["count"])
+    kern = collections.defaultdict(lambda: [0, 0])
+    for s in steps:
+        for b, e, name in s:
+            kern[name][0] += 1
+            kern[name][1] += e - b
+    out = {
+        "steps": n,
+        "span_us_per_step": us(sum(r["span"] for r in res)),
+        "busy_us_per_step": us(sum(r["busy"] for r in res)),
+        "idle_us_per_step": us(sum(sum(r["idle"].values()) + r["small"] for r in res)),
+        "idle_below_min_us_per_step": us(sum(r["small"] for r in res)),
+        "idle_before": {k: {"us_per_step": us(v), "intervals_per_step": count[k] / n} for k, v in idle.most_common()},
+        "kernels": {k: {"dispatches_per_step": c / n, "avg_us": t / 1000.0 / c, "us_per_step": us(t)}
+                    for k, (c, t) in sorted(kern.items(), key=lambda kv: -kv[1][1])},
+    }
+    if a.json:
+        print(json.dumps(out, indent=1))
+        return
+    print("%d steps: span %.1f us, busy %.1f us, idle %.1f us per step (of it %.1f us in intervals below %g us)" % (
+        n, out["span_us_per_step"], out["busy_us_per_step"], out["idle_us_per_step"], out["idle_below_min_us_per_step"],
+        a.min_us))
+    print("\n| idle before | us per step | intervals per step |\n|---|---|---|")
+    for k, v in out["idle_before"].items():
+        print("| `%s` | %.1f | %.2f |" % (k, v["us_per_step"], v["intervals_per_step"]))
+    print("\n| kernel | dispatches per step | avg us | us per step |\n|---|---|---|---|")
+    for k, v in out["kernels"].items():
+        print("| `%s` | %.2f | %.1f | %.1f |" % (k, v["dispatches_per_step"], v["avg_us"], v["us_per_step"]))
+
+
+if __name__ == "__main__":
+    main()
diff --git a/fedrann_amd/csrc/fedrann_hip.hip b/fedrann_amd/csrc/fedrann_hip.hip
--- a/fedrann_amd/csrc/fedrann_hip.hip
+++ b/fedrann_amd/csrc/fedrann_hip.hip
@@ -718,9 +718,11 @@
     int knn_mode = FDR_MODE_AUTO;
     int dedup_mode = FDR_DEDUP_AUTO;
     int live_mode = FDR_LIVE_AUTO;
-    std::vector<unsigned> live_host;
     int skip_mode = FDR_SKIP_AUTO;
     std::vector<int> skip_host;
+    PinnedBuf pin;
+    hipEvent_t pin_ev = nullptr;
+    std::vector<std::pair<const void *, int>> lds_set;
     int compact_mode = FDR_COMPACT_AUTO;
     KnnCallRecord last;
     struct {
@@ -794,6 +796,50 @@
     return FDR_OK;
 }
 
+enum { PIN_NU = 0, PIN_NUQ = 1, PIN_DUPS = 2, PIN_RANGE = 3, PIN_CERTIFY = 4 , PIN_SCALARS = 16 };
+struct KnnPin {
+    int *scalars;
+    unsigned *masks;
+    int *lens;
+    unsigned *ids;
+    int *order;
+};
+static int knn_pin(fdr_ctx *ctx, int nqb, int nseg, hipStream_t st, KnnPin &P) {
+    const size_t bytes = ((size_t)PIN_SCALARS + 3 * (size_t)nqb + (size_t)nseg * 256) * 4;
+    if (bytes > ctx->pin.cap) {
+        HIP_TRY(hipStreamSynchronize(st));
+        if (int rc = ctx->pin.reserve((bytes + 65535) / 65536 * 65536)) return rc;
+    }
+    int *const w = static_cast<int *>(ctx->pin.p);
+    P.scalars = w;
+    P.masks = reinterpret_cast<unsigned *>(w + PIN_SCALARS);
+    P.lens = w + PIN_SCALARS + nqb;
+    P.ids = reinterpret_cast<unsigned *>(P.lens + (size_t)nseg * 256);
+    P.order = reinterpret_cast<int *>(P.ids + nqb);
+    return FDR_OK;
+}
+static int knn_pin_read(fdr_ctx *ctx, int at, const int *dev, int count, hipStream_t st, const int *&host) {
+    KnnPin P;
+    if (int rc = knn_pin(ctx, 0, 0, st, P)) return rc;
+    HIP_TRY(hipMemcpyAsync(P.scalars + at, dev, (size_t)count * 4, hipMemcpyDeviceToHost, st));
+    HIP_TRY(hipStreamSynchronize(st));
+    host = P.scalars + at;
+    return FDR_OK;
+}
+
+static int set_lds_limit(fdr_ctx *ctx, const void *kern, int bytes) {
+    for (auto &s : ctx->lds_set)
+        if (s.first == kern) {
+            if (s.second >= bytes) return FDR_OK;
+            HIP_TRY(hipFuncSetAttribute(kern, hipFuncAttributeMaxDynamicSharedMemorySize, bytes));
+            s.second = bytes;
+            return FDR_OK;
+        }
+    HIP_TRY(hipFuncSetAttribute(kern, hipFuncAttributeMaxDynamicSharedMemorySize, bytes));
+    ctx->lds_set.emplace_back(kern, bytes);
+    return FDR_OK;
+}
+
 FDR_EXPORT const char *fdr_last_error(void) { return g_err; }
 
 FDR_EXPORT int fdr_padded_dim(int d) { return padded_dim(d); }
@@ -842,6 +888,7 @@
         }
     for (hipEvent_t e : ctx->aux_ev)
         if (e) (void)hipEventDestroy(e);
+    if (ctx->pin_ev) (void)hipEventDestroy(ctx->pin_ev);
     delete ctx;
     return FDR_OK;
 }
@@ -1325,6 +1372,7 @@
     int ib;
     const _Float16 *p1_q, *p1_t;
     OrderArgs ord;
+    KnnPin pin;
     const KnnShape &sh() const { return kShapes[shape]; }
     size_t lds() const { return knn_lds_bytes(sh(), L.kp); }
     _Float16 *hq() const { return self ? L.ht : L.hq; }
@@ -1338,9 +1386,11 @@
     int trc = timing_begin(ctx, FDR_KERNEL_KNN_RERANK, st);
     if (trc) return trc;
     HIP_TRY(hipMemsetAsync(L.counter, 0, 64, st));
+    const bool tkeys = L.rc && L.ordered;
     if (L.rc) {
         hipLaunchKernelGGL(to_half_compact_kernel, dim3((unsigned)((nt * (dp / 8) + 255) / 256)), dim3(256), 0, st, a.That,
-                           (long long)nt * (dp / 8), L.ht, L.rc, L.counter + 8);
+                           (long long)nt * (dp / 8), L.ht, L.rc, L.counter + 8, tkeys ? L.okeys : nullptr,
+                           tkeys ? L.ovals : nullptr);
     } else
         hipLaunchKernelGGL(to_half_kernel, dim3((unsigned)((nt * (dp / 8) + 255) / 256)), dim3(256), 0, st, a.That,
                            (long long)nt * (dp / 8), L.ht);
@@ -1355,19 +1405,22 @@
     p1_t = L.ht;
     if (L.ordered) {
         _Float16 *const ho_t = L.ho_t, *const ho_q = self ? L.ho_t : L.ho_q;
-        auto order = [&](const float *X, int64_t n, int *perm, _Float16 *out) -> int {
-            hipLaunchKernelGGL(row_chunk_keys_kernel, dim3((unsigned)(((size_t)n * 16 + 255) / 256)), dim3(256), 0, st, X,
-                               (int)n, dp, L.okeys, L.ovals);
+        auto sort_rows = [&](const float *X, int64_t n, bool keyed, int *perm) -> int {
+            if (!keyed)
+                hipLaunchKernelGGL(row_chunk_keys_kernel, dim3((unsigned)(((size_t)n * 16 + 255) / 256)), dim3(256), 0, st, X,
+                                   (int)n, dp, L.okeys, L.ovals);
             size_t tb = L.otmp_bytes;
             HIP_TRY(rocprim::radix_sort_pairs(L.otmp, tb, L.okeys, L.okeys_s, L.ovals, perm, (size_t)n, 0, 40, st));
-            const long long groups = (long long)n * (dp / 8);
-            hipLaunchKernelGGL(to_half_ordered_kernel, dim3((unsigned)((groups + 255) / 256)), dim3(256), 0, st, X,
-                               (const int *)perm, groups, dp / 8, out);
             HIP_TRY(hipGetLastError());
             return FDR_OK;
         };
+        auto ordered_copy = [&](const _Float16 *H, int64_t n, const int *perm, _Float16 *out) {
+            const long long groups = (long long)n * (dp / 8);
+            hipLaunchKernelGGL(half_ordered_kernel, dim3((unsigned)((groups + 255) / 256)), dim3(256), 0, st, H, perm, groups,
+                               dp / 8, out);
+        };
         int orc;
-        if ((orc = order(a.That, nt, L.perm_t, ho_t))) return orc;
+        if ((orc = sort_rows(a.That, nt, tkeys, L.perm_t))) return orc;
         if (L.live) {
             int max_stages = 1;
             for (int i = 0; i < p.nseg; ++i)
@@ -1380,27 +1433,34 @@
             HIP_TRY(hipGetLastError());
             ctx->last.trace.skip_live = !all;
         }
-        if (!self && (orc = order(a.Qhat, nq, L.perm_q, ho_q))) return orc;
+        if (!self && (orc = sort_rows(a.Qhat, nq, false, L.perm_q))) return orc;
         ord.perm_t = L.perm_t;
         p1_t = ho_t;
         ord.perm_q = self ? L.perm_t : L.perm_q;
         p1_q = ho_q;
         if (L.live) {
-            const long long bgroups = (long long)((nt + 31) / 32 + 4) * 32 * 16;
-            hipLaunchKernelGGL(to_half_blocked_kernel, dim3((unsigned)((bgroups + 255) / 256)), dim3(256), 0, st, a.That,
-                               (const int *)L.perm_t, (int)nt, bgroups, L.hb_t);
             hipLaunchKernelGGL(live_block_masks_kernel, dim3((unsigned)((nq + 255) / 256)), dim3(64), 0, st,
                                (const u64 *)L.okeys_s, (int)nq, L.live_masks);
             HIP_TRY(hipGetLastError());
-        }
+            if ((orc = knn_pin(ctx, p.nqb, p.nseg, st, pin))) return orc;
+            if (!ctx->pin_ev) HIP_TRY(hipEventCreateWithFlags(&ctx->pin_ev, hipEventDisableTiming));
+            HIP_TRY(hipMemcpyAsync(pin.masks, L.live_masks, (size_t)p.nqb * 4, hipMemcpyDeviceToHost, st));
+            HIP_TRY(hipMemcpyAsync(pin.lens, L.live_lens, (size_t)p.nseg * 256 * 4, hipMemcpyDeviceToHost, st));
+            HIP_TRY(hipEventRecord(ctx->pin_ev, st));
+            const long long bgroups = (long long)((nt + 31) / 32 + 4) * 32 * 16;
+            hipLaunchKernelGGL(half_ordered_blocked_kernel, dim3((unsigned)((bgroups + 255) / 256)), dim3(256), 0, st,
+                               (const _Float16 *)L.ht, (const int *)L.perm_t, (int)nt, bgroups, ho_t, L.hb_t);
+        } else
+            ordered_copy(L.ht, nt, L.perm_t, ho_t);
+        if (!self) ordered_copy(L.hq, nq, L.perm_q, ho_q);
+        HIP_TRY(hipGetLastError());
     }
     int max_seg = 1;
     for (int i = 0; i < p.nseg; ++i) max_seg = std::max(max_seg, p.segs.b[i + 1] - p.segs.b[i]);
     ib = prefilter_index_bits(max_seg);
     if (ib > FDR_PREFILTER_MAX_IB) return fail(FDR_E_ARG, "knn prefilter: segment of %d rows", max_seg);
     if ((trc = timing_end(ctx, FDR_KERNEL_KNN_RERANK, st))) return trc;
-    if (lds() > 32768)
-        HIP_TRY(hipFuncSetAttribute(reinterpret_cast<const void *>(kern), hipFuncAttributeMaxDynamicSharedMemorySize, (int)lds()));
+    if (lds() > 32768) return set_lds_limit(ctx, reinterpret_cast<const void *>(kern), (int)lds());
     return FDR_OK;
 }
 
@@ -1416,13 +1476,10 @@
     const hipStream_t st = a.st;
     const int nqb = p.nqb, kp = L.kp;
     fdr_knn_trace &tr = ctx->last.trace;
-    std::vector<unsigned> &masks = ctx->live_host;
-    masks.resize((size_t)nqb);
-    HIP_TRY(hipMemcpyAsync(masks.data(), L.live_masks, (size_t)nqb * 4, hipMemcpyDeviceToHost, st));
+    HIP_TRY(hipEventSynchronize(ctx->pin_ev));
+    const unsigned *const masks = pin.masks;
     std::vector<int> &lens = ctx->skip_host;
-    lens.resize((size_t)p.nseg * 256);
-    HIP_TRY(hipMemcpyAsync(lens.data(), L.live_lens, (size_t)p.nseg * 256 * 4, hipMemcpyDeviceToHost, st));
-    HIP_TRY(hipStreamSynchronize(st));
+    lens.assign(pin.lens, pin.lens + (size_t)p.nseg * 256);
     if (ctx->cap.what & FDR_CAPTURE_LIVE_LISTS) {
         const size_t bytes = live_stage_rows(a.nt) * 256 * sizeof(uint16_t);
         int crc = ctx->cap.lists.reserve(bytes);
@@ -1433,10 +1490,11 @@
         ctx->last.skip.segs = p.segs;
         ctx->last.skip.stream = st;
     }
-    const LivePlan lp = live_plan(masks.data(), nqb, p.nseg, ctx->live_mode == FDR_LIVE_FORCE ? 0 : p.cohort);
-    HIP_TRY(hipMemcpyAsync(L.live_ids, lp.ids.data(), (size_t)nqb * 4, hipMemcpyHostToDevice, st));
-    HIP_TRY(hipMemcpyAsync(L.live_order, lp.order.data(), (size_t)nqb * 4, hipMemcpyHostToDevice, st));
-    HIP_TRY(hipStreamSynchronize(st));
+    const LivePlan lp = live_plan(masks, nqb, p.nseg, ctx->live_mode == FDR_LIVE_FORCE ? 0 : p.cohort);
+    memcpy(pin.ids, lp.ids.data(), (size_t)nqb * 4);
+    memcpy(pin.order, lp.order.data(), (size_t)nqb * 4);
+    HIP_TRY(hipMemcpyAsync(L.live_ids, pin.ids, (size_t)nqb * 4, hipMemcpyHostToDevice, st));
+    HIP_TRY(hipMemcpyAsync(L.live_order, pin.order, (size_t)nqb * 4, hipMemcpyHostToDevice, st));
     tr.pass_live = 1;
     int dense_nq = 0;
     std::vector<long long> items;
@@ -1464,8 +1522,9 @@
     }
     for (int nl = FDR_LIVE_MIN_NL; nl <= FDR_LIVE_MAX_NL; ++nl)
         if (live_lds_bytes(nl) > 32768)
-            HIP_TRY(hipFuncSetAttribute(reinterpret_cast<const void *>(kLiveKernels[nl - FDR_LIVE_MIN_NL]),
-                                        hipFuncAttributeMaxDynamicSharedMemorySize, (int)live_lds_bytes(nl)));
+            if (int arc = set_lds_limit(ctx, reinterpret_cast<const void *>(kLiveKernels[nl - FDR_LIVE_MIN_NL]),
+                                        (int)live_lds_bytes(nl)))
+                return arc;
     return launch_rounds(ctx, p, items, 4, FDR_KERNEL_KNN_PREFILTER, false, st, r,
                          [&](hipStream_t s, unsigned grid, int base, int group) {
         const LiveGroup &g = lp.groups[(size_t)group];
@@ -1488,7 +1547,7 @@
     const int64_t nq = a.nq;
     int trc;
     if ((trc = timing_begin(ctx, FDR_KERNEL_KNN_RERANK, st))) return trc;
-    const int64_t mq = p.nseg * kp <= 64 ? 4 * MERGE_QPW : 4;
+    const int64_t mq = merge_keys_queries(p.nseg, kp);
     hipLaunchKernelGGL(knn_merge_keys_kernel, dim3((unsigned)((nq + mq - 1) / mq)), dim3(256), 0, st,
                        (const u64 *)R.partial, p.nseg, (int)nq, p.nq_pad, kp, L.cand);
     HIP_TRY(hipGetLastError());
@@ -1505,7 +1564,7 @@
     const auto rerank = L.rc ? knn_rerank_kernel<RERANK_ROWS_COMPACT> : knn_rerank_kernel<RERANK_ROWS_DENSE>;
     const int rerank_lds = L.rc ? RERANK_LDS_BYTES(RERANK_ROWS_COMPACT) : RERANK_LDS_BYTES(RERANK_ROWS_DENSE);
     const int long_limit = ctx->compact_mode == FDR_COMPACT_FORCE ? 0x7fffffff : (int)(a.nt / RC_LONG_SHARE);
-    HIP_TRY(hipFuncSetAttribute(reinterpret_cast<const void *>(rerank), hipFuncAttributeMaxDynamicSharedMemorySize, rerank_lds));
+    if ((trc = set_lds_limit(ctx, reinterpret_cast<const void *>(rerank), rerank_lds))) return trc;
     hipLaunchKernelGGL(rerank, dim3((unsigned)((nq + 3) / 4)), dim3(256), rerank_lds, st,
                        (const u64 *)L.cand, kp, k, a.Qhat, a.qzero, a.That, (int)nq, dp, (int)a.t_base, margin,
                        a.idx, a.dist, L.counter, L.flagged, L.rlist, L.theta, L.path, (const unsigned char *)L.rc, long_limit);
@@ -1516,9 +1575,8 @@
                        (const int *)L.flagged, (int)nq, (const int *)L.counter, k, a.idx, a.dist);
     HIP_TRY(hipGetLastError());
     if ((trc = timing_end(ctx, FDR_KERNEL_KNN_RERANK, st))) return trc;
-    int counts[9] = {};
-    HIP_TRY(hipMemcpyAsync(counts, L.counter, sizeof counts, hipMemcpyDeviceToHost, st));
-    HIP_TRY(hipStreamSynchronize(st));
+    const int *counts;
+    if ((trc = knn_pin_read(ctx, PIN_CERTIFY, L.counter, 9, st, counts))) return trc;
     n = {counts[0], counts[1], counts[2]};
     ctx->last.trace.rerank_compact = L.rc && counts[8] <= long_limit;
     ctx->last.trace.rerank_compact_entries = L.rc ? RC_ENTRIES : 0;
@@ -1581,9 +1639,9 @@
         ctx->cap.range_valid = true;
     }
     if ((trc = timing_end(ctx, FDR_KERNEL_KNN_RERANK, st))) return trc;
-    int count = 0;
-    HIP_TRY(hipMemcpyAsync(&count, L.counter, 4, hipMemcpyDeviceToHost, st));
-    HIP_TRY(hipStreamSynchronize(st));
+    const int *counted;
+    if ((trc = knn_pin_read(ctx, PIN_RANGE, L.counter, 1, st, counted))) return trc;
+    const int count = *counted;
     tr.range_overflow = count - n.exact;
     n.exact = count;
     return FDR_OK;
@@ -1752,10 +1810,9 @@
         hipLaunchKernelGGL(dedup_probe_kernel, dim3(g1), dim3(256), 0, st, (const u64 *)W.hash, n, W.probe_table,
                            W.probe_slots - 1, W.probe_count);
         HIP_TRY(hipGetLastError());
-        int dups = 0;
-        HIP_TRY(hipMemcpyAsync(&dups, W.probe_count, 4, hipMemcpyDeviceToHost, st));
-        HIP_TRY(hipStreamSynchronize(st));
-        if ((double)dups < 0.05 * (double)n) {
+        const int *dups;
+        if ((rc = knn_pin_read(ctx, PIN_DUPS, W.probe_count, 1, st, dups))) return rc;
+        if ((double)*dups < 0.05 * (double)n) {
             if ((trc = timing_end(ctx, FDR_KERNEL_KNN_DEDUP, st))) return trc;
             return plain(W.inner_bytes);
         }
@@ -1767,18 +1824,23 @@
     size_t tb = W.tmp_bytes;
     HIP_TRY(rocprim::inclusive_scan(W.tmp, tb, W.uqflag, W.uqpos, (size_t)n, rocprim::plus<int>(), st));
     HIP_TRY(hipGetLastError());
-    int nu = 0, nuq = 0;
-    HIP_TRY(hipMemcpyAsync(&nu, W.cid + (n - 1), 4, hipMemcpyDeviceToHost, st));
-    HIP_TRY(hipMemcpyAsync(&nuq, W.uqpos + (n - 1), 4, hipMemcpyDeviceToHost, st));
-    HIP_TRY(hipStreamSynchronize(st));
+    KnnPin pin;
+    if ((rc = knn_pin(ctx, 0, 0, st, pin))) return rc;
+    HIP_TRY(hipMemcpyAsync(pin.scalars + PIN_NU, W.cid + (n - 1), 4, hipMemcpyDeviceToHost, st));
+    HIP_TRY(hipMemcpyAsync(pin.scalars + PIN_NUQ, W.uqpos + (n - 1), 4, hipMemcpyDeviceToHost, st));
+    if (!ctx->pin_ev) HIP_TRY(hipEventCreateWithFlags(&ctx->pin_ev, hipEventDisableTiming));
+    HIP_TRY(hipEventRecord(ctx->pin_ev, st));
+    hipLaunchKernelGGL(gather_unique_rows_kernel, dim3(g16), dim3(256), 0, st, d_That, a.tzero, n, dp,
+                       (const int *)W.isrep, (const int *)W.upos, W.U, W.uzero);
+    HIP_TRY(hipGetLastError());
+    HIP_TRY(hipEventSynchronize(ctx->pin_ev));
+    const int nu = pin.scalars[PIN_NU], nuq = pin.scalars[PIN_NUQ];
     if (!dedup_worth(nu, nuq, nt, nq, k, ctx->dedup_mode) || knn_mode_workspace_bytes(env, nuq, nu, d, k) > W.inner_bytes) {
         if ((trc = timing_end(ctx, FDR_KERNEL_KNN_DEDUP, st))) return trc;
         return plain(W.inner_bytes);
     }
     ctx->last.unique_targets = nu;
     ctx->last.unique_queries = nuq;
-    hipLaunchKernelGGL(gather_unique_rows_kernel, dim3(g16), dim3(256), 0, st, d_That, a.tzero, n, dp,
-                       (const int *)W.isrep, (const int *)W.upos, W.U, W.uzero);
     if (nuq != nu)
         hipLaunchKernelGGL(gather_unique_queries_kernel, dim3((unsigned)(((size_t)nu * 16 + 255) / 256)), dim3(256),
                            0, st, (const float *)W.U, (const unsigned char *)W.uzero, nu, dp, (const int *)W.uqflag,
@@ -1832,9 +1894,9 @@
     hipLaunchKernelGGL(hash_rows_kernel, dim3(g16), dim3(256), 0, st, d_That, n, dp, W.hash, W.idx);
     HIP_TRY(hipGetLastError());
     if ((rc = queue_class_tables(W, d_That, n, dp, st))) return rc;
-    int nu = 0;
-    HIP_TRY(hipMemcpyAsync(&nu, W.cid + (n - 1), 4, hipMemcpyDeviceToHost, st));
-    HIP_TRY(hipStreamSynchronize(st));
+    const int *counted;
+    if ((rc = knn_pin_read(ctx, PIN_NU, W.cid + (n - 1), 1, st, counted))) return rc;
+    const int nu = *counted;
     if (!dedup_worth(nu, nu, nt, nt, k, ctx->dedup_mode)) return timing_end(ctx, FDR_KERNEL_KNN_DEDUP, st);
     hipLaunchKernelGGL(gather_unique_rows_kernel, dim3(g16), dim3(256), 0, st, d_That, d_tzero, n, dp,
                        (const int *)W.isrep, (const int *)W.upos, W.U, W.uzero);
diff --git a/fedrann_amd/csrc/knn_order.inc b/fedrann_amd/csrc/knn_order.inc
--- a/fedrann_amd/csrc/knn_order.inc
+++ b/fedrann_amd/csrc/knn_order.inc
@@ -21,17 +21,11 @@
     }
 }
 
-__global__ __launch_bounds__(256) void to_half_ordered_kernel(const float *__restrict__ Ehat,
-                                                              const int *__restrict__ perm, long long n_groups,
-                                                              int gpr, _Float16 *__restrict__ out) {
+__global__ __launch_bounds__(256) void half_ordered_kernel(const _Float16 *__restrict__ H, const int *__restrict__ perm,
+                                                           long long n_groups, int gpr, _Float16 *__restrict__ out) {
     const long long t = (long long)blockIdx.x * 256 + threadIdx.x;
     if (t >= n_groups) return;
     const long long i = t / gpr;
     const int g = (int)(t - i * gpr);
-    const f32x4 *src = reinterpret_cast<const f32x4 *>(Ehat) + ((size_t)perm[i] * gpr + g) * 2;
-    const f32x4 e = src[0], o = src[1];
-    f16x8 h;
-    h[0] = (_Float16)e.x; h[1] = (_Float16)o.x; h[2] = (_Float16)e.y; h[3] = (_Float16)o.y;
-    h[4] = (_Float16)e.z; h[5] = (_Float16)o.z; h[6] = (_Float16)e.w; h[7] = (_Float16)o.w;
-    reinterpret_cast<f16x8 *>(out)[t] = h;
+    reinterpret_cast<f16x8 *>(out)[t] = reinterpret_cast<const f16x8 *>(H)[(size_t)perm[i] * gpr + g];
 }
diff --git a/fedrann_amd/csrc/knn_prefilter.inc b/fedrann_amd/csrc/knn_prefilter.inc
--- a/fedrann_amd/csrc/knn_prefilter.inc
+++ b/fedrann_amd/csrc/knn_prefilter.inc
@@ -20,7 +20,8 @@
 
 __global__ __launch_bounds__(256) void to_half_compact_kernel(const float *__restrict__ Ehat, long long n_groups,
                                                               _Float16 *__restrict__ out, unsigned char *__restrict__ rc,
-                                                              int *__restrict__ n_long) {
+                                                              int *__restrict__ n_long, u64 *__restrict__ keys,
+                                                              int *__restrict__ vals) {
     __shared__ int wg_long;
     if (threadIdx.x == 0) wg_long = 0;
     __syncthreads();
@@ -40,6 +41,15 @@
         if (g >= off) incl += below;
     }
     const int total = __shfl(incl, 15, 16);
+    if (keys) {
+        unsigned m = (unsigned)(nzm != 0u) << (g >> 1);
+#pragma unroll
+        for (int off = 8; off >= 1; off >>= 1) m |= __shfl_xor(m, off, 16);
+        if (live && g == 0) {
+            keys[t >> 4] = ((u64)__popc(m) << 32) | m;
+            vals[t >> 4] = (int)(t >> 4);
+        }
+    }
     if (live) {
         unsigned char *rec = rc + (size_t)(t >> 4) * RC_BYTES;
         if (g == 0) rec[0] = (unsigned char)total;
@@ -619,6 +629,20 @@
 
 #define MERGE_QPW 4
 #define MERGE_ADAPTIVE_FROM 8
+#define MERGE_RUNS_QPW 2
+static FDR_HOST_DEVICE inline int merge_keys_queries(int nseg, int KP) {
+    if (nseg * KP <= 64) return 4 * MERGE_QPW;
+    return KP == 32 && nseg <= MERGE_ADAPTIVE_FROM ? 4 * MERGE_RUNS_QPW : 4;
+}
+__device__ __forceinline__ u64 wave_bitonic32_halves(u64 key, const int lane) {
+    static_for(std::integer_sequence<int, 16, 8, 4, 2, 1>{}, [&](auto jc) {
+        constexpr int j = decltype(jc)::value;
+        const u64 other = lane_xor64<j>(key, lane);
+        const bool take_min = ((lane & j) == 0) == ((lane & 32) == 0);
+        key = (take_min == (other < key)) ? other : key;
+    });
+    return key;
+}
 __device__ __forceinline__ u64 lane_reverse64(u64 v, const int lane) {
     u64 r = v;
     r = lane_xor64<1>(r, lane);
@@ -655,6 +679,42 @@
 #pragma unroll
         for (int t = 0; t < MERGE_QPW; ++t)
             if (lane < KP && q0 + t < nq) cand[(size_t)(q0 + t) * KP + lane] = kv[t];
+        return;
+    }
+    if (KP == 32 && nseg <= MERGE_ADAPTIVE_FROM) {
+        const int q0 = (blockIdx.x * 4 + wave) * MERGE_RUNS_QPW;
+        const int l = lane & 31, e = (l & 16) ? 47 - l : l;
+        const int np = (nseg + 1) >> 1;
+        u64 r[MERGE_RUNS_QPW][MERGE_ADAPTIVE_FROM / 2];
+#pragma unroll
+        for (int i = 0; i < MERGE_ADAPTIVE_FROM / 2; ++i) {
+            const int sg = min(2 * i + (lane >> 5), nseg - 1);
+#pragma unroll
+            for (int t = 0; t < MERGE_RUNS_QPW; ++t)
+                r[t][i] = (i < np && q0 + t < nq) ? partial[((size_t)sg * nq_pad + q0 + t) * 32 + e] : KEY_INF;
+        }
+        auto step = [&](u64 v) {
+            v = wave_bitonic32_halves(v, lane);
+            const u64 o = lane_xor64<32>(v, lane);
+            return o < v ? o : v;
+        };
+        u64 acc[MERGE_RUNS_QPW] = {};
+#pragma unroll
+        for (int i = 0; i < MERGE_ADAPTIVE_FROM / 2; ++i) {
+            if (i < np) {
+                const bool pair = 2 * i + 1 < nseg;
+#pragma unroll
+                for (int t = 0; t < MERGE_RUNS_QPW; ++t) {
+                    const u64 v = pair ? step(r[t][i]) : r[t][i];
+                    acc[t] = i == 0 ? v : step(lane < 32 ? acc[t] : v);
+                }
+            }
+        }
+#pragma unroll
+        for (int t = 0; t < MERGE_RUNS_QPW; ++t) {
+            const u64 kv = wave_bitonic<32, 32>(acc[t], lane);
+            if (lane < 32 && q0 + t < nq) cand[(size_t)(q0 + t) * 32 + lane] = kv;
+        }
         return;
     }
     u64 *sv = stage[wave];
diff --git a/fedrann_amd/csrc/knn_prefilter_live.inc b/fedrann_amd/csrc/knn_prefilter_live.inc
--- a/fedrann_amd/csrc/knn_prefilter_live.inc
+++ b/fedrann_amd/csrc/knn_prefilter_live.inc
@@ -51,9 +51,10 @@
     if (lane == 0) lens[seg * 256 + (int)v] = count;
 }
 
-__global__ __launch_bounds__(256) void to_half_blocked_kernel(const float *__restrict__ Ehat,
-                                                              const int *__restrict__ perm, int n, long long n_groups,
-                                                              _Float16 *__restrict__ out) {
+__global__ __launch_bounds__(256) void half_ordered_blocked_kernel(const _Float16 *__restrict__ H,
+                                                                   const int *__restrict__ perm, int n, long long n_groups,
+                                                                   _Float16 *__restrict__ ordered,
+                                                                   _Float16 *__restrict__ blocked) {
     const long long t = (long long)blockIdx.x * 256 + threadIdx.x;
     if (t >= n_groups) return;
     const long long i = t >> 4;
@@ -62,13 +63,11 @@
 #pragma unroll
     for (int e = 0; e < 8; ++e) h[e] = (_Float16)0.0f;
     if (i < n) {
-        const f32x4 *src = reinterpret_cast<const f32x4 *>(Ehat) + ((size_t)perm[i] * 16 + g) * 2;
-        const f32x4 e = src[0], o = src[1];
-        h[0] = (_Float16)e.x; h[1] = (_Float16)o.x; h[2] = (_Float16)e.y; h[3] = (_Float16)o.y;
-        h[4] = (_Float16)e.z; h[5] = (_Float16)o.z; h[6] = (_Float16)e.w; h[7] = (_Float16)o.w;
+        h = reinterpret_cast<const f16x8 *>(H)[(size_t)perm[i] * 16 + g];
+        reinterpret_cast<f16x8 *>(ordered)[t] = h;
     }
     const size_t slot = ((((size_t)(i >> 5) * 8 + (size_t)(g >> 1)) * 32 + (size_t)(i & 31)) << 1) + (size_t)(g & 1);
-    reinterpret_cast<f16x8 *>(out)[slot] = h;
+    reinterpret_cast<f16x8 *>(blocked)[slot] = h;
 }
 
 __global__ __launch_bounds__(256) void live_gather_dense_kernel(const _Float16 *__restrict__ hq, const int *__restrict__ perm_q,
```

After: 286.3 million, median of 2. Within noise of the previous version (+0.3%).
